# TigreGotico/phoonnx

Measured on AMD Instinct MI355X. Metric: audio samples/sec (22.05 kHz), batch-32 256-phoneme utterances, higher is better.
Workload: dtype f32 (f16x3 split: fp32 operands as two fp16 planes, three MFMA products, fp32 accumulate)

## Files before the change

include/vitsmi.h:

```cpp
#ifndef VITSMI_H
#define VITSMI_H

#include <stddef.h>
#include <stdint.h>

#ifdef __cplusplus
extern "C" {
#endif

typedef struct vits_handle vits_handle;

enum {
    VITS_OK = 0,
    VITS_E_IO = -1,
    VITS_E_FORMAT = -2,
    VITS_E_ARG = -3,
    VITS_E_DEVICE = -4,
    VITS_E_NOMEM = -5,
    VITS_E_RANGE = -6
};

#define VITS_MAX_DIMS 4


// ... 302 lines not shown
int vits_glide_emit_end(const vits_glide_seg *segs, int n_segs, int64_t n_in, int64_t n_out, int64_t X, int64_t *ready);
int64_t vits_warp_stream_cap(int64_t piece_samples, int64_t S_w);
int vits_run_chunked_glided(vits_handle *h, const int64_t *ids, const int64_t *lens, int B, int T, const int64_t *sid,
                            const vits_noise *noise, const vits_controls *ctl, const vits_contour *contour, int chunk_frames,
                            vits_chunk_fn fn, void *user);
int vits_run_chunked_enc_glided(vits_handle *h, const int64_t *ids, const int64_t *lens, int B, int T, const int64_t *sid,
                                const vits_noise *noise, const vits_controls *ctl, const vits_stream_format *fmt,
                                const vits_stream_shaping *shaping, const vits_stream_onset *onsets, const vits_contour *contour,
                                int chunk_frames, vits_enc_chunk_trim_fn fn, void *user);

enum { VITS_FIT_MET = 0, VITS_FIT_FLOOR = 1, VITS_FIT_CEIL = 2, VITS_FIT_KEPT = 3 };
typedef struct {
    const int32_t *group;
    int n_groups;
    const int64_t *target_frames;
    const int32_t *mode;
} vits_fit;
int vits_fit_plan(const float *w, const int64_t *lens, int B, int T, const vits_fit *fit, int64_t *durations, double *scale,
                  int64_t *frames, int32_t *status);
int vits_run_async_fitted(vits_handle *h, const int64_t *ids, const int64_t *lens, int B, int T, const int64_t *sid,
                          const vits_noise *noise, const vits_controls *ctl, const vits_fit *fit);
int vits_run_chunked_fitted(vits_handle *h, const int64_t *ids, const int64_t *lens, int B, int T, const int64_t *sid,
                            const vits_noise *noise, const vits_controls *ctl, const vits_fit *fit, int chunk_frames,
                            vits_chunk_fn fn, void *user);
int vits_run_chunked_enc_fitted(vits_handle *h, const int64_t *ids, const int64_t *lens, int B, int T, const int64_t *sid,
                                const vits_noise *noise, const vits_controls *ctl, const vits_stream_format *fmt,
                                const vits_stream_shaping *shaping, const vits_stream_onset *onsets, const vits_fit *fit,
                                int chunk_frames, vits_enc_chunk_trim_fn fn, void *user);
int vits_last_fit(vits_handle *h, double *scale, int64_t *frames, int32_t *status, int n);

int vits_reserve(vits_handle *h, int B, int T, int F);
int vits_get_stats(vits_handle *h, vits_stats *out);

typedef struct {
    char kernel[128];
    double flops, bytes;
    float ms;
    int stage;
    int cin, cout, k, dil, t;
} vits_launch_record;
int vits_launch_records(vits_handle *h, vits_launch_record *buf, int n);

void *vits_stream(vits_handle *h);


int vits_test_conv1d(int device_id, const float *x, int B, int Cin, int T, const float *w, const float *bias,
                     int Cout, int K, int dil, int pad_l, int flags, float slope, float *out);
int vits_bench_conv1d(int device_id, int B, int Cin, int Cout, int T, int K, int dil, int hint, int iters,
                      int cfg_override, int ck_override, float *ms_out);
int vits_test_conv_transpose1d(int device_id, const float *x, int B, int Cin, int T, const float *w,
                               const float *bias, int Cout, int K, int stride, float *out);
enum {
    VITS_CONV_PRO_LRELU = 1, VITS_CONV_PRO_MASK = 2, VITS_CONV_EPI_RELU = 4, VITS_CONV_EPI_MASK = 8, VITS_CONV_EPI_RES = 16,
    VITS_CONV_EPI_ACC = 32, VITS_CONV_EPI_DIV = 64, VITS_CONV_EPI_COUPLING = 128, VITS_CONV_EPI_WN = 256,
    VITS_CONV_EPI_WN_FIRST = 512
};
typedef struct {
    int B, Cin, T, Cout;
    int K, dil, pad_l;
    int stride;
    int hint, cfg, ck;
    int flags;
    float slope, div, oslope, oslope2;
    int wn_split;
    const float *x;
    const float *w, *bias;
    const int64_t *lens;
    const float *bias_b;
    int bias_b_stride;
    const float *res;
    int x_cstride;
    int out_cstride;
    int out_rows, out_row0;
    const float *old_out, *old_out2;
    float sentinel;
    float *out, *out2;
    int pl_rows;
    float *planes_out;
    char kernel[128];
    int cfg_used, ck_used;
} vits_test_conv_epi_args;
int vits_test_conv1d_epi(int device_id, vits_test_conv_epi_args *a);
int vits_test_wn_gate(int device_id, const float *a, int B, int H, int T, int form, float *acts);
int vits_test_cond_matvec(int device_id, const float *emb_g, int n_speakers, int gin, const int64_t *sid, int B,
                          const float *W, const float *bias, int rows, float *out);
int vits_test_conv1d_sx(int device_id, const float *x, int B, int Cin, int T, const float *w, const float *bias,
                        int Cout, int K, int dil, int pad_l, int flags, float slope, float *out);
enum { VITS_SX_EPI_RES = 1, VITS_SX_EPI_ACC = 2, VITS_SX_EPI_DIV = 4, VITS_SX_EPI_NO_RAW_STORE = 8 };
enum { VITS_SX_BF16X6 = 0, VITS_SX_F16X3 = 1, VITS_SX_F16 = 2 };
typedef struct {
    int B, Cin, T, Cout;
    int K, dil, pad_l;
    int stride;
    int precision;
    int force16, no_s16, min_cfg;
    int run_cfg;
    int flags;
    const float *x;
    const float *w, *bias;
    const float *res;
    int res_is_x;
    int res_planes;
    float res_slope;
    const float *old_out;
    const float *bias_b;
    int bias_b_stride;
    float div, oslope, oslope2, islope;
    const int64_t *lens;
    int rag_add, rag_mul;
    float sentinel;
    float *out;
    float *planes_out;
    float *res_seen;
    char kernel[128];
    int pack_cfg, run_cfg_used, rawin, s16, ck;
    float peak;
} vits_test_conv_sx_epi_args;
int vits_test_conv1d_sx_epi(int device_id, vits_test_conv_sx_epi_args *a);
int vits_test_conv1d_sx_planar(int device_id, const float *x, int B, int Cin, int T, const float *w, const float *bias,
                               int Cout, int K, int dil, int flags, const int64_t *lens, const float *old, int row_split,
                               int pl_rows, float *out, float *planes_out);
long long vits_test_set_sx_small_max(long long wgs);
int vits_test_conv1d_sx_gate(int device_id, const float *x, int B, int Cin, int T, const float *w, const float *bias,
                             const float *bias_b, int Cout, int K, int dil, int flags, float *out);
int vits_test_conv_transpose1d_sx(int device_id, const float *x, int B, int Cin, int T, const float *w,
                                  const float *bias, int Cout, int K, int stride, float *out);
int vits_bench_conv1d_sx(int device_id, int B, int Cin, int Cout, int T, int K, int dil, int dbg, int iters,
                         float *ms_out);
int vits_test_conv_pair_sx(int device_id, const float *x, int B, int C, int T, const float *w1, const float *b1,
                           const float *w2, const float *b2, int K, int dil1, int dil2, int chain, float slope, float *out,
                           float *ms_out);
enum { VITS_P16_EPI_ACC = 1, VITS_P16_EPI_DIV = 2, VITS_P16_EPI_RAW = 4, VITS_P16_EPI_PLANES = 8 };
typedef struct {
    int B, C, T, K, dil1, dil2, chain;
    int precision;
    int flags;
    float slope, div, sentinel;
    const float *x;
    const float *w1, *b1, *w2, *b2;
    const float *old_out;
    const float *x_tail;
    const int64_t *lens;
    int rag_add, rag_mul;
    float *out;
    float *planes_out;
    float *x_seen;
    float *ms_out;
    char kernel[128];
    int BN, BNo, ovl;
    float peak;
    int guard_ok;
} vits_test_conv_pair16_epi_args;
int vits_test_conv_pair16_epi(int device_id, vits_test_conv_pair16_epi_args *a);
int vits_test_attention(int device_id, const float *qkv, int B, int C, int T, int n_heads, const float *rel_k,
                        const float *rel_v, int window, const int64_t *lens, float *out);
int vits_test_attention16(int device_id, const float *qkv, int B, int C, int T, int n_heads, const float *rel_k,
                          const float *rel_v, int window, const int64_t *lens, float *out, uint16_t *out_planes, int kernel,
                          int reps, float *ms_out);
typedef struct {
    int kernel;
    const float *qkv;
    const uint16_t *qkv_planes;
    int B, C, T, n_heads, window;
    const float *rel_k, *rel_v;
    const int64_t *lens;
    int want_out;
    int want_planes;
    int ns, qt;
    int kh;
    float *out;
    uint16_t *out_planes;
    float peak;
    char kernel_name[128];
} vits_test_attention_form_args;
int vits_test_attention_form(int device_id, vits_test_attention_form_args *a);

int vits_test_resample(int device_id, const float *x, const int64_t *lens, int B, int S, int in_rate, int out_rate, float *y,
                       int64_t S_out);
int vits_test_resample_pieces(int device_id, const float *x, const int64_t *lens, int B, int S, int in_rate, int out_rate,
                              int piece_samples, float *y, int64_t S_out, int64_t *ranges, int max_ranges);
int vits_test_resample_rows(int device_id, const float *x, const int64_t *lens, int B, int S, int in_rate,
                            const int32_t *out_rates, float *y, size_t y_elems, int64_t *n_out);
int vits_test_warp(int device_id, const float *x, const int64_t *counts, int B, int S, const vits_warp_seg *segs,
                   const int32_t *seg_first , float *y, int S_w);
int vits_test_glide(int device_id, const float *x, const int64_t *counts, int B, int S, const vits_glide_seg *segs,
                    const int32_t *seg_first , float *y, int S_w);
int vits_test_warp_pieces(int device_id, const float *x, const int64_t *counts, int B, int S, const vits_warp_seg *segs,
                          const int32_t *seg_first , const int64_t *piece_bounds, int n_pieces, float *y, int S_w,
                          int64_t *ranges, int max_ranges);
int vits_test_glide_pieces(int device_id, const float *x, const int64_t *counts, int B, int S, const vits_glide_seg *segs,
                           const int32_t *seg_first , const int64_t *piece_bounds, int n_pieces, float *y, int S_w,
                           int64_t *ranges, int max_ranges);

int vits_test_durations(int device_id, const float *logw, const int64_t *dur, const int64_t *lens, int B, int T, float length_scale,
                        const float *rows, const float *token_rate, float *w_ceil, int32_t *cum, int32_t *y_len);
int vits_test_fit_durations(int device_id, const float *w, const int64_t *lens, int B, int T, const vits_fit *fit, float *w_ceil,
                            int32_t *cum, int32_t *y_len, double *scale, int64_t *frames, int32_t *status);
int vits_test_expand_prior(int device_id, const float *m_logs, int B, int C, int T, const int32_t *cum, const int64_t *lens,
                           const int32_t *y_len, int F, const float *noise, int64_t noise_stride, int noise_frames,
                           float noise_scale, const float *rows, const uint64_t *seeds, float *z_p);
int vits_test_fill_normal(int device_id, int64_t n, uint64_t seed, uint64_t stream_id, float *out);
int vits_test_fill_normal_rows(int device_id, int B, int channels, int T, const uint64_t *seeds, uint32_t stream, const float *rows,
                               int col, float *out);
int vits_test_post_conv(int device_id, const float *x, int B, int C, int T, const float *w, int K, float slope, const int64_t *vlen,
                        int hop, int kernel, float *out);

int vits_test_layernorm(int device_id, const float *x, const float *out_init, int B, int C, int T, const float *gamma,
                        const float *beta, const int64_t *lens, int flags, int form, int in_place, const float *dw_w,
                        const float *dw_b, int K, int dil, float *out, uint16_t *planes);
typedef struct vits_test_dds_layer {
    const float *dw_w, *dw_b;
    const float *ln1_g, *ln1_b;
    const float *pw_w, *pw_b;
    const float *ln2_g, *ln2_b;
    int32_t dil;
} vits_test_dds_layer;
int vits_test_dds(int device_id, int form, const float *x, int B, int C, int T, const int64_t *lens, int n_layers,
                  const vits_test_dds_layer *layers, int mask_out, const float *head_cond, const float *head_z, int head_ch,
                  const float *head_w, const float *head_b, const float *tail_w, const float *tail_b, int tail_rows, float *out);
int vits_test_cf_pre(int device_id, const float *z, int ch, const float *w, const float *bias, const float *cond, int B, int C, int T,
                     float *out);
int vits_test_rqs_inverse(int device_id, const float *pr, const float *z, int B, int T, const int64_t *lens, int ch0, int nb,
                          float sqrt_c, float *out);
int vits_test_ea_logw(int device_id, const float *z, int ch, float m0, float logs0, const int64_t *lens, int B, int T, float *out);

int vits_test_deliver(int device_id, const float *x, const int64_t *counts, int B, int S, const vits_segment *segs, int n_segs,
                      int n_streams, int encoding, void *dst, size_t dst_bytes, int64_t *stream_samples, int64_t *stream_offsets);

int vits_test_deliver_trimmed(int device_id, const float *x, const int64_t *counts, int B, int S, const vits_segment *segs,
                              const vits_trim *trims, int n_segs, int n_streams, int encoding, void *dst, size_t dst_bytes,
                              int64_t *stream_samples, int64_t *stream_offsets, int64_t *kept_first, int64_t *kept_count);

int vits_test_loudness_blocks(int device_id, const float *x, const int64_t *counts, const int64_t *firsts, int B, int S,
                              int sample_rate, float *e, size_t e_cap, int32_t *n_sub, int32_t *chunk);

int vits_test_deliver_leveled(int device_id, const float *x, const int64_t *counts, int B, int S, const vits_segment *segs,
                              const vits_trim *trims, const vits_level *levels, int n_segs, int n_streams, int encoding,
                              int sample_rate, void *dst, size_t dst_bytes, int64_t *stream_samples, int64_t *stream_offsets,
                              int64_t *kept_first, int64_t *kept_count, double *loudness, float *gain);

int vits_test_deliver_shaped(int device_id, const float *x, const int64_t *counts, int B, int S, const vits_segment *segs,
                             const vits_trim *trims, const vits_level *levels, const vits_shape *shapes, const vits_env_point *points,
                             int64_t n_points, int n_segs, int n_streams, int encoding, int sample_rate, void *dst, size_t dst_bytes,
                             int64_t *stream_samples, int64_t *stream_offsets, int64_t *kept_first, int64_t *kept_count,
                             double *loudness, float *gain);

int vits_test_deliver_limited(int device_id, const float *x, const int64_t *counts, int B, int S, const vits_segment *segs,
                              const vits_trim *trims, const vits_level *levels, const vits_shape *shapes, const vits_env_point *points,
                              int64_t n_points, const vits_limit *limits, int n_segs, int n_streams, int encoding, int sample_rate,
                              void *dst, size_t dst_bytes, int64_t *stream_samples, int64_t *stream_offsets, int64_t *kept_first,
                              int64_t *kept_count, double *loudness, float *gain);

int vits_test_stream_pack(int device_id, const float *x, const int64_t *counts, int B, int S, int piece_samples,
                          const vits_stream_format *fmt, void *bytes, size_t bytes_cap, int64_t *pitches, int32_t *valid,
                          float *peaks, int max_pieces);

int vits_test_stream_pack_shaped(int device_id, const float *x, const int64_t *counts, int B, int S, int piece_samples,
                                 const vits_stream_format *fmt, const vits_stream_shaping *shaping, void *bytes, size_t bytes_cap,
                                 int64_t *pitches, int32_t *valid, float *peaks, int64_t *firsts, int64_t *ns, int max_pieces);

int vits_test_stream_pack_trimmed(int device_id, const float *x, const int64_t *counts, int B, int S, int piece_samples,
                                  const vits_stream_format *fmt, const vits_stream_shaping *shaping, const vits_stream_onset *onsets,
                                  void *bytes, size_t bytes_cap, int64_t *pitches, int32_t *valid, int32_t *skip, float *peaks,
                                  int64_t *firsts, int64_t *ns, int32_t *start, int max_pieces);

#ifdef __cplusplus
}
#endif
#endif
```

phoonnx_amd/_ffi.py:

```python
import ctypes as C
import os

import numpy as np

from . import audio_encoding

_HERE = os.path.dirname(os.path.abspath(__file__))
_LIB = None

VITS_MAX_DIMS = 4


class VitsNoise(C.Structure):
    _fields_ = [("noise_dp", C.c_void_p), ("noise_z", C.c_void_p), ("noise_z_stride", C.c_int64),
                ("seed", C.c_uint64)]


class VitsOutput(C.Structure):
    _fields_ = [("data", C.POINTER(C.c_float)), ("dims", C.c_int64 * 4), ("y_lengths", C.POINTER(C.c_int64))]


class VitsStats(C.Structure):
    _fields_ = [("conv_flops", C.c_double), ("conv_bytes", C.c_double), ("dec_flops", C.c_double),
                ("dec_bytes", C.c_double), ("flow_flops", C.c_double), ("enc_flops", C.c_double),
                ("dp_flops", C.c_double), ("conv_ms", C.c_float), ("dec_ms", C.c_float), ("flow_ms", C.c_float),
                ("enc_ms", C.c_float), ("dp_ms", C.c_float), ("total_ms", C.c_float), ("conv_launches", C.c_int),
                ("total_launches", C.c_int), ("sx_flops", C.c_double), ("sx_ms", C.c_float), ("sx_launches", C.c_int),
                ("f16_peak_max", C.c_float), ("f16_peak_min", C.c_float), ("f16_tracked", C.c_int),
                ("f16_saturated", C.c_int), ("sx_bytes", C.c_double)]


class VitsLaunchRecord(C.Structure):
    _fields_ = [("kernel", C.c_char * 128), ("flops", C.c_double), ("bytes", C.c_double), ("ms", C.c_float),
                ("stage", C.c_int), ("cin", C.c_int), ("cout", C.c_int), ("k", C.c_int), ("dil", C.c_int), ("t", C.c_int)]


class VitsTestConvEpiArgs(C.Structure):
    _fields_ = [(n, C.c_int) for n in ("B", "Cin", "T", "Cout", "K", "dil", "pad_l", "stride", "hint", "cfg", "ck", "flags")] + \
               [(n, C.c_float) for n in ("slope", "div", "oslope", "oslope2")] + [("wn_split", C.c_int)] + \
               [(n, C.c_void_p) for n in ("x", "w", "bias", "lens", "bias_b")] + [("bias_b_stride", C.c_int), ("res", C.c_void_p)] + \
               [(n, C.c_int) for n in ("x_cstride", "out_cstride", "out_rows", "out_row0")] + \
               [("old_out", C.c_void_p), ("old_out2", C.c_void_p), ("sentinel", C.c_float), ("out", C.c_void_p), ("out2", C.c_void_p),
                ("pl_rows", C.c_int), ("planes_out", C.c_void_p), ("kernel", C.c_char * 128), ("cfg_used", C.c_int), ("ck_used", C.c_int)]


class VitsTestConvSxEpiArgs(C.Structure):
    _fields_ = [(n, C.c_int) for n in ("B", "Cin", "T", "Cout", "K", "dil", "pad_l", "stride", "precision", "force16", "no_s16",
                                       "min_cfg", "run_cfg", "flags")] + \
               [(n, C.c_void_p) for n in ("x", "w", "bias", "res")] + \
               [("res_is_x", C.c_int), ("res_planes", C.c_int), ("res_slope", C.c_float), ("old_out", C.c_void_p),
                ("bias_b", C.c_void_p), ("bias_b_stride", C.c_int)] + \
               [(n, C.c_float) for n in ("div", "oslope", "oslope2", "islope")] + \
               [("lens", C.c_void_p), ("rag_add", C.c_int), ("rag_mul", C.c_int), ("sentinel", C.c_float), ("out", C.c_void_p),
                ("planes_out", C.c_void_p), ("res_seen", C.c_void_p), ("kernel", C.c_char * 128)] + \
               [(n, C.c_int) for n in ("pack_cfg", "run_cfg_used", "rawin", "s16", "ck")] + [("peak", C.c_float)]


class VitsTestConvPair16EpiArgs(C.Structure):
    _fields_ = [(n, C.c_int) for n in ("B", "C", "T", "K", "dil1", "dil2", "chain", "precision", "flags")] + \
               [(n, C.c_float) for n in ("slope", "div", "sentinel")] + \
               [(n, C.c_void_p) for n in ("x", "w1", "b1", "w2", "b2", "old_out", "x_tail", "lens")] + \
               [("rag_add", C.c_int), ("rag_mul", C.c_int)] + \
               [(n, C.c_void_p) for n in ("out", "planes_out", "x_seen", "ms_out")] + [("kernel", C.c_char * 128)] + \
               [(n, C.c_int) for n in ("BN", "BNo", "ovl")] + [("peak", C.c_float), ("guard_ok", C.c_int)]


class VitsTestAttentionFormArgs(C.Structure):
    _fields_ = [("kernel", C.c_int), ("qkv", C.c_void_p), ("qkv_planes", C.c_void_p)] + \
               [(n, C.c_int) for n in ("B", "C", "T", "n_heads", "window")] + \
               [(n, C.c_void_p) for n in ("rel_k", "rel_v", "lens")] + \
               [(n, C.c_int) for n in ("want_out", "want_planes", "ns", "qt", "kh")] + \
               [("out", C.c_void_p), ("out_planes", C.c_void_p), ("peak", C.c_float), ("kernel_name", C.c_char * 128)]


class VitsOpenOptions(C.Structure):
    _fields_ = [("device_id", C.c_int), ("gen_precision", C.c_char_p), ("arena_dev", C.c_void_p),
                ("arena_bytes", C.c_size_t), ("host_only", C.c_int), ("layout_only", C.c_int)]


class VitsControls(C.Structure):
    _fields_ = [("scales_rows", C.c_void_p), ("seeds", C.c_void_p), ("durations", C.c_void_p), ("token_rate", C.c_void_p)]


class VitsFit(C.Structure):
    _fields_ = [("group", C.c_void_p), ("n_groups", C.c_int), ("target_frames", C.c_void_p), ("mode", C.c_void_p)]


VITS_FIT_MET, VITS_FIT_FLOOR, VITS_FIT_CEIL, VITS_FIT_KEPT = 0, 1, 2, 3


class VitsWarpSeg(C.Structure):
    _fields_ = [("n0", C.c_int64), ("pos0", C.c_int64), ("k", C.c_int64), ("step", C.c_int32), ("c", C.c_int32),
                ("half_taps", C.c_int32), ("pad_", C.c_int32)]


class VitsIntonation(C.Structure):
    _fields_ = [("token_semitones", C.c_void_p), ("compensate", C.c_int)]


class VitsGlideSeg(C.Structure):
    _fields_ = [("n0", C.c_int64), ("pos0", C.c_int64), ("k", C.c_int64), ("step0", C.c_int32), ("step1", C.c_int32),
                ("pad_", C.c_int32 * 2)]


class VitsContour(C.Structure):
    _fields_ = [("token_semitones", C.c_void_p), ("token_semitones_end", C.c_void_p), ("compensate", C.c_int)]


class VitsSegment(C.Structure):
    _fields_ = [("row", C.c_int32), ("stream", C.c_int32), ("lead_samples", C.c_int64), ("normalize", C.c_int32),
                ("volume", C.c_float)]


class VitsTrim(C.Structure):
    _fields_ = [("mode", C.c_int32), ("threshold", C.c_float), ("keep_lead", C.c_int32), ("keep_tail", C.c_int32),
                ("tail_samples", C.c_int64)]


class VitsTestDdsLayer(C.Structure):
    _fields_ = [("dw_w", C.c_void_p), ("dw_b", C.c_void_p), ("ln1_g", C.c_void_p), ("ln1_b", C.c_void_p), ("pw_w", C.c_void_p),
                ("pw_b", C.c_void_p), ("ln2_g", C.c_void_p), ("ln2_b", C.c_void_p), ("dil", C.c_int32)]


class VitsLevel(C.Structure):
    _fields_ = [("mode", C.c_int32), ("target_lufs", C.c_float), ("max_gain_db", C.c_float), ("peak_ceiling", C.c_float)]


class VitsEnvPoint(C.Structure):
    _fields_ = [("pos", C.c_int32), ("gain", C.c_float)]


class VitsShape(C.Structure):
    _fields_ = [("fade_in", C.c_int32), ("fade_out", C.c_int32), ("curve", C.c_int32), ("n_points", C.c_int32),
                ("first_point", C.c_int64)]


class VitsLimit(C.Structure):
    _fields_ = [("mode", C.c_int32), ("ceiling", C.c_float), ("lookahead", C.c_int32), ("reserved", C.c_int32)]


class VitsStreamFormat(C.Structure):
    _fields_ = [("encoding", C.c_int32), ("ref_peak", C.c_void_p), ("volume", C.c_void_p)]


class VitsStreamShaping(C.Structure):
    pass


STREAM_PLAN_FN = C.CFUNCTYPE(C.c_int, C.c_void_p, C.c_int, C.c_int, C.POINTER(C.c_int64), C.POINTER(C.c_int64), C.POINTER(VitsStreamShaping))

VitsStreamShaping._fields_ = [("shapes", C.c_void_p), ("points", C.c_void_p), ("n_points", C.c_int64), ("ceiling", C.c_void_p),
                              ("lookahead", C.c_int32), ("reserved", C.c_int32), ("plan", STREAM_PLAN_FN), ("plan_user", C.c_void_p)]


class VitsStreamOnset(C.Structure):
    _fields_ = [("mode", C.c_int32), ("threshold", C.c_float), ("keep_lead", C.c_int32), ("reserved", C.c_int32)]


ENCODINGS = {name: (code, audio_encoding.DTYPES[name]) for code, name in enumerate(audio_encoding.ENCODINGS)}


CHUNK_FN = C.CFUNCTYPE(C.c_int, C.c_void_p, C.POINTER(C.c_float), C.c_int, C.c_int64, C.c_int64, C.c_int64)

ENC_CHUNK_FN = C.CFUNCTYPE(C.c_int, C.c_void_p, C.c_void_p, C.c_int, C.c_int64, C.c_int64, C.c_int64, C.POINTER(C.c_int32),
                           C.POINTER(C.c_float), C.c_int64)

ENC_CHUNK_TRIM_FN = C.CFUNCTYPE(C.c_int, C.c_void_p, C.c_void_p, C.c_int, C.c_int64, C.c_int64, C.c_int64, C.POINTER(C.c_int32),
                                C.POINTER(C.c_int32), C.POINTER(C.c_float), C.c_int64)

VITS_E_RANGE = -6


EXPORTS = [
    "vits_open", "vits_open_with_arena", "vits_open_host", "vits_open_layout", "vits_open_opts", "vits_close",
    "vits_run_chunked", "vits_run_vocoder_chunked", "vits_last_error", "vits_num_inputs",
    "vits_input_name", "vits_meta", "vits_hparam", "vits_arena_bytes", "vits_arena_host", "vits_arena_device",
    "vits_run", "vits_free_output", "vits_run_device", "vits_sync", "vits_last_y_lengths", "vits_last_pcm16", "vits_run_vocoder",
    "vits_tap",
    "vits_set_timing", "vits_set_tails", "vits_reserve", "vits_get_stats", "vits_stream", "vits_test_conv1d", "vits_test_conv_transpose1d",
    "vits_test_attention", "vits_test_attention16", "vits_bench_conv1d", "vits_test_conv1d_sx", "vits_test_conv1d_sx_planar", "vits_test_conv1d_sx_gate", "vits_test_set_sx_small_max",
    "vits_test_conv_transpose1d_sx",
    "vits_bench_conv1d_sx", "vits_test_conv_pair_sx", "vits_fetch_output", "vits_run_async", "vits_host_alloc", "vits_host_free",
    "vits_launch_records", "vits_run_async_rows", "vits_run_device_rows", "vits_run_chunked_rows",
    "vits_run_async_ctl", "vits_run_chunked_ctl", "vits_last_durations",
    "vits_set_output_rate", "vits_last_sample_counts", "vits_resample_plan", "vits_test_resample", "vits_test_resample_pieces",
    "vits_set_output_rates", "vits_last_sample_rates", "vits_test_resample_rows",
    "vits_run_async_warped", "vits_last_token_spans", "vits_warp_token", "vits_warp_plan", "vits_test_warp",
    "vits_run_async_glided", "vits_glide_token", "vits_glide_cutoff", "vits_glide_plan", "vits_test_glide",
    "vits_warp_emit_end", "vits_glide_emit_end", "vits_warp_stream_cap", "vits_run_chunked_glided", "vits_run_chunked_enc_glided",
    "vits_test_warp_pieces", "vits_test_glide_pieces",
    "vits_fit_plan", "vits_run_async_fitted", "vits_run_chunked_fitted", "vits_run_chunked_enc_fitted", "vits_last_fit",
    "vits_test_fit_durations",
    "vits_test_durations", "vits_test_expand_prior", "vits_test_fill_normal", "vits_test_fill_normal_rows", "vits_test_post_conv",
    "vits_delivery_plan", "vits_deliver", "vits_test_deliver",
    "vits_trim_range", "vits_delivery_plan_trimmed", "vits_deliver_trimmed", "vits_test_deliver_trimmed",
    "vits_loudness_filter", "vits_loudness_gate", "vits_level_gain", "vits_delivery_plan_leveled", "vits_deliver_leveled",
    "vits_test_loudness_blocks", "vits_test_deliver_leveled",
    "vits_shape_check", "vits_shape_gain", "vits_deliver_shaped", "vits_test_deliver_shaped",
    "vits_limit_check", "vits_limit_gains", "vits_deliver_limited", "vits_test_deliver_limited",
    "vits_run_chunked_enc", "vits_run_vocoder_chunked_enc", "vits_test_stream_pack",
    "vits_stream_shaping_check", "vits_stream_emit_range", "vits_run_chunked_enc_shaped", "vits_run_vocoder_chunked_enc_shaped",
    "vits_test_stream_pack_shaped",
    "vits_stream_onset_check", "vits_stream_onset_start", "vits_run_chunked_enc_trimmed", "vits_run_vocoder_chunked_enc_trimmed",
    "vits_test_stream_pack_trimmed",
    "vits_test_layernorm", "vits_test_dds", "vits_test_cf_pre", "vits_test_rqs_inverse", "vits_test_ea_logw",
    "vits_test_conv1d_epi", "vits_test_wn_gate", "vits_test_cond_matvec", "vits_test_conv1d_sx_epi",
    "vits_test_conv_pair16_epi", "vits_test_attention_form",
]


G2P_EXPORTS = ["g2p_open", "g2p_close", "g2p_last_error", "g2p_hparam", "g2p_num_outputs", "g2p_output_name", "g2p_bucket",
               "g2p_run", "g2p_generate", "g2p_generate_batch", "g2p_test_forced_steps", "g2p_test_linear", "g2p_test_step"]


def lib_path():
    return os.environ.get("VITSMI_LIB") or os.path.join(_HERE, "libvitsmi.so")


def load():
    global _LIB
    if _LIB is not None:
        return _LIB
    path = lib_path()
    if not os.environ.get("VITSMI_LIB"):
        from . import build as _build
        if _build.stale():
            try:
                _build.build()
            except Exception as e:
                raise RuntimeError(f"{path} is missing or was not built from the sources in this tree (source_sha "
                                   f"{_build.source_sha()} vs recorded {_build.read_build_info().get('source_sha')}) "
                                   f"and cannot be rebuilt here: {e}") from e
    lib = C.CDLL(path)
    vp, i64p, f32p = C.c_void_p, C.POINTER(C.c_int64), C.POINTER(C.c_float)
    lib.vits_open.argtypes = [C.c_char_p, C.c_int, C.POINTER(vp)]
    lib.vits_open_with_arena.argtypes = [C.c_char_p, C.c_int, vp, C.c_size_t, C.POINTER(vp)]
    lib.vits_open_host.argtypes = [C.c_char_p, C.POINTER(vp)]
    lib.vits_open_layout.argtypes = [C.c_char_p, C.POINTER(vp)]
    lib.vits_open_opts.argtypes = [C.c_char_p, C.POINTER(VitsOpenOptions), C.POINTER(vp)]
    lib.vits_run_chunked.argtypes = [vp, vp, vp, C.c_int, C.c_int, vp, vp, C.POINTER(VitsNoise), C.c_int, CHUNK_FN, vp]
    lib.vits_run_vocoder_chunked.argtypes = [vp, vp, C.c_int, C.c_int, vp, C.c_int, CHUNK_FN, vp]
    lib.vits_close.argtypes = [vp]
    lib.vits_close.restype = None
    lib.vits_last_error.argtypes = [vp]
    lib.vits_last_error.restype = C.c_char_p
    lib.vits_num_inputs.argtypes = [vp]
    lib.vits_input_name.argtypes = [vp, C.c_int]
    lib.vits_input_name.restype = C.c_char_p
    lib.vits_meta.argtypes = [vp, C.c_char_p, C.c_char_p, C.c_size_t]
    lib.vits_hparam.argtypes = [vp, C.c_char_p, i64p]
    lib.vits_arena_bytes.argtypes = [vp]
    lib.vits_arena_bytes.restype = C.c_size_t
    lib.vits_arena_host.argtypes = [vp]
    lib.vits_arena_host.restype = vp
    lib.vits_arena_device.argtypes = [vp]
    lib.vits_arena_device.restype = vp
    run_args = [vp, vp, vp, C.c_int, C.c_int, vp, vp, C.POINTER(VitsNoise), C.POINTER(VitsOutput)]
    lib.vits_run.argtypes = run_args
    lib.vits_run_device.argtypes = run_args
    lib.vits_run_async.argtypes = run_args[:-1]
    lib.vits_run_async_rows.argtypes = run_args[:-1] + [vp]
    lib.vits_run_device_rows.argtypes = run_args[:-1] + [vp, C.POINTER(VitsOutput)]
    lib.vits_run_chunked_rows.argtypes = [vp, vp, vp, C.c_int, C.c_int, vp, vp, C.POINTER(VitsNoise), vp, C.c_int, CHUNK_FN, vp]
    lib.vits_run_async_ctl.argtypes = [vp, vp, vp, C.c_int, C.c_int, vp, C.POINTER(VitsNoise), C.POINTER(VitsControls)]
    lib.vits_run_chunked_ctl.argtypes = [vp, vp, vp, C.c_int, C.c_int, vp, C.POINTER(VitsNoise), C.POINTER(VitsControls),
                                         C.c_int, CHUNK_FN, vp]
    lib.vits_run_chunked_enc.argtypes = [vp, vp, vp, C.c_int, C.c_int, vp, C.POINTER(VitsNoise), C.POINTER(VitsControls),
                                         C.POINTER(VitsStreamFormat), C.c_int, ENC_CHUNK_FN, vp]
    lib.vits_run_vocoder_chunked_enc.argtypes = [vp, vp, C.c_int, C.c_int, vp, C.POINTER(VitsStreamFormat), C.c_int, ENC_CHUNK_FN, vp]
    lib.vits_stream_shaping_check.argtypes = [C.POINTER(VitsStreamShaping), C.POINTER(VitsStreamFormat), C.c_int]
    lib.vits_stream_emit_range.argtypes = [C.c_int64, C.c_int64, C.c_int, C.c_int64, C.c_int, i64p, i64p]
    lib.vits_run_chunked_enc_shaped.argtypes = [vp, vp, vp, C.c_int, C.c_int, vp, C.POINTER(VitsNoise), C.POINTER(VitsControls),
                                                C.POINTER(VitsStreamFormat), C.POINTER(VitsStreamShaping), C.c_int, ENC_CHUNK_FN, vp]
    lib.vits_run_vocoder_chunked_enc_shaped.argtypes = [vp, vp, C.c_int, C.c_int, vp, C.POINTER(VitsStreamFormat),
                                                        C.POINTER(VitsStreamShaping), C.c_int, ENC_CHUNK_FN, vp]
    lib.vits_test_stream_pack_shaped.argtypes = [C.c_int, vp, vp, C.c_int, C.c_int, C.c_int, C.POINTER(VitsStreamFormat),
                                                 C.POINTER(VitsStreamShaping), vp, C.c_size_t, vp, vp, vp, vp, vp, C.c_int]
    lib.vits_stream_onset_check.argtypes = [C.POINTER(VitsStreamOnset), C.POINTER(VitsStreamFormat), C.c_int]
    lib.vits_stream_onset_start.argtypes = [C.c_int64, C.c_int64, C.c_int64, i64p]
    lib.vits_run_chunked_enc_trimmed.argtypes = [vp, vp, vp, C.c_int, C.c_int, vp, C.POINTER(VitsNoise), C.POINTER(VitsControls),
                                                 C.POINTER(VitsStreamFormat), C.POINTER(VitsStreamShaping), C.POINTER(VitsStreamOnset),
                                                 C.c_int, ENC_CHUNK_TRIM_FN, vp]
    lib.vits_run_vocoder_chunked_enc_trimmed.argtypes = [vp, vp, C.c_int, C.c_int, vp, C.POINTER(VitsStreamFormat),
                                                         C.POINTER(VitsStreamShaping), C.POINTER(VitsStreamOnset), C.c_int,
                                                         ENC_CHUNK_TRIM_FN, vp]
    lib.vits_test_stream_pack_trimmed.argtypes = [C.c_int, vp, vp, C.c_int, C.c_int, C.c_int, C.POINTER(VitsStreamFormat),
                                                  C.POINTER(VitsStreamShaping), C.POINTER(VitsStreamOnset), vp, C.c_size_t, vp, vp, vp, vp,
                                                  vp, vp, vp, C.c_int]
    lib.vits_test_stream_pack.argtypes = [C.c_int, vp, vp, C.c_int, C.c_int, C.c_int, C.POINTER(VitsStreamFormat), vp, C.c_size_t,
                                          vp, vp, vp, C.c_int]
    lib.vits_last_durations.argtypes = [vp, i64p, C.c_size_t]
    lib.vits_set_output_rate.argtypes = [vp, C.c_int, C.c_int]
    lib.vits_last_sample_counts.argtypes = [vp, i64p, C.c_int]
    lib.vits_resample_plan.argtypes = [C.c_int, C.c_int, i64p, i64p, i64p, vp, C.c_size_t]
    lib.vits_test_resample.argtypes = [C.c_int, vp, vp, C.c_int, C.c_int, C.c_int, C.c_int, vp, C.c_int64]
    lib.vits_test_resample_pieces.argtypes = [C.c_int, vp, vp, C.c_int, C.c_int, C.c_int, C.c_int, C.c_int, vp, C.c_int64, vp, C.c_int]
    lib.vits_set_output_rates.argtypes = [vp, C.c_int, vp, C.c_int]
    lib.vits_last_sample_rates.argtypes = [vp, vp, C.c_int]
    lib.vits_test_resample_rows.argtypes = [C.c_int, vp, vp, C.c_int, C.c_int, C.c_int, vp, vp, C.c_size_t, vp]
    lib.vits_run_async_warped.argtypes = [vp, vp, vp, C.c_int, C.c_int, vp, C.POINTER(VitsNoise), C.POINTER(VitsControls),
                                          C.POINTER(VitsIntonation)]
    lib.vits_last_token_spans.argtypes = [vp, i64p, C.c_size_t]
    lib.vits_warp_token.argtypes = [C.c_float, i64p, i64p, C.POINTER(C.c_int32)]
    lib.vits_warp_plan.argtypes = [vp, vp, C.c_int, C.c_int, vp, vp, i64p]
    lib.vits_test_warp.argtypes = [C.c_int, vp, vp, C.c_int, C.c_int, vp, vp, vp, C.c_int]
    lib.vits_run_async_glided.argtypes = [vp, vp, vp, C.c_int, C.c_int, vp, C.POINTER(VitsNoise), C.POINTER(VitsControls),
                                          C.POINTER(VitsContour)]
    lib.vits_glide_token.argtypes = [C.c_float, C.c_float, i64p, i64p, C.POINTER(C.c_float)]
    lib.vits_glide_cutoff.argtypes = [C.c_int64, i64p, C.POINTER(C.c_int32)]
    lib.vits_glide_plan.argtypes = [vp, vp, vp, C.c_int, C.c_int, vp, vp, i64p]
    lib.vits_test_glide.argtypes = [C.c_int, vp, vp, C.c_int, C.c_int, vp, vp, vp, C.c_int]
    for name in ("vits_warp_emit_end", "vits_glide_emit_end"):
        getattr(lib, name).argtypes = [vp, C.c_int, C.c_int64, C.c_int64, C.c_int64, i64p]
    lib.vits_warp_stream_cap.argtypes = [C.c_int64, C.c_int64]
    lib.vits_warp_stream_cap.restype = C.c_int64
    lib.vits_run_chunked_glided.argtypes = [vp, vp, vp, C.c_int, C.c_int, vp, C.POINTER(VitsNoise), C.POINTER(VitsControls),
                                            C.POINTER(VitsContour), C.c_int, CHUNK_FN, vp]
    lib.vits_run_chunked_enc_glided.argtypes = [vp, vp, vp, C.c_int, C.c_int, vp, C.POINTER(VitsNoise), C.POINTER(VitsControls),
                                                C.POINTER(VitsStreamFormat), C.POINTER(VitsStreamShaping), C.POINTER(VitsStreamOnset),
                                                C.POINTER(VitsContour), C.c_int, ENC_CHUNK_TRIM_FN, vp]
    for name in ("vits_test_warp_pieces", "vits_test_glide_pieces"):
        getattr(lib, name).argtypes = [C.c_int, vp, vp, C.c_int, C.c_int, vp, vp, vp, C.c_int, vp, C.c_int, vp, C.c_int]
    lib.vits_fit_plan.argtypes = [vp, vp, C.c_int, C.c_int, C.POINTER(VitsFit), vp, vp, vp, vp]
    lib.vits_run_async_fitted.argtypes = [vp, vp, vp, C.c_int, C.c_int, vp, C.POINTER(VitsNoise), C.POINTER(VitsControls),
                                          C.POINTER(VitsFit)]
    lib.vits_run_chunked_fitted.argtypes = [vp, vp, vp, C.c_int, C.c_int, vp, C.POINTER(VitsNoise), C.POINTER(VitsControls),
                                            C.POINTER(VitsFit), C.c_int, CHUNK_FN, vp]
    lib.vits_run_chunked_enc_fitted.argtypes = [vp, vp, vp, C.c_int, C.c_int, vp, C.POINTER(VitsNoise), C.POINTER(VitsControls),
                                                C.POINTER(VitsStreamFormat), C.POINTER(VitsStreamShaping), C.POINTER(VitsStreamOnset),
                                                C.POINTER(VitsFit), C.c_int, ENC_CHUNK_TRIM_FN, vp]
    lib.vits_last_fit.argtypes = [vp, vp, vp, vp, C.c_int]
    lib.vits_test_fit_durations.argtypes = [C.c_int, vp, vp, C.c_int, C.c_int, C.POINTER(VitsFit), vp, vp, vp, vp, vp, vp]
    lib.vits_test_durations.argtypes = [C.c_int, vp, vp, vp, C.c_int, C.c_int, C.c_float, vp, vp, vp, vp, vp]
    lib.vits_test_expand_prior.argtypes = [C.c_int, vp, C.c_int, C.c_int, C.c_int, vp, vp, vp, C.c_int, vp, C.c_int64, C.c_int,
                                           C.c_float, vp, vp, vp]
    lib.vits_test_fill_normal.argtypes = [C.c_int, C.c_int64, C.c_uint64, C.c_uint64, vp]
    lib.vits_test_fill_normal_rows.argtypes = [C.c_int, C.c_int, C.c_int, C.c_int, vp, C.c_uint32, vp, C.c_int, vp]
    lib.vits_test_post_conv.argtypes = [C.c_int, vp, C.c_int, C.c_int, C.c_int, vp, C.c_int, C.c_float, vp, C.c_int, C.c_int, vp]
    lib.vits_test_layernorm.argtypes = [C.c_int, vp, vp, C.c_int, C.c_int, C.c_int, vp, vp, vp, C.c_int, C.c_int, C.c_int, vp, vp,
                                        C.c_int, C.c_int, vp, vp]
    lib.vits_test_dds.argtypes = [C.c_int, C.c_int, vp, C.c_int, C.c_int, C.c_int, vp, C.c_int, C.POINTER(VitsTestDdsLayer), C.c_int,
                                  vp, vp, C.c_int, vp, vp, vp, vp, C.c_int, vp]
    lib.vits_test_cf_pre.argtypes = [C.c_int, vp, C.c_int, vp, vp, vp, C.c_int, C.c_int, C.c_int, vp]
    lib.vits_test_rqs_inverse.argtypes = [C.c_int, vp, vp, C.c_int, C.c_int, vp, C.c_int, C.c_int, C.c_float, vp]
    lib.vits_test_ea_logw.argtypes = [C.c_int, vp, C.c_int, C.c_float, C.c_float, vp, C.c_int, C.c_int, vp]
    lib.vits_delivery_plan.argtypes = [vp, C.c_int, vp, C.c_int, C.c_int, C.c_int, vp, vp, i64p]
    lib.vits_deliver.argtypes = [vp, vp, C.c_int, C.c_int, C.c_int, vp, C.c_size_t, vp, vp]
    lib.vits_test_deliver.argtypes = [C.c_int, vp, vp, C.c_int, C.c_int, vp, C.c_int, C.c_int, C.c_int, vp, C.c_size_t, vp, vp]
    lib.vits_trim_range.argtypes = [C.c_int64, C.c_int64, C.c_int64, C.POINTER(VitsTrim), i64p, i64p]
    lib.vits_delivery_plan_trimmed.argtypes = [vp, C.c_int, vp, vp, C.c_int, C.c_int, C.c_int, vp, vp, i64p]
    lib.vits_deliver_trimmed.argtypes = [vp, vp, vp, C.c_int, C.c_int, C.c_int, vp, C.c_size_t, vp, vp, vp, vp]
    lib.vits_test_deliver_trimmed.argtypes = [C.c_int, vp, vp, C.c_int, C.c_int, vp, vp, C.c_int, C.c_int, C.c_int, vp, C.c_size_t,
                                              vp, vp, vp, vp]
    lib.vits_loudness_filter.argtypes = [C.c_int, vp, vp]
    lib.vits_loudness_gate.argtypes = [vp, vp, C.c_int, C.c_int32, vp, vp, vp, vp]
    lib.vits_level_gain.argtypes = [C.c_double, C.c_float, C.POINTER(VitsLevel), C.POINTER(C.c_float)]
    lib.vits_delivery_plan_leveled.argtypes = [vp, C.c_int, vp, vp, vp, C.c_int, C.c_int, C.c_int, C.c_int, vp, vp, i64p]
    lib.vits_deliver_leveled.argtypes = [vp, vp, vp, vp, C.c_int, C.c_int, C.c_int, C.c_int, vp, C.c_size_t, vp, vp, vp, vp, vp, vp]
    lib.vits_test_loudness_blocks.argtypes = [C.c_int, vp, vp, vp, C.c_int, C.c_int, C.c_int, vp, C.c_size_t, vp, vp]
    lib.vits_test_deliver_leveled.argtypes = [C.c_int, vp, vp, C.c_int, C.c_int, vp, vp, vp, C.c_int, C.c_int, C.c_int, C.c_int, vp,
                                              C.c_size_t, vp, vp, vp, vp, vp, vp]
    lib.vits_shape_check.argtypes = [vp, C.c_int, vp, C.c_int64]
    lib.vits_shape_gain.argtypes = [C.POINTER(VitsShape), vp, C.c_int64, C.c_int64, C.c_int64, C.POINTER(C.c_float)]
    lib.vits_deliver_shaped.argtypes = [vp, vp, vp, vp, vp, vp, C.c_int64, C.c_int, C.c_int, C.c_int, C.c_int, vp, C.c_size_t, vp, vp, vp,
                                        vp, vp, vp]
    lib.vits_test_deliver_shaped.argtypes = [C.c_int, vp, vp, C.c_int, C.c_int, vp, vp, vp, vp, vp, C.c_int64, C.c_int, C.c_int, C.c_int,
                                             C.c_int, vp, C.c_size_t, vp, vp, vp, vp, vp, vp]
    lib.vits_limit_check.argtypes = [vp, vp, C.c_int]
    lib.vits_limit_gains.argtypes = [vp, C.c_int64, C.POINTER(VitsLimit), vp]
    lib.vits_deliver_limited.argtypes = [vp, vp, vp, vp, vp, vp, C.c_int64, vp, C.c_int, C.c_int, C.c_int, C.c_int, vp, C.c_size_t, vp,
                                         vp, vp, vp, vp, vp]
    lib.vits_test_deliver_limited.argtypes = [C.c_int, vp, vp, C.c_int, C.c_int, vp, vp, vp, vp, vp, C.c_int64, vp, C.c_int, C.c_int,
                                              C.c_int, C.c_int, vp, C.c_size_t, vp, vp, vp, vp, vp, vp]
    lib.vits_free_output.argtypes = [vp, C.POINTER(VitsOutput)]
    lib.vits_free_output.restype = None
    lib.vits_sync.argtypes = [vp]
    lib.vits_last_y_lengths.argtypes = [vp, i64p, C.c_int]
    lib.vits_last_pcm16.argtypes = [vp, C.c_int, C.c_float, vp, C.c_size_t]
    lib.vits_run_vocoder.argtypes = [vp, vp, C.c_int, C.c_int, vp, C.POINTER(VitsOutput)]
    lib.vits_tap.argtypes = [vp, C.c_char_p, vp, C.c_size_t, i64p]
    lib.vits_set_timing.argtypes = [vp, C.c_int]
    lib.vits_set_tails.argtypes = [vp, C.c_int]
    lib.vits_reserve.argtypes = [vp, C.c_int, C.c_int, C.c_int]
    lib.vits_get_stats.argtypes = [vp, C.POINTER(VitsStats)]
    lib.vits_stream.argtypes = [vp]
    lib.vits_stream.restype = vp
    lib.vits_fetch_output.argtypes = [vp, vp, C.c_size_t, C.c_size_t]
    lib.vits_host_alloc.argtypes = [C.c_size_t]
    lib.vits_host_alloc.restype = vp
    lib.vits_host_free.argtypes = [vp]
    lib.vits_host_free.restype = None
    lib.vits_launch_records.argtypes = [vp, C.POINTER(VitsLaunchRecord), C.c_int]
    lib.vits_test_conv1d.argtypes = [C.c_int, vp, C.c_int, C.c_int, C.c_int, vp, vp, C.c_int, C.c_int, C.c_int,
                                     C.c_int, C.c_int, C.c_float, vp]
    lib.vits_test_conv_transpose1d.argtypes = [C.c_int, vp, C.c_int, C.c_int, C.c_int, vp, vp, C.c_int, C.c_int,
                                               C.c_int, vp]
    lib.vits_test_attention.argtypes = [C.c_int, vp, C.c_int, C.c_int, C.c_int, C.c_int, vp, vp, C.c_int, vp, vp]
    lib.vits_test_attention16.argtypes = [C.c_int, vp, C.c_int, C.c_int, C.c_int, C.c_int, vp, vp, C.c_int, vp, vp, vp,
                                          C.c_int, C.c_int, f32p]
    lib.vits_bench_conv1d.argtypes = [C.c_int] * 11 + [f32p]
    lib.vits_test_conv1d_sx.argtypes = lib.vits_test_conv1d.argtypes
    lib.vits_test_conv_transpose1d_sx.argtypes = lib.vits_test_conv_transpose1d.argtypes
    lib.vits_test_conv1d_sx_planar.argtypes = [C.c_int, vp, C.c_int, C.c_int, C.c_int, vp, vp, C.c_int, C.c_int, C.c_int, C.c_int,
                                               vp, vp, C.c_int, C.c_int, vp, vp]
    lib.vits_test_set_sx_small_max.argtypes = [C.c_longlong]
    lib.vits_test_set_sx_small_max.restype = C.c_longlong
    lib.vits_test_conv1d_sx_gate.argtypes = [C.c_int, vp, C.c_int, C.c_int, C.c_int, vp, vp, vp, C.c_int, C.c_int, C.c_int, C.c_int, vp]
    lib.vits_bench_conv1d_sx.argtypes = [C.c_int] * 9 + [f32p]
    lib.vits_test_conv1d_epi.argtypes = [C.c_int, C.POINTER(VitsTestConvEpiArgs)]
    lib.vits_test_conv1d_sx_epi.argtypes = [C.c_int, C.POINTER(VitsTestConvSxEpiArgs)]
    lib.vits_test_conv_pair16_epi.argtypes = [C.c_int, C.POINTER(VitsTestConvPair16EpiArgs)]
    lib.vits_test_attention_form.argtypes = [C.c_int, C.POINTER(VitsTestAttentionFormArgs)]
    lib.vits_test_wn_gate.argtypes = [C.c_int, vp, C.c_int, C.c_int, C.c_int, C.c_int, vp]
    lib.vits_test_cond_matvec.argtypes = [C.c_int, vp, C.c_int, C.c_int, vp, C.c_int, vp, vp, C.c_int, vp]
    lib.vits_test_conv_pair_sx.argtypes = [C.c_int, vp, C.c_int, C.c_int, C.c_int, vp, vp, vp, vp, C.c_int, C.c_int,
                                           C.c_int, C.c_int, C.c_float, vp, f32p]
    lib.g2p_open.argtypes = [C.c_char_p, C.c_int, C.POINTER(vp)]
    lib.g2p_close.argtypes = [vp]
    lib.g2p_close.restype = None
    lib.g2p_last_error.argtypes = [vp]
    lib.g2p_last_error.restype = C.c_char_p
    lib.g2p_hparam.argtypes = [vp, C.c_char_p, i64p]
    lib.g2p_num_outputs.argtypes = [vp]
    lib.g2p_output_name.argtypes = [vp, C.c_int]
    lib.g2p_output_name.restype = C.c_char_p
    lib.g2p_bucket.argtypes = [vp, C.c_int, C.c_int]
    lib.g2p_run.argtypes = [vp, vp, C.c_int, vp, vp, C.c_int, vp]
    lib.g2p_generate.argtypes = [vp, vp, C.c_int, C.c_int, C.c_int64, C.c_int64, vp, C.POINTER(C.c_int)]
    lib.g2p_generate_batch.argtypes = [vp, vp, vp, C.c_int, C.c_int, C.c_int64, C.c_int64, vp, vp]
    lib.g2p_test_forced_steps.argtypes = [vp, vp, vp, C.c_int, vp, C.c_int, vp]
    lib.g2p_test_linear.argtypes = [C.c_int, C.c_int, vp, vp, C.c_int, vp, C.c_int, C.c_int, vp, C.c_int64, C.c_int64, C.c_int, vp]
    lib.g2p_test_step.argtypes = [C.c_int, C.c_int, C.c_int, vp, vp, vp, C.c_int, vp, vp, C.c_int, C.c_float, C.c_float, vp, vp]
    _LIB = lib
    return lib


def ptr(a):
    return None if a is None else a.ctypes.data_as(C.c_void_p)


def last_error(h=None):
    return load().vits_last_error(h).decode("utf-8", "replace")
```

phoonnx_amd/csrc/conv_sx_pair.hip.hpp:

```cpp
#pragma once
#include <cstdlib>
#include "conv_geom.hpp"
#include "conv_sx_engine.hip.hpp"

namespace vitsmi {

struct SxPairArgs {
    const float *xr;
    float islope, mslope;
    int T;
    const u32x4 *wp1, *wp2;
    const float *bias1, *bias2;
    float wscale1, wscale2;
    float *out_raw;
    const float *zeros;
    int C, nchunks;
    int K1, dil1, pad1;
    int K2, dil2, pad2;
    int LW1;
    unsigned x_bytes;
    int LW2;
    unsigned y_chunk_bytes;
    int BNo, NT, B;
    int flags;
    float div;
    unsigned *peak;
    struct Chain {
        const u32x4 *wp1, *wp2;
        const float *bias1, *bias2;
        float wscale1, wscale2;
        int K1, dil1, K2, dil2;
        int xoff, yoff;
    } ch[3];
    int nchain;
    unsigned a_ring;
    unsigned bias_off;
    unsigned long long *prof;
    SxRagged rag;
    int xgs = 0;
};

#ifndef SX_PAIR_PROF
#define SX_PAIR_PROF 0
#endif
#ifndef SX_PAIR_SHARED_A
#define SX_PAIR_SHARED_A 0
#endif
#ifndef SX_PAIR_ALIAS
#define SX_PAIR_ALIAS 0
#endif
#ifndef SX_PAIR_DEPTH32
#define SX_PAIR_DEPTH32 2
#endif
#ifndef SX_PAIR_DEPTH64
#define SX_PAIR_DEPTH64 2
#endif
#ifndef SX_PAIR_EARLY_ACC
#define SX_PAIR_EARLY_ACC 0
#endif
#ifndef SX_PAIR_WGS32
#define SX_PAIR_WGS32 3
#endif
#ifndef SX_PAIR_EARLY32
#define SX_PAIR_EARLY32 1
#endif
#ifndef SX_PAIR_ST_SC1
#define SX_PAIR_ST_SC1 0
#endif
#ifndef SX_PAIR_ONE_READ64
#define SX_PAIR_ONE_READ64 1
#endif
#ifndef SX_PAIR_ONE_READ32
#define SX_PAIR_ONE_READ32 1
#endif
template <int MW, int NW, int WM, int WN, int EPI, bool CHAIN, int NCH = 1>
__global__ __launch_bounds__(256, (NW == 2 && !SX_PAIR_EARLY_ACC && NCH == 1) ? SX_PAIR_WGS32 : 2) void conv_sx_pair_kernel(SxPairArgs a) {
    constexpr int BN = NW * WN * 32, NH = NW / 2;
    static_assert(NCH == 1 || (CHAIN && NW == 2 && (EPI & EPI_ACC) == 0), "fused chains: 32 channels, no external running sum");
    constexpr bool ONE_READ = NW == 4 ? SX_PAIR_ONE_READ64 != 0 : SX_PAIR_ONE_READ32 != 0;
    constexpr bool EARLY = ONE_READ || (NW == 2 && SX_PAIR_EARLY32);
    constexpr int DEPTH = NW == 2 ? SX_PAIR_DEPTH32 : SX_PAIR_DEPTH64;
    static_assert(DEPTH >= 2 && DEPTH <= 6, "wait_a covers up to five younger sets");
    constexpr bool ACC = (EPI & EPI_ACC) != 0 && SX_PAIR_EARLY_ACC;
    static_assert(!(ONE_READ && ACC), "the running sum is not pulled into the single-read prologue");
    static_assert(WM * WN == 4 && MW == 1 && BN == 256, "one block row per wave, 256 columns");
    constexpr int NPW = 2, STEPBYTES = WM * MW * NPW * 1024;
    constexpr int MAXCH = WM * 2;
    extern __shared__ __attribute__((aligned(16))) unsigned char lds_sx[];
    const int tid = threadIdx.x, lane = tid & 63;
    const int wave = __builtin_amdgcn_readfirstlane(tid >> 6);
    const int wm = wave / WN, wn = wave % WN;
    const int l31 = lane & 31, hi = lane >> 5;
    const int wg_xcd = blockIdx.x & 7, wg_seq = blockIdx.x >> 3;
    const int tile_nb = __builtin_amdgcn_readfirstlane(sx_xcd_tile(wg_seq, wg_xcd, a.xgs));
    if (tile_nb >= a.NT * a.B) return;
    const int b = tile_nb / a.NT, t0 = (tile_nb - b * a.NT) * a.BNo;
    const int t1 = t0 - a.pad2;
    const int T = a.T, LW = a.LW1;
    const int TV = __builtin_amdgcn_readfirstlane(sx_valid_cols(a.rag, b, T));
    if (t0 >= TV) return;
    const uint32_t lds0 = (uint32_t)(uintptr_t)lds_sx;
    const uint32_t XB = a.x_bytes;
    const char *wbase1 = reinterpret_cast<const char *>(a.wp1) + wm * (MW * NPW * 1024);
    const char *wbase2 = reinterpret_cast<const char *>(a.wp2) + wm * (MW * NPW * 1024);
    const float *xrb = a.xr + (int64_t)b * a.C * T;
    float pk = 0.f;

    struct ASet {
        u32x4 fa[2];
    };
    const uint32_t voff0 = (uint32_t)lane * 16u;
    auto load_a = [&](ASet &f, const char *wb, int step) {
        const char *sb = wb + (int64_t)step * STEPBYTES;
        f.fa[0] = global_read128<0>(voff0, sb);
        f.fa[1] = global_read128<1024>(voff0, sb);
    };

    f32x4 pre[NW / 2][2][4], ad[EARLY && ACC ? NW / 2 : 1][2][4];
    auto load_res = [&](const float *base, f32x4 (*dst)[2][4]) {
        static_for<NW / 2>([&](auto R) {
            constexpr int rr = decltype(R)::value;
#pragma unroll
            for (int j = 0; j < 2; j++) {
                const int row0 = wm * 32;
                const int t = t1 + (wn * NW + rr * 2 + j) * 32 + l31;
                const int tl = t < 0 ? 0 : (t < T ? t : T - 1);
#pragma unroll
                for (int q = 0; q < 4; q++) {
                    const float *p = base + ((int64_t)((row0 >> 3) + q) * T + tl) * 8 + 4 * hi;
                    if constexpr (EARLY) dst[rr][j][q] = __builtin_bit_cast(f32x4, global_read128_v<0>(p));
                    else dst[rr][j][q] = *reinterpret_cast<const f32x4 *>(p);
                }
            }
        });
    };
    auto load_pre = [&]() { load_res(xrb, pre); };

#if SX_PAIR_PROF
    auto stamp = [&]() {
        unsigned long long t;
        __builtin_amdgcn_sched_barrier(0);
        asm volatile("s_memtime %0\n\ts_waitcnt lgkmcnt(0)" : "=s"(t)::"memory");
        __builtin_amdgcn_sched_barrier(0);
        return t;
    };
    unsigned long long tp[8];
    tp[0] = stamp();
#endif
    if constexpr (NW == 2 && WM == 1 && NCH == 1 && SX_PAIR_SHARED_A != 0)
        for (int g = 0; g < 3; g++)
            if (g < ((a.nchunks * a.K1) >> 1)) {
                const int sub = wave >> 1, pl = wave & 1;
                lds_dma<16>(wbase1 + (int64_t)(2 * g + sub) * STEPBYTES + pl * 1024 + lane * 16,
                            reinterpret_cast<float *>(lds_sx + a.a_ring + (unsigned)((g * 2 + sub) * 2048 + pl * 1024)));
            }
    constexpr bool BIAS_LDS = NCH == 1;
    if constexpr (BIAS_LDS) {
        if (wave == 0) {
            constexpr int CC = WM * 32;
            const int k = lane - (lane >= CC / 4 ? CC / 4 : 0);
            const float *bp = lane < CC / 4 ? a.bias1 : a.bias2;
            const void *src = (bp && lane < CC / 2) ? static_cast<const void *>(bp + 4 * k) : static_cast<const void *>(a.zeros + 4 * (lane & 31));
            lds_dma<16>(src, reinterpret_cast<float *>(lds_sx + a.bias_off));
        }
    }
    auto bias_from_lds = [&](int conv, f32x4 (&bq)[4]) __attribute__((always_inline)) {
        u32x4 t4[4];
#pragma unroll
        for (int q = 0; q < 4; q++)
            asm volatile("ds_read_b128 %0, %1" : "=v"(t4[q]) : "v"(lds0 + a.bias_off + (uint32_t)(conv * (WM * 32) + wm * 32 + 8 * q + 4 * hi) * 4u) : "memory");
        asm volatile("s_waitcnt lgkmcnt(0)" ::: "memory");
        __builtin_amdgcn_sched_barrier(0);
#pragma unroll
        for (int q = 0; q < 4; q++) bq[q] = __builtin_bit_cast(f32x4, t4[q]);
    };
    constexpr int NXC = 3;
    if constexpr (ONE_READ) {
        constexpr int NXH = MAXCH, NG = 2 * MAXCH;
        const int HW = LW - 256, pad1 = a.pad1;
        const int nhc = HW * NG, nxh = (nhc + 255) >> 8;
        u32x4 hst[NXH][2];
        bool hin[NXH], hok[NXH];
        uint32_t hlds[NXH];
        const float *hp[NXH];
#pragma unroll
        for (int it = 0; it < NXH; it++) {
            const int h = it * 256 + tid;
            hin[it] = h < nhc;
            const int g = hin[it] ? h / HW : 0;
            const int c = hin[it] ? h - g * HW : 0;
            const int col = c < pad1 ? c : c + 256;
            const int t = t1 - pad1 + col;
            hok[it] = hin[it] && t >= 0 && t < TV;
            hp[it] = xrb + (hok[it] ? ((int64_t)g * T + t) * 8 : (int64_t)0);
            hlds[it] = lds0 + (uint32_t)(g >> 1) * XB + (uint32_t)((g & 1) * LW + col) * 16u;
        }
        static_for<NXH>([&](auto I) {
            constexpr int it = decltype(I)::value;
            if (it < nxh) {
                hst[it][0] = global_read128_v<0>(hp[it]);
                hst[it][1] = global_read128_v<16>(hp[it]);
            }
        });
        load_pre();
        const float isl = a.islope;
        static_for<NW>([&](auto N) {
            constexpr int n = decltype(N)::value;
            asm volatile("s_waitcnt vmcnt(%0)" ::"n"(4 * (NW - 1 - n)) : "memory");
            __builtin_amdgcn_sched_barrier(0);
#if SX_PAIR_PROF
            if constexpr (n == 0) tp[1] = stamp();
#endif
            if constexpr (n == 0) {
                static_for<NXH>([&](auto I) {
                    constexpr int it = decltype(I)::value;
                    if (it < nxh && hin[it]) {
                        float v[8];
#pragma unroll
                        for (int e = 0; e < 8; e++) {
                            const float x = hok[it] ? __uint_as_float(hst[it][e >> 2][e & 3]) : 0.f;
                            v[e] = fmaxf(x, x * isl);
                        }
                        unsigned p0[4], p1[4];
#pragma unroll
                        for (int e = 0; e < 4; e++) split2h_pair_pk(v[2 * e], v[2 * e + 1], p0[e], p1[e], pk);
                        ds_write128(hlds[it], u32x4{p0[0], p0[1], p0[2], p0[3]});
                        ds_write128(hlds[it] + (uint32_t)(2 * LW) * 16u, u32x4{p1[0], p1[1], p1[2], p1[3]});
                    }
                });
            }
            const int col = (wn * NW + n) * 32 + l31;
            const int t = t1 + col;
            const bool ok = t >= 0 && t < TV;
#pragma unroll
            for (int q = 0; q < 4; q++) {
                float v[4];
#pragma unroll
                for (int e = 0; e < 4; e++) {
                    const float x = ok ? pre[n / 2][n % 2][q][e] : 0.f;
                    v[e] = fmaxf(x, x * isl);
                }
                unsigned wa[2], wb[2];
                split2h_pair_pk(v[0], v[1], wa[0], wa[1], pk);
                split2h_pair_pk(v[2], v[3], wb[0], wb[1], pk);
                const int g = 4 * wm + q;
                const uint32_t cell = lds0 + (uint32_t)(g >> 1) * XB + (uint32_t)((g & 1) * LW + pad1 + col) * 16u + 8u * hi;
                asm volatile("ds_write_b64 %0, %1" ::"v"(cell), "v"(u32x2{wa[0], wb[0]}) : "memory");
                asm volatile("ds_write_b64 %0, %1" ::"v"(cell + (uint32_t)(2 * LW) * 16u), "v"(u32x2{wa[1], wb[1]}) : "memory");
            }
            asm volatile("" : "+v"(pk));
        });
    } else {
        u32x4 xst[MAXCH][NXC][2];
        const int nxc = (2 * LW + 255) >> 8;
        uint32_t xroff[NXC];
        bool xrok[NXC];
        int xkh[NXC], xcol[NXC];
#pragma unroll
        for (int it = 0; it < NXC; it++) {
            const int i = it * 256 + tid;
            const int kh = (i >= LW ? 1 : 0) + (i >= 2 * LW ? 1 : 0);
            const int col = i - kh * LW;
            const int t = t1 - a.pad1 + col;
            xkh[it] = kh;
            xcol[it] = col;
            xrok[it] = it < nxc && kh < 2 && t >= 0 && t < TV;
            xroff[it] = xrok[it] ? (uint32_t)(((int64_t)kh * T + t) * 32) : 0u;
        }
        static_for<MAXCH>([&](auto CH) {
            constexpr int ch = decltype(CH)::value;
            const float *cbase = xrb + (int64_t)(2 * ch) * T * 8;
            static_for<NXC>([&](auto I) {
                constexpr int it = decltype(I)::value;
                if (it < nxc) {
                    xst[ch][it][0] = global_read128_x<0>(xroff[it], cbase);
                    xst[ch][it][1] = global_read128_x<16>(xroff[it], cbase);
                }
            });
        });
        if constexpr (EARLY) {
            load_pre();
            if constexpr (ACC) {
                load_res(a.out_raw + (int64_t)b * a.C * T, ad);
                asm volatile("s_waitcnt vmcnt(16)" ::: "memory");
            } else
                asm volatile("s_waitcnt vmcnt(8)" ::: "memory");
        } else
            asm volatile("s_waitcnt vmcnt(0)" ::: "memory");
#if SX_PAIR_PROF
        tp[1] = stamp();
#endif
        const float isl = a.islope;
        static_for<MAXCH>([&](auto CH) {
            constexpr int ch = decltype(CH)::value;
            static_for<NXC>([&](auto I) {
                constexpr int it = decltype(I)::value;
                if (it < nxc && xkh[it] < 2) {
                    float v[8];
#pragma unroll
                    for (int e = 0; e < 8; e++) {
                        const float x = xrok[it] ? __uint_as_float(xst[ch][it][e >> 2][e & 3]) : 0.f;
                        v[e] = fmaxf(x, x * isl);
                    }
                    unsigned p0[4], p1[4];
#pragma unroll
                    for (int e = 0; e < 4; e++) split2h_pair_pk(v[2 * e], v[2 * e + 1], p0[e], p1[e], pk);
                    const uint32_t ad = lds0 + (uint32_t)ch * XB + (uint32_t)(xkh[it] * LW + xcol[it]) * 16u;
                    ds_write128(ad, u32x4{p0[0], p0[1], p0[2], p0[3]});
                    ds_write128(ad + (uint32_t)(2 * LW) * 16u, u32x4{p1[0], p1[1], p1[2], p1[3]});
                }
            });
        });
    }

    f32x16 acc[NW];
    auto zero_acc = [&]() {
#pragma unroll
        for (int n = 0; n < NW; n++)
#pragma unroll
            for (int r = 0; r < 16; r++) acc[n][r] = 0.f;
    };
    zero_acc();
    u32x4 fb[NW][2];
// ... 24 lines not shown
    };
    const std::integral_constant<int, 0> H0{};
    const std::integral_constant<int, 1> H1{};

    auto wait_a = [&](int younger) {
        switch (younger) {
            case 0: asm volatile("s_waitcnt vmcnt(0)" ::: "memory"); break;
            case 1: asm volatile("s_waitcnt vmcnt(2)" ::: "memory"); break;
            case 2: asm volatile("s_waitcnt vmcnt(4)" ::: "memory"); break;
            case 3: asm volatile("s_waitcnt vmcnt(6)" ::: "memory"); break;
            case 4: asm volatile("s_waitcnt vmcnt(8)" ::: "memory"); break;
            default: asm volatile("s_waitcnt vmcnt(10)" ::: "memory"); break;
        }
    };
    auto run_conv = [&](ASet(&fs)[DEPTH + 1], const char *wb, int K, int dil, uint32_t rows0, uint32_t chunk_bytes,
                        uint32_t pstride) {
        constexpr int NS = DEPTH + 1;
        const int S = a.nchunks * K;
        int chunk = 0, tap = 0;
        static_for<DEPTH - 1>([&](auto I) {
            constexpr int i = decltype(I)::value + 1;
            if (i < S) load_a(fs[i], wb, i);
        });
        load_b_half(H0, rows0, pstride);
        load_b_half(H1, rows0, pstride);
        auto step = [&](ASet &fc, ASet &fload, int s) {
            const int left = S - 1 - s;
            wait_a(left < DEPTH - 1 ? left : DEPTH - 1);
            __builtin_amdgcn_sched_barrier(0);
            if (s + DEPTH < S && !SX_NOA) load_a(fload, wb, s + DEPTH);
            int ntap = tap + 1, nchunk = chunk;
            if (ntap == K) {
                ntap = 0;
                nchunk++;
            }
            const bool more = s + 1 < S;
            const uint32_t next = rows0 + (uint32_t)nchunk * chunk_bytes + (uint32_t)(ntap * dil) * 16u;
            __builtin_amdgcn_sched_barrier(0);
            wait_lds_older_half();
            __builtin_amdgcn_sched_barrier(0);
            mma_half(fc, H0);
            __builtin_amdgcn_sched_barrier(0);
            if (more) {
                load_b_half(H0, next, pstride);
                wait_lds_older_half();
            } else
                asm volatile("s_waitcnt lgkmcnt(0)" ::: "memory");
            __builtin_amdgcn_sched_barrier(0);
            mma_half(fc, H1);
            __builtin_amdgcn_sched_barrier(0);
            if (more) load_b_half(H1, next, pstride);
            __builtin_amdgcn_sched_barrier(0);
            tap = ntap;
            chunk = nchunk;
        };
        int s = 0;
        for (; s + NS <= S; s += NS)
            static_for<NS>([&](auto I) {
                constexpr int i = decltype(I)::value;
                step(fs[i], fs[(i + DEPTH) % NS], s + i);
            });
        __builtin_amdgcn_sched_barrier(0);
        asm volatile("s_waitcnt lgkmcnt(0)" ::: "memory");
        __builtin_amdgcn_sched_barrier(0);
        static_for<NS - 1>([&](auto I) {
            constexpr int i = decltype(I)::value;
            if (s + i < S) step(fs[i], fs[(i + DEPTH) % NS], s + i);
        });
    };

    constexpr bool SHA = NW == 2 && WM == 1 && NCH == 1 && SX_PAIR_SHARED_A != 0;
    constexpr int RG = 3;
    auto sha_dma = [&](const char *wb, int g) {
        const int sub = wave >> 1, pl = wave & 1;
        const char *src = wb + (int64_t)(2 * g + sub) * STEPBYTES + pl * 1024 + lane * 16;
        lds_dma<16>(src, reinterpret_cast<float *>(lds_sx + a.a_ring + (unsigned)(((g % RG) * 2 + sub) * 2048 + pl * 1024)));
    };
    auto sha_prefetch = [&](const char *wb, int K) {
        const int NG = (a.nchunks * K) >> 1;
#pragma unroll
        for (int g = 0; g < RG; g++)
            if (g < NG) sha_dma(wb, g);
    };
    auto wait_vm_le = [&](int n) {
        switch (n) {
            case 0: asm volatile("s_waitcnt vmcnt(0)" ::: "memory"); break;
            case 1: asm volatile("s_waitcnt vmcnt(1)" ::: "memory"); break;
            default: asm volatile("s_waitcnt vmcnt(2)" ::: "memory"); break;
        }
    };
    auto run_conv_sha = [&](ASet &fa0, ASet &fa1, const char *wb, int K, int dil, uint32_t rows0, uint32_t chunk_bytes,
                            uint32_t pstride) {
        const int S = a.nchunks * K, NG = S >> 1;
        const uint32_t alds = lds0 + a.a_ring + (uint32_t)lane * 16u;
        auto read_a = [&](ASet &f, int st) {
            const uint32_t ad = alds + (uint32_t)((((st >> 1) % RG) * 2 + (st & 1)) * 2048);
            f.fa[0] = ds_read128<0>(ad);
            f.fa[1] = ds_read128<1024>(ad);
        };
        int chunk = 0, tap = 0;
        wait_vm_le((NG < RG ? NG : RG) - 1);
        __builtin_amdgcn_s_barrier();
        __builtin_amdgcn_sched_barrier(0);
        read_a(fa0, 0);
        load_b_half(H0, rows0, pstride);
        load_b_half(H1, rows0, pstride);
        auto step = [&](ASet &fc, ASet &fload, int st, bool boundary) {
            int ntap = tap + 1, nchunk = chunk;
            if (ntap == K) {
                ntap = 0;
                nchunk++;
            }
            const bool more = st + 1 < S;
            const uint32_t next = rows0 + (uint32_t)nchunk * chunk_bytes + (uint32_t)(ntap * dil) * 16u;
            __builtin_amdgcn_sched_barrier(0);
            wait_lds_older_half();
            __builtin_amdgcn_sched_barrier(0);
            mma_half(fc, H0);
            __builtin_amdgcn_sched_barrier(0);
            if (more) {
                if (boundary && NG > RG) {
                    const int g = st >> 1;
                    const int last = g + RG - 1 < NG - 1 ? g + RG - 1 : NG - 1;
                    wait_vm_le(last - (g + 1));
                    __builtin_amdgcn_s_barrier();
                    __builtin_amdgcn_sched_barrier(0);
                    if (g + RG < NG) sha_dma(wb, g + RG);
                }
                read_a(fload, st + 1);
                load_b_half(H0, next, pstride);
                asm volatile("s_waitcnt lgkmcnt(4)" ::: "memory");
            } else
                asm volatile("s_waitcnt lgkmcnt(0)" ::: "memory");
            __builtin_amdgcn_sched_barrier(0);
            mma_half(fc, H1);
            __builtin_amdgcn_sched_barrier(0);
            if (more) load_b_half(H1, next, pstride);
            __builtin_amdgcn_sched_barrier(0);
            tap = ntap;
            chunk = nchunk;
        };
        for (int g = 0; g < NG; g++) {
            step(fa0, fa1, 2 * g, false);
            step(fa1, fa0, 2 * g + 1, true);
        }
    };

    struct ChainPar {
        const char *wb1, *wb2;
        const float *bias1, *bias2;
        float ws1, ws2;
        int K1, dil1, K2, dil2;
        uint32_t xoff, yoff;
    };
    auto chain_par = [&](int ci) {
        ChainPar c;
        if constexpr (NCH == 1) {
            c = ChainPar{wbase1, wbase2, a.bias1, a.bias2, a.wscale1, a.wscale2, a.K1, a.dil1, a.K2, a.dil2, 0u, 0u};
        } else {
            const auto &h = a.ch[ci];
            c = ChainPar{reinterpret_cast<const char *>(h.wp1) + wm * (MW * NPW * 1024),
                         reinterpret_cast<const char *>(h.wp2) + wm * (MW * NPW * 1024),
                         h.bias1, h.bias2, h.wscale1, h.wscale2, h.K1, h.dil1, h.K2, h.dil2, (uint32_t)h.xoff, (uint32_t)h.yoff};
        }
        return c;
    };
    static_assert(NCH == 1 || EARLY, "fused chains keep x in registers from the prologue on");
    const uint32_t ylds = NCH > 1 ? lds0 + (uint32_t)a.nchunks * XB : lds0;
    f32x4 xkeep[NCH > 1 ? NW / 2 : 1][2][4], tot[NCH > 1 ? NW / 2 : 1][2][4];
#if SX_PAIR_ALIAS
    ASet f1s[DEPTH + 1];
    ASet(&f2s)[DEPTH + 1] = f1s;
#else
    ASet f1s[DEPTH + 1], f2s[DEPTH + 1];
#endif
#pragma unroll 1
    for (int ci = 0; ci < NCH; ci++) {
    const ChainPar cp = chain_par(ci);
    if constexpr (NCH > 1) {
        if (ci > 0) {
#pragma unroll
            for (int rr = 0; rr < NW / 2; rr++)
#pragma unroll
                for (int j = 0; j < 2; j++)
#pragma unroll
                    for (int q = 0; q < 4; q++) pre[rr][j][q] = xkeep[rr][j][q];
            zero_acc();
        }
    }
    if constexpr (!SHA) load_a(f1s[0], cp.wb1, 0);
    if (ci == 0) {
        asm volatile("s_waitcnt lgkmcnt(0)" ::: "memory");
#if SX_PAIR_PROF
        tp[2] = stamp();
#endif
        __builtin_amdgcn_s_barrier();
#if SX_PAIR_PROF
        tp[3] = stamp();
#endif
    }
    __builtin_amdgcn_sched_barrier(0);
    if constexpr (SHA)
        run_conv_sha(f1s[0], f1s[1], cp.wb1, cp.K1, cp.dil1, lds0 + (uint32_t)(hi * LW + wn * (NW * 32) + l31 + (int)cp.xoff) * 16u,
                     XB, (uint32_t)(2 * LW) * 16u);
    else
        run_conv(f1s, cp.wb1, cp.K1, cp.dil1, lds0 + (uint32_t)(hi * LW + wn * (NW * 32) + l31 + (int)cp.xoff) * 16u, XB,
                 (uint32_t)(2 * LW) * 16u);

#if SX_PAIR_PROF
    tp[4] = stamp();
#endif
    if constexpr (CHAIN && !EARLY) load_pre();

    if constexpr (!SHA) load_a(f2s[0], cp.wb2, 0);
    asm volatile("s_waitcnt lgkmcnt(0)" ::: "memory");
    __builtin_amdgcn_s_barrier();
    __builtin_amdgcn_sched_barrier(0);
    if constexpr (SHA) sha_prefetch(cp.wb2, cp.K2);
    {
        const float wsc = cp.ws1, msl = a.mslope;
        const float *biasp = cp.bias1 ? cp.bias1 : a.zeros;
        const int b_on = cp.bias1 ? 1 : 0;
        const uint32_t YC = a.y_chunk_bytes, LW2 = (uint32_t)a.LW2;
        const int row0 = wm * 32;
        f32x4 bq[4];
        if constexpr (BIAS_LDS) bias_from_lds(0, bq);
        else {
#pragma unroll
            for (int q = 0; q < 4; q++) bq[q] = *reinterpret_cast<const f32x4 *>(biasp + (row0 + 8 * q + 4 * hi) * b_on);
        }
#pragma unroll
        for (int n = 0; n < NW; n++) {
            const int col = (wn * NW + n) * 32 + l31;
            const int t = t1 + col;
            const bool live = t >= 0 && t < TV;
#pragma unroll
            for (int q = 0; q < 4; q++) {
                float o[4];
#pragma unroll
                for (int e = 0; e < 4; e++) {
                    float v = __builtin_fmaf(acc[n][4 * q + e], wsc, bq[q][e]);
                    if constexpr (CHAIN) {
                        if constexpr (NCH > 1) {
                            if (ci == 0) xkeep[n / 2][n % 2][q][e] = pre[n / 2][n % 2][q][e];
                        }
                        v += pre[n / 2][n % 2][q][e];
                        pre[n / 2][n % 2][q][e] = v;
                    }
                    o[e] = live ? fmaxf(v, v * msl) : 0.f;
                }
                unsigned wa[2], wb[2];
                split2h_pair_pk(o[0], o[1], wa[0], wa[1], pk);
                split2h_pair_pk(o[2], o[3], wb[0], wb[1], pk);
                const int g = 4 * wm + q;
                const uint32_t cell = ylds + (uint32_t)(g >> 1) * YC + ((uint32_t)(g & 1) * LW2 + (uint32_t)(col + a.pad2)) * 16u + 8u * hi;
                asm volatile("ds_write_b64 %0, %1" ::"v"(cell), "v"(u32x2{wa[0], wb[0]}) : "memory");
                asm volatile("ds_write_b64 %0, %1" ::"v"(cell + 2u * LW2 * 16u), "v"(u32x2{wa[1], wb[1]}) : "memory");
            }
            asm volatile("" : "+v"(pk));
        }
    }
    zero_acc();
    asm volatile("s_waitcnt lgkmcnt(0)" ::: "memory");
    __builtin_amdgcn_s_barrier();
    __builtin_amdgcn_sched_barrier(0);
#if SX_PAIR_PROF
    tp[5] = stamp();
#endif

    if constexpr (SHA)
        run_conv_sha(f2s[0], f2s[1], cp.wb2, cp.K2, cp.dil2, ylds + (uint32_t)(hi * a.LW2 + wn * (NW * 32) + l31 + (int)cp.yoff) * 16u,
                     a.y_chunk_bytes, (uint32_t)(2 * a.LW2) * 16u);
    else
        run_conv(f2s, cp.wb2, cp.K2, cp.dil2, ylds + (uint32_t)(hi * a.LW2 + wn * (NW * 32) + l31 + (int)cp.yoff) * 16u,
                 a.y_chunk_bytes, (uint32_t)(2 * a.LW2) * 16u);
#if SX_PAIR_PROF
    tp[6] = stamp();
#endif
    if constexpr (!CHAIN && !EARLY) load_pre();

    {
        constexpr int flags = EPI;
        float *rawb = a.out_raw + (int64_t)b * a.C * T;
        const float wsc = cp.ws2, rdiv = a.div;
        const float *biasp = cp.bias2 ? cp.bias2 : a.zeros;
        const int b_on = cp.bias2 ? 1 : 0;
        const int row0 = wm * 32;
        f32x4 bq[4];
        if constexpr (BIAS_LDS) bias_from_lds(1, bq);
        else {
#pragma unroll
            for (int q = 0; q < 4; q++) bq[q] = *reinterpret_cast<const f32x4 *>(biasp + (row0 + 8 * q + 4 * hi) * b_on);
        }
        static_for<NW / 2>([&](auto R) {
            constexpr int rr = decltype(R)::value;
            f32x4 adl[2][4];
            if constexpr ((flags & EPI_ACC) != 0 && !(EARLY && ACC)) {
#pragma unroll
                for (int j = 0; j < 2; j++) {
                    const int t = t1 + (wn * NW + rr * 2 + j) * 32 + l31;
                    const int tl = t < 0 ? 0 : (t < T ? t : T - 1);
#pragma unroll
                    for (int q = 0; q < 4; q++)
                        adl[j][q] = *reinterpret_cast<const f32x4 *>(rawb + ((int64_t)((row0 >> 3) + q) * T + tl) * 8 + 4 * hi);
                }
            }
#pragma unroll
            for (int j = 0; j < 2; j++) {
                const int n = rr * 2 + j;
                const int col = (wn * NW + n) * 32 + l31;
                const int t = t1 + col;
                const bool kept = !(col < a.pad2 || col >= a.pad2 + a.BNo || t >= TV);
                if constexpr (NCH == 1) {
                    if (!kept) continue;
                }
#pragma unroll
                for (int q = 0; q < 4; q++) {
                    f32x4 v;
#pragma unroll
                    for (int e = 0; e < 4; e++) v[e] = __builtin_fmaf(acc[n][4 * q + e], wsc, bq[q][e]);
                    v += pre[rr][j][q];
                    if constexpr (NCH > 1) {
                        if (ci > 0) v += tot[rr][j][q];
                        tot[rr][j][q] = v;
                        if (ci < NCH - 1 || !kept) continue;
                    }
                    if constexpr ((flags & EPI_ACC) != 0) {
                        if constexpr (EARLY && ACC) v += ad[rr][j][q];
                        else v += adl[j][q];
                    }
                    if constexpr ((flags & EPI_DIV) != 0) {
#pragma unroll
                        for (int e = 0; e < 4; e++) v[e] = v[e] / rdiv;
                    }
#if SX_PAIR_ST_SC1
                    {
                        float *sp = rawb + ((int64_t)((row0 >> 3) + q) * T + t) * 8 + 4 * hi;
                        const f32x4 sv = v;
                        asm volatile("global_store_dwordx4 %0, %1, off sc1" ::"v"(sp), "v"(sv) : "memory");
                    }
#else
                    *reinterpret_cast<f32x4 *>(rawb + ((int64_t)((row0 >> 3) + q) * T + t) * 8 + 4 * hi) = v;
#endif
                }
            }
        });
    }
    }
#if SX_PAIR_PROF
    asm volatile("s_waitcnt vmcnt(0)" ::: "memory");
    tp[7] = stamp();
    if (a.prof && tid == 0) {
        for (int i = 0; i < 7; i++) atomicAdd(a.prof + i, tp[i + 1] - tp[i]);
        atomicAdd(a.prof + 7, 1ull);
    }
#endif
    if (a.peak) sx_publish_peak(a.peak, (int)blockIdx.x, pk);
}

template <int MW, int NW, int WM, int WN, int EPI, bool CHAIN, int NCH = 1>
inline hipError_t launch_conv_sx_pair_k(const SxPairArgs &a, dim3 grid, size_t lds, hipStream_t stream) {
    static std::atomic<uint64_t> attr_done{0};
    auto kern = conv_sx_pair_kernel<MW, NW, WM, WN, EPI, CHAIN, NCH>;
    if (hipError_t e = sx_allow_big_lds(reinterpret_cast<const void *>(kern), attr_done); e != hipSuccess) return e;
    if (g_launch_name_on)
        snprintf(g_launch_name, sizeof g_launch_name, "conv_sx_pair_kernel<%d, %d, %d, %d, %d, %s, %d>", MW, NW, WM, WN, EPI,
                 CHAIN ? "true" : "false", NCH);
    kern<<<grid, 256, lds, stream>>>(a);
    return hipGetLastError();
}

inline bool sx_pair_supported(int C, int cfg, int K1, int dil1, int K2, int dil2) {
    if (K1 < 3 || K2 < 3 || dil1 < 1 || dil2 < 1) return false;
    if (!((C == 64 && cfg == 1) || (C == 32 && cfg == 2))) return false;
    const int LW1 = 256 + (K1 - 1) * dil1;
    if (2 * LW1 > kSxRawStageCells) return false;
    const int halo2 = (K2 - 1) * dil2;
    static const int keep_min = [] {
        const char *e = std::getenv("VITSMI_PAIR_MIN_KEEP");
        return e ? std::atoi(e) : 160;
    }();
    if (halo2 % 2 || 256 - halo2 < keep_min) return false;
    static const int keep64 = [] {
        const char *e = std::getenv("VITSMI_PAIR_MIN_KEEP64");
        return e ? std::atoi(e) : 200;
    }();
    if (C == 64 && 256 - halo2 < keep64) return false;
    const size_t lds_y = (size_t)(C / 16) * 4 * (size_t)((256 + halo2 / 2 + 7) / 8 * 8) * 16 + (size_t)(halo2 / 2) * 16;
    const size_t lds_x = (size_t)(C / 16) * 4 * LW1 * 16;
    return (lds_y > lds_x ? lds_y : lds_x) <= kLdsTwoPerCu;
}

hipError_t launch_conv_sx_pair(SxPairArgs a, int cfg, int B, hipStream_t stream, bool chain = false);
hipError_t launch_conv_sx_mrf(SxPairArgs a, int B, hipStream_t stream);
#ifdef VITSMI_IMPL_PAIR
hipError_t launch_conv_sx_pair(SxPairArgs a, int cfg, int B, hipStream_t stream, bool chain) {
    a.LW1 = 256 + (a.K1 - 1) * a.dil1;
    a.x_bytes = (unsigned)((size_t)4 * a.LW1 * 16);
    if (a.dil2 < 1) a.dil2 = 1;
    const int halo2 = (a.K2 - 1) * a.dil2;
    if (a.pad2 * 2 != halo2) return hipErrorInvalidValue;
    a.LW2 = (256 + a.pad2 + 7) / 8 * 8;
    a.y_chunk_bytes = (unsigned)(4 * a.LW2 * 16);
    a.BNo = 256 - halo2;
    a.NT = (a.T + a.BNo - 1) / a.BNo;
    a.B = B;
    a.nchunks = a.C / 16;
    if (a.islope == 0.f) a.islope = 1.f;
    if (a.mslope == 0.f) a.mslope = 1.f;
    if (a.wscale1 == 0.f) a.wscale1 = 1.f;
    if (a.wscale2 == 0.f) a.wscale2 = 1.f;
    if ((long long)a.T * 64 + 64 >= (1ll << 32)) return hipErrorInvalidValue;
    const size_t lds_x = (size_t)a.nchunks * a.x_bytes, lds_y = (size_t)a.nchunks * a.y_chunk_bytes + (size_t)a.pad2 * 16;
    size_t lds = lds_x > lds_y ? lds_x : lds_y;
    if (lds > kLdsTwoPerCu || !sx_pair_supported(a.C, cfg, a.K1, a.dil1, a.K2, a.dil2)) return hipErrorInvalidValue;
    if (cfg != 1 && SX_PAIR_SHARED_A) {
        a.a_ring = (unsigned)((lds + 1023) / 1024 * 1024);
        lds = a.a_ring + 3 * 4096;
    }
    a.bias_off = (unsigned)((lds + 15) / 16 * 16);
    lds = a.bias_off + 1024;
    const long long nb = (long long)a.NT * B;
    if (nb == 0) return hipSuccess;
    a.xgs = a.NT >= (2 << sx_xcd_group_shift()) ? sx_xcd_group_shift() : 0;
    const long long per_round = 8ll << a.xgs;
    const long long wgs = (nb + per_round - 1) / per_round * per_round;
    if (wgs >= (1ll << 31)) return hipErrorInvalidValue;
    dim3 grid((unsigned)wgs, 1, 1);
    const int epi = a.flags & (EPI_ACC | EPI_DIV);
    if ((epi & EPI_DIV) && !(epi & EPI_ACC)) return hipErrorInvalidValue;
#define SX_PAIR_CASES(MW, NW, WM, WN, CH)                                                                        \
    switch (epi) {                                                                                               \
        case 0: return launch_conv_sx_pair_k<MW, NW, WM, WN, 0, CH>(a, grid, lds, stream);                       \
        case EPI_ACC: return launch_conv_sx_pair_k<MW, NW, WM, WN, EPI_ACC, CH>(a, grid, lds, stream);           \
        default: return launch_conv_sx_pair_k<MW, NW, WM, WN, EPI_ACC | EPI_DIV, CH>(a, grid, lds, stream);      \
    }
    if (cfg == 1) {
        if (chain) {
            SX_PAIR_CASES(1, 4, 2, 2, true)
        }
        SX_PAIR_CASES(1, 4, 2, 2, false)
    }
    if (chain) {
        SX_PAIR_CASES(1, 2, 1, 4, true)
    }
    SX_PAIR_CASES(1, 2, 1, 4, false)
#undef SX_PAIR_CASES
}
#endif

struct SxMrfGeom {
    int pad1, pad2, LW1, LW2;
    size_t lds;
};
inline bool sx_mrf_geom(int C, int n, const int *K1, const int *dil1, const int *K2, const int *dil2, SxMrfGeom *g) {
    if (C != 32 || n < 2 || n > 3) return false;
    int p1 = 0, p2 = 0;
    for (int i = 0; i < n; i++) {
        if (K1[i] < 3 || K2[i] < 3 || !(K1[i] & 1) || !(K2[i] & 1) || dil1[i] < 1 || dil2[i] < 1) return false;
        const int a1 = (K1[i] - 1) / 2 * dil1[i], a2 = (K2[i] - 1) / 2 * dil2[i];
        p1 = a1 > p1 ? a1 : p1;
        p2 = a2 > p2 ? a2 : p2;
    }
    const int LW1 = 256 + 2 * p1;
    if (2 * LW1 > kSxRawStageCells) return false;
    if (256 - 2 * p2 < 160) return false;
    const int LW2 = (256 + p2 + 7) / 8 * 8;
    const size_t lds = (size_t)(C / 16) * 4 * LW1 * 16 + (size_t)(C / 16) * 4 * LW2 * 16 + (size_t)p2 * 16;
    if (lds > kLdsTwoPerCu) return false;
    if (g) *g = SxMrfGeom{p1, p2, LW1, LW2, lds};
    return true;
}

#ifdef VITSMI_IMPL_PAIR
hipError_t launch_conv_sx_mrf(SxPairArgs a, int B, hipStream_t stream) {
    int K1[3], d1[3], K2[3], d2[3];
    if (a.nchain < 2 || a.nchain > 3) return hipErrorInvalidValue;
    for (int i = 0; i < a.nchain; i++) {
        K1[i] = a.ch[i].K1;
        d1[i] = a.ch[i].dil1;
        K2[i] = a.ch[i].K2;
        d2[i] = a.ch[i].dil2;
    }
    SxMrfGeom g;
    if (!sx_mrf_geom(a.C, a.nchain, K1, d1, K2, d2, &g)) return hipErrorInvalidValue;
    for (int i = 0; i < a.nchain; i++) {
        a.ch[i].xoff = g.pad1 - (K1[i] - 1) / 2 * d1[i];
        a.ch[i].yoff = g.pad2 - (K2[i] - 1) / 2 * d2[i];
        if (a.ch[i].wscale1 == 0.f) a.ch[i].wscale1 = 1.f;
        if (a.ch[i].wscale2 == 0.f) a.ch[i].wscale2 = 1.f;
    }
    a.pad1 = g.pad1;
    a.pad2 = g.pad2;
    a.LW1 = g.LW1;
    a.x_bytes = (unsigned)((size_t)4 * a.LW1 * 16);
    a.LW2 = g.LW2;
    a.y_chunk_bytes = (unsigned)(4 * a.LW2 * 16);
    a.BNo = 256 - 2 * g.pad2;
    a.NT = (a.T + a.BNo - 1) / a.BNo;
    a.B = B;
    a.nchunks = a.C / 16;
    if (a.islope == 0.f) a.islope = 1.f;
    if (a.mslope == 0.f) a.mslope = 1.f;
    if ((long long)a.T * 64 + 64 >= (1ll << 32)) return hipErrorInvalidValue;
    const long long nb = (long long)a.NT * B;
    if (nb == 0) return hipSuccess;
    a.xgs = a.NT >= (2 << sx_xcd_group_shift()) ? sx_xcd_group_shift() : 0;
    const long long per_round = 8ll << a.xgs;
    const long long wgs = (nb + per_round - 1) / per_round * per_round;
    if (wgs >= (1ll << 31)) return hipErrorInvalidValue;
    dim3 grid((unsigned)wgs, 1, 1);
    a.flags = EPI_DIV;
    if (a.nchain == 2) return launch_conv_sx_pair_k<1, 2, 1, 4, EPI_DIV, true, 2>(a, grid, g.lds, stream);
    return launch_conv_sx_pair_k<1, 2, 1, 4, EPI_DIV, true, 3>(a, grid, g.lds, stream);
}
#endif

}
```

phoonnx_amd/csrc/vitsmi.hip:

```cpp
#include <climits>
#include <hip/hip_runtime.h>

#include <cmath>
#include <cstdarg>
#include <chrono>
#include <cstdio>
#include <cstring>
#include <mutex>
#include <string>
#include <vector>

#include "../../include/vitsmi.h"
#include "conv_geom.hpp"
#include "conv_sx_engine.hip.hpp"
#include "conv_sx_pair.hip.hpp"
#include "conv_sx_pair16.hip.hpp"
#include "attention16.hip.hpp"
#include "conv_sx_small.hip.hpp"
#include "delivery.hip.hpp"
#include "delivery_run.hip.hpp"
#include "fit.hip.hpp"
#include "shape.hip.hpp"
#include "kernels.hip.hpp"
#include "loudness.hip.hpp"
// ... 585 lines not shown
    const int ns = ns_arg ? ns_arg : (env_ns ? env_ns : 2), qt = qt_arg ? qt_arg : (env_qt ? env_qt : 1);
    if (dk == 32) return launch_attention16_t<1, 3, 1>(st, a);
    if (dk == 64) return launch_attention16_t<2, 3, 1>(st, a);
    if (qt == 2) return ns >= 3 ? launch_attention16_t<3, 3, 2>(st, a) : launch_attention16_t<3, 2, 2>(st, a);
    if (ns >= 4) return launch_attention16_t<3, 4, 1>(st, a);
    return ns == 3 ? launch_attention16_t<3, 3, 1>(st, a) : launch_attention16_t<3, 2, 1>(st, a);
}

void launch_durations(hipStream_t st, int B, int T, const float *logw, const int *len, float length_scale, const float *rows,
                      const float *token_rate, float *w_ceil, int *cum, int *y_len) {
    duration_kernel<<<B, 256, 0, st>>>(logw, len, length_scale, rows, token_rate, w_ceil, cum, y_len, T);
}

void launch_fit_weights(hipStream_t st, int B, int T, const float *logw, const int *len, float length_scale, const float *rows,
                        const float *token_rate, float *w) {
    fit_weight_kernel<<<dim3((T + 255) / 256, B), 256, 0, st>>>(logw, len, length_scale, rows, token_rate, w, T);
}

void launch_fit_durations(hipStream_t st, int B, int T, int G, const float *w, const int *len, const int *group, const int64_t *target,
                          const int *mode, float *w_ceil, int *cum, int *y_len, FitResult *res) {
    fit_duration_kernel<<<G, 256, 0, st>>>(w, len, group, target, mode, B, T, w_ceil, cum, y_len, res);
}

void launch_forced_durations(hipStream_t st, int B, int T, const int64_t *dur, const int *len, float *w_ceil, int *cum, int *y_len) {
    forced_duration_kernel<<<B, 256, 0, st>>>(dur, len, w_ceil, cum, y_len, T);
}

void launch_fill_normal_rows(hipStream_t st, int B, int channels, int T, float *out, const uint64_t *seeds, uint32_t stream,
                             const float *rows, int col) {
    fill_normal_rows_kernel<<<dim3((unsigned)(((T + 3) / 4 + 63) / 64), channels, B), 64, 0, st>>>(out, T, seeds, stream, rows, col);
}

void launch_fill_normal(hipStream_t st, float *out, int64_t n, uint64_t seed, uint64_t stream_id) {
    fill_normal_kernel<<<(unsigned)((n / 4 + 256) / 256), 256, 0, st>>>(out, n, seed, stream_id);
}

void launch_expand_prior(hipStream_t st, int B, int C, int T, int F, const float *m_p, const float *logs_p, int64_t bstride,
                         const int *cum, const int *len, const int *y_len, const float *noise, int64_t noise_stride,
                         float noise_scale, const float *rows, const uint64_t *seeds, float *z_p, int Fnoise) {
    expand_prior_strided_kernel<<<dim3((F + 255) / 256, (C + 3) / 4, B), 64, 0, st>>>(m_p, logs_p, bstride, cum, len, y_len, noise,
                                                                                     noise_stride, noise_scale, rows, seeds, z_p, C,
                                                                                     T, F, Fnoise);
}

size_t post_conv_lds(int C, int K) { return ((size_t)C * (256 + K - 1) + (size_t)C * K) * sizeof(float); }
void launch_post_conv(hipStream_t st, int B, int C, int K, int T, const float *x, const float *w, float *out, float slope,
                      const int *vlen, int hop) {
    const size_t lds = post_conv_lds(C, K);
    post_conv_tanh_kernel<<<dim3((T + 255) / 256, B), 256, lds, st>>>(x, w, out, C, K, T, slope, vlen, hop);
}

size_t post_conv_blocked_lds(int C, int K) { return (size_t)C * (256 + K - 1) * sizeof(float); }
void launch_post_conv_blocked(hipStream_t st, int B, int C, int K, int T, const float *x, const float *w, float *out, float slope,
                              const int *vlen, int hop, bool generic = false) {
    const size_t lds = post_conv_blocked_lds(C, K);
    if (K == 7 && !generic)
        post_conv_tanh_blocked_kernel<7><<<dim3((T + 255) / 256, B), 256, lds, st>>>(x, w, out, C, K, T, slope, vlen, hop);
    else
        post_conv_tanh_blocked_kernel<0><<<dim3((T + 255) / 256, B), 256, lds, st>>>(x, w, out, C, K, T, slope, vlen, hop);
}

void conv_sx_planar(Ctx &c, const ConvDesc &d, const uint16_t *x_pl, int T, float *out, uint16_t *out_pl, int flags,
                    SxOpt o = {}) {
    o.row_split = d.Cout;
    o.pl_rows = out_pl ? d.Cout : 0;
    conv_sx(c, d, x_pl, T, out, out_pl, SX_WN_RMW | flags, o);
}

void split_planes(Ctx &c, const float *x, uint16_t *pl, int C, int T, const int *len) {
    sx_split_planes_kernel<<<dim3((T + 255) / 256, C / 8, c.B), 256, 0, c.st>>>(x, (int64_t)C * T, T, len, pl, C, T, 1,
                                                                                range_slots(c.h, true));
    c.note(hipGetLastError());
    c.h->stats.total_launches++;
}

void fused_launch_end(Ctx &c, bool ev, const ConvDesc *const *members, int n, const ConvDesc &rec, int T, double fl, double by) {
    vits_stats &st = c.h->stats;
    if (ev) conv_event_end(c, true, fl, by, rec, T);
    for (int i = 0; i < n; i++) conv_account(c, *members[i], T);
    st.conv_launches -= n - 1;
    st.total_launches -= n - 1;
    st.sx_flops += fl;
    st.sx_bytes += by;
    st.sx_launches++;
}

bool sx_pair_ok(const vits_handle *h, const ConvDesc &c1, const ConvDesc &c2) {
    static const bool off = std::getenv("VITSMI_SX_NO_PAIR") != nullptr;
    return !off && h->gen_nprod == 2 && c1.f16 && c2.f16 && c1.rawin && c2.rawin && c1.cfg == c2.cfg && c1.ups == 1 &&
           c2.ups == 1 && c1.Cin == c1.Cout && c2.Cin == c2.Cout && c1.Cin == c2.Cin && c2.padL * 2 == (c2.K - 1) * c2.dil &&
           sx_pair_supported(c1.Cin, c1.cfg, c1.K, c1.dil, c2.K, c2.dil);
}

void conv_sx_pair(Ctx &c, const ConvDesc &c1, const ConvDesc &c2, const float *x, int T, float *out, int flags, float div,
                  float slope, bool chain = false) {
    SxPairArgs a{};
    a.xr = x;
    a.islope = slope;
    a.mslope = slope;
    a.T = T;
    a.wp1 = reinterpret_cast<const u32x4 *>(c.P(c1.w_off));
    a.wp2 = reinterpret_cast<const u32x4 *>(c.P(c2.w_off));
    a.bias1 = c.P(c1.b_off);
    a.bias2 = c.P(c2.b_off);
    a.wscale1 = c1.wscale;
    a.wscale2 = c2.wscale;
    a.out_raw = out;
    a.zeros = c.P(c.m.zeros_off);
    a.C = c1.Cin;
    a.K1 = c1.K;
    a.dil1 = c1.dil;
    a.pad1 = c1.padL;
    a.K2 = c2.K;
    a.dil2 = c2.dil;
    a.pad2 = c2.padL;
    a.flags = flags & (EPI_ACC | EPI_DIV);
    a.div = div;
    vits_handle *h = c.h;
    a.rag = c.rag_at(T);
    a.peak = range_slots(h, true);
#if SX_PAIR_PROF
    {
        static unsigned long long *rows = nullptr;
        static int idx = 0;
        if (!rows) {
            hipMalloc((void **)&rows, 64 * 8 * sizeof(unsigned long long));
            hipMemset(rows, 0, 64 * 8 * sizeof(unsigned long long));
        }
        if (h->stats.sx_launches == 0 || idx >= 64) idx = 0;
        a.prof = rows + (idx++ % 64) * 8;
        if (std::getenv("VITSMI_PAIR_PROF_DUMP") && idx == 1) {
            unsigned long long hrows[64 * 8];
            hipDeviceSynchronize();
            hipMemcpy(hrows, rows, sizeof hrows, hipMemcpyDeviceToHost);
            for (int r = 0; r < 64; r++)
                if (hrows[r * 8 + 7]) {
                    fprintf(stderr, "pairprof row %d wgs %llu:", r, hrows[r * 8 + 7]);
                    for (int i = 0; i < 7; i++) fprintf(stderr, " %.0f", (double)hrows[r * 8 + i] / (double)hrows[r * 8 + 7]);
                    fprintf(stderr, "\n");
                }
            hipMemset(rows, 0, sizeof hrows);
        }
    }
#endif
    const bool ev = conv_event_begin(c);
    c.note(launch_conv_sx_pair(a, c1.cfg, c.B, c.st, chain));
    const double wf = c.work_frac();
    const double fl = 2.0 * (c1.macs_per_t + c2.macs_per_t) * (double)T * c.B * wf;
    const double by = 4.0 * c.B * ((double)(c1.Cin + c1.Cout) * T + (double)(c2.Cin + c2.Cout) * T) * wf;
    const ConvDesc *const members[] = {&c1, &c2};
    fused_launch_end(c, ev, members, 2, c1, T, fl, by);
}

bool sx_pair16_ok(const vits_handle *h, const ConvDesc &c1, const ConvDesc &c2) {
    static const bool off = [] {
        const char *e = std::getenv("VITSMI_PAIR16");
        return (e && e[0] == '0') || std::getenv("VITSMI_SX_NO_PAIR") != nullptr;
    }();
    if (off || c1.Cin != c1.Cout || c2.Cin != c2.Cout || c1.Cin != c2.Cin || c1.ups != 1 || c2.ups != 1) return false;
    if (c1.padL * 2 != (c1.K - 1) * c1.dil || c2.padL * 2 != (c2.K - 1) * c2.dil) return false;
    const bool h1 = c1.h1 && c2.h1, f3 = c1.f16 && c2.f16 && c1.s16 && c2.s16 && !c1.rawin && !c2.rawin;
    if (!h1 && !f3) return false;
    if (c1.cfg != c2.cfg || c1.cfg != (c1.Cin == 64 ? 1 : 2)) return false;
    (void)h;
    return sx_pair16_plan(c1.Cin, h1 ? 1 : 2, c1.K, c1.dil, c2.K, c2.dil, nullptr) != 0;
}

static SxPair16Args sx_pair16_args(const ConvDesc &c1, const ConvDesc &c2, const float *A, const float *zeros, const uint16_t *x, int T,
                                   float *out_raw, uint16_t *out_pl, int flags, float div, float slope, SxRagged rag, unsigned *peak) {
    SxPair16Args a{};
    const int C = c1.Cin;
    const auto P = [A](int64_t off) { return off >= 0 ? A + off : nullptr; };
    a.xpl = x;
    a.x_bstride = (int64_t)3 * C * T;
    a.islope = a.mslope = a.oslope = slope;
    a.T = T;
    a.wp1 = reinterpret_cast<const u32x4 *>(P(c1.w_off));
    a.wp2 = reinterpret_cast<const u32x4 *>(P(c2.w_off));
    a.bias1 = P(c1.b_off);
    a.bias2 = P(c2.b_off);
    a.wscale1 = c1.wscale;
    a.wscale2 = c2.wscale;
    a.out_raw = out_raw;
    a.raw_bstride = (int64_t)C * T;
    a.out_pl = out_pl;
    a.pl_bstride = (int64_t)3 * C * T;
    a.zeros = zeros;
    a.K1 = c1.K; a.dil1 = c1.dil; a.pad1 = c1.padL;
    a.K2 = c2.K; a.dil2 = c2.dil; a.pad2 = c2.padL;
    a.flags = flags;
    a.div = div;
    a.rag = rag;
    a.peak = peak;
    return a;
}

void conv_sx_pair16(Ctx &c, const ConvDesc &c1, const ConvDesc &c2, const uint16_t *x, int T, float *out_raw, uint16_t *out_pl, int flags,
                    float div, float slope, bool chain) {
    const bool h1 = c1.h1;
    const int C = c1.Cin;
    vits_handle *h = c.h;
    const SxPair16Args a = sx_pair16_args(c1, c2, c.A, c.P(c.m.zeros_off), x, T, out_raw, out_pl, flags, div, slope, c.rag_at(T),
                                          range_slots(h, true));
    const double ebytes = h1 ? 2.0 : 4.0;
    const bool ev = conv_event_begin(c);
    c.note(launch_conv_sx_pair16(a, C, h1 ? 1 : 2, c.B, c.st, chain));
    const double fl = 2.0 * (c1.macs_per_t + c2.macs_per_t) * (double)T * c.B * c.work_frac();
    const double by = ebytes * c.B * ((double)(c1.Cin + c1.Cout) * T + (double)(c2.Cin + c2.Cout) * T) * c.work_frac();
    const ConvDesc *const members[] = {&c1, &c2};
    fused_launch_end(c, ev, members, 2, c1, T, fl, by);
}

bool sx_mrf_ok(const vits_handle *h, const UpStageDesc &stg) {
    const bool off = std::getenv("VITSMI_SX_MRF") == nullptr;
    const int n = (int)stg.rbs.size();
    if (off || n < 2 || n > 3) return false;
    int K1[3], d1[3], K2[3], d2[3];
    for (int j = 0; j < n; j++) {
        const auto &rb = stg.rbs[j];
        if (rb.type1 || rb.n != 2 || !sx_pair_ok(h, rb.c1[0], rb.c1[1]) || rb.c1[0].padL * 2 != (rb.c1[0].K - 1) * rb.c1[0].dil)
            return false;
        K1[j] = rb.c1[0].K;
        d1[j] = rb.c1[0].dil;
        K2[j] = rb.c1[1].K;
        d2[j] = rb.c1[1].dil;
    }
    return sx_mrf_geom(stg.rbs[0].c1[0].Cin, n, K1, d1, K2, d2, nullptr);
}

void conv_sx_mrf(Ctx &c, const UpStageDesc &stg, const float *x, int T, float *out, float slope) {
    const int n = (int)stg.rbs.size();
    SxPairArgs a{};
    a.xr = x;
    a.islope = slope;
    a.mslope = slope;
    a.T = T;
    a.out_raw = out;
    a.zeros = c.P(c.m.zeros_off);
    a.C = stg.rbs[0].c1[0].Cin;
    a.div = (float)n;
    a.nchain = n;
    double macs = 0, bytes = 0;
    const ConvDesc *members[6];
    for (int j = 0; j < n; j++) {
        const ConvDesc &c1 = stg.rbs[j].c1[0], &c2 = stg.rbs[j].c1[1];
        members[2 * j] = &c1;
        members[2 * j + 1] = &c2;
        auto &ch = a.ch[j];
        ch.wp1 = reinterpret_cast<const u32x4 *>(c.P(c1.w_off));
        ch.wp2 = reinterpret_cast<const u32x4 *>(c.P(c2.w_off));
        ch.bias1 = c.P(c1.b_off);
        ch.bias2 = c.P(c2.b_off);
        ch.wscale1 = c1.wscale;
        ch.wscale2 = c2.wscale;
        ch.K1 = c1.K;
        ch.dil1 = c1.dil;
        ch.K2 = c2.K;
        ch.dil2 = c2.dil;
        macs += c1.macs_per_t + c2.macs_per_t;
        bytes += 4.0 * ((double)(c1.Cin + c1.Cout) + (double)(c2.Cin + c2.Cout));
    }
    vits_handle *h = c.h;
    a.rag = c.rag_at(T);
    a.peak = range_slots(h, true);
    macs *= c.work_frac();
    bytes *= c.work_frac();
    const bool ev = conv_event_begin(c);
    c.note(launch_conv_sx_mrf(a, c.B, c.st));
    fused_launch_end(c, ev, members, 2 * n, stg.rbs[n - 1].c1[0], T, 2.0 * macs * (double)T * c.B, bytes * T * c.B);
}

void *pinned_get(vits_handle *h, size_t bytes) {
    PinnedPool &p = h->pin;
    if (!p.busy) {
        if (bytes > p.cap) {
            if (p.base) hipHostFree(p.base);
            p.base = nullptr;
            p.cap = 0;
            size_t want = bytes + bytes / 4 + 4096;
            if (hipHostMalloc((void **)&p.base, want) != hipSuccess) return nullptr;
            p.cap = want;
        }
        p.busy = true;
        return p.base;
    }
    void *q = nullptr;
    return hipHostMalloc(&q, bytes) == hipSuccess ? q : nullptr;
}

void pinned_put(vits_handle *h, void *q) {
    if (!q) return;
    if (h && q == h->pin.base) h->pin.busy = false;
    else hipHostFree(q);
}

enum LnForm : int { LN_FORM_TILE16 = 0, LN_FORM_TILE32 = 1, LN_FORM_COLUMN = 2 };
void launch_layernorm(hipStream_t st, int form, int B, int C, int T, const float *in, float *out, const float *gamma,
                      const float *beta, const int *len, int flags, uint16_t *planes, unsigned *peak) {
    if (form == LN_FORM_TILE16 && planes)
        ln_tile_kernel<0, true, 16><<<dim3((T + 15) / 16, B), 256, 0, st>>>(in, out, gamma, beta, len, C, T, flags, nullptr, nullptr, 1, 1,
                                                                              planes, peak);
    else if (form == LN_FORM_TILE32 && planes)
        ln_tile_kernel<0, true><<<dim3((T + 31) / 32, B), 256, 0, st>>>(in, out, gamma, beta, len, C, T, flags, nullptr, nullptr, 1, 1,
                                                                          planes, peak);
    else if (form == LN_FORM_TILE16)
        ln_tile_kernel<0, false, 16><<<dim3((T + 15) / 16, B), 256, 0, st>>>(in, out, gamma, beta, len, C, T, flags, nullptr, nullptr, 1, 1);
// ... 530 lines not shown
void run_generator_planes(vits_handle *h, Ctx &c, const float *z, int64_t z_bstride, int z_cstride, const int *ylen, int B,
                          int F, const float *dec_cond, const GenBufs &gb) {
    const Model &m = h->model;
    hipStream_t st = h->stream;
    uint16_t *const *stage_in = gb.stage_in, *y_pl = gb.y_pl, *const *raa = gb.raa, *tmp_pl = gb.tmp_pl;
    float *xs_raw = gb.xs_raw;
    rag_begin(h, c, ylen, B, F);
    const float S = 0.1f;
    const int nst = (int)m.ups.size();
    SxOpt act;
    act.oslope2 = S;
    sx_split_planes_kernel<<<dim3((F + 255) / 256, m.C / 8, B), 256, 0, st>>>(z, z_bstride, z_cstride, ylen, tmp_pl, m.C, F,
                                                                              m.gen_h1 ? 2 : 1, range_slots(h, true));
    c.note(hipGetLastError());
    h->stats.total_launches++;
    SxOpt pre = act;
    pre.bias_b = dec_cond;
    pre.bias_b_stride = m.C0;
    conv_sx(c, m.conv_pre, tmp_pl, F, nullptr, stage_in[0], 0, pre);
    const uint16_t *xa = stage_in[0];
    int T = F;
    for (int si = 0; si < nst; si++) {
        const auto &stg = m.ups[si];
        rag_margin(c, m.gen_rf_stage[si]);
        conv_sx(c, stg.up, xa, T, nullptr, y_pl, 0, act);
        T *= stg.u;
        uint16_t *xs_pl = stage_in[(si + 1) & 1];
        const int nk = (int)stg.rbs.size();
        const bool last_stage = si == nst - 1;
        for (int j = 0; j < nk; j++) {
            const auto &rbk = stg.rbs[j];
            auto step_out = [&](int q) {
                StepOut w{EPI_RES, nullptr, raa[q & 1]};
                if (q == rbk.n - 1) {
                    w.flags |= mrf_flags(j, nk);
                    w.raw = xs_raw;
                    w.pl = nullptr;
                    if (j == nk - 1 && !last_stage) {
                        w.pl = xs_pl;
                        if (nk > 1) w.flags |= SX_NO_RAW_STORE;
                        else w.raw = nullptr;
                    }
                }
                return w;
            };
            auto p16_flags = [](const StepOut &w) {
                return (w.flags & (EPI_ACC | EPI_DIV)) | (w.raw && !(w.flags & SX_NO_RAW_STORE) ? P16_HAS_RAW : 0) | (w.pl ? P16_HAS_PL : 0);
            };
            const uint16_t *cur = y_pl;
            for (int q = 0; q < rbk.n; q++) {
                StepOut w = step_out(q);
                SxOpt res = act;
                res.div = (float)nk;
                res.res_pl = cur;
                res.res_slope = S;
                if (rbk.type1) {
                    if (sx_pair16_ok(h, rbk.c1[q], rbk.c2[q]))
                        conv_sx_pair16(c, rbk.c1[q], rbk.c2[q], cur, T, w.raw, w.pl, p16_flags(w), (float)nk, S, false);
                    else {
                        conv_sx(c, rbk.c1[q], cur, T, nullptr, tmp_pl, 0, act);
                        conv_sx(c, rbk.c2[q], tmp_pl, T, w.raw, w.pl, w.flags, res);
                    }
                } else if (q + 1 < rbk.n && sx_pair16_ok(h, rbk.c1[q], rbk.c1[q + 1])) {
                    w = step_out(++q);
                    conv_sx_pair16(c, rbk.c1[q - 1], rbk.c1[q], cur, T, w.raw, w.pl, p16_flags(w), (float)nk, S, true);
                } else
                    conv_sx(c, rbk.c1[q], cur, T, w.raw, w.pl, w.flags, res);
                cur = w.pl;
            }
        }
        xa = xs_pl;
    }
    conv_post_sx(h, c, xs_raw, ylen, B, T, F, gb.out);
}

bool res_planes_on() {
    const char *e = std::getenv("VITSMI_F16X3_RES");
    return e ? std::string(e) != "raw" : true;
}

void run_generator_sx(vits_handle *h, Ctx &c, const float *z, int64_t z_bstride, int z_cstride, const int *ylen, int B,
                      int F, const float *dec_cond, const GenBufs &gb) {
    const Model &m = h->model;
    hipStream_t st = h->stream;
    uint16_t *const *stage_in = gb.stage_in, *y_pl = gb.y_pl, *const *raa = gb.raa, *tmp_pl = gb.tmp_pl;
    float *y_raw = gb.y_raw, *const *ra = gb.ra, *xs_raw = gb.xs_raw;
    float *tmp_raw = reinterpret_cast<float *>(tmp_pl), *xin_raw = reinterpret_cast<float *>(stage_in[0]);
    rag_begin(h, c, ylen, B, F);
    const float S = 0.1f;
    const int nst = (int)m.ups.size();
    SxOpt lrelu;
    lrelu.oslope2 = S;
    lrelu.islope = S;
    const void *zin;
    if (sx_raw_format(m.C)) {
        sx_block_kernel<<<dim3((F + 255) / 256, m.C / 8, B), 256, 0, st>>>(z, z_bstride, z_cstride, ylen, tmp_raw, m.C, F,
                                                                           range_slots(h, m.gen_f16));
        zin = tmp_raw;
    } else {
        sx_split_planes_kernel<<<dim3((F + 255) / 256, m.C / 8, B), 256, 0, st>>>(z, z_bstride, z_cstride, ylen, tmp_pl, m.C, F,
                                                                                  m.gen_f16 ? 1 : 0, range_slots(h, m.gen_f16));
        zin = tmp_pl;
    }
    c.note(hipGetLastError());
    h->stats.total_launches++;
    SxOpt pre;
    pre.bias_b = dec_cond;
    pre.bias_b_stride = m.C0;
    const void *xa;
    if (sx_raw_format(m.C0)) {
        conv_sx(c, m.conv_pre, zin, F, xin_raw, nullptr, 0, pre);
        xa = xin_raw;
    } else {
        pre.oslope2 = S;
        conv_sx(c, m.conv_pre, zin, F, nullptr, stage_in[0], 0, pre);
        xa = stage_in[0];
    }
    int T = F;
    for (int si = 0; si < nst; si++) {
        const auto &stg = m.ups[si];
        rag_margin(c, m.gen_rf_stage[si]);
        const bool fr = sx_raw_format(stg.C);
        SxOpt act;
        if (fr) act.islope = S;
        else act.oslope2 = S;
        bool rpl = !fr && h->gen_nprod == 2 && res_planes_on() && stg.up.s16;
        for (const auto &rbk : stg.rbs)
            for (int q = 0; q < rbk.n && rpl; q++) rpl = rbk.c1[q].s16 && rbk.c1[q].f16 && (!rbk.type1 || (rbk.c2[q].s16 && rbk.c2[q].f16));
        conv_sx(c, stg.up, xa, T, rpl ? nullptr : y_raw, fr ? nullptr : y_pl, 0, lrelu);
        T *= stg.u;
        uint16_t *xs_pl = stage_in[(si + 1) & 1];
        const int nk = (int)stg.rbs.size();
        const bool last_stage = si == nst - 1;
        if (fr && sx_mrf_ok(h, stg)) {
            conv_sx_mrf(c, stg, y_raw, T, xs_raw, S);
            xa = xs_raw;
            continue;
        }
        for (int j = 0; j < nk; j++) {
            const auto &rbk = stg.rbs[j];
            auto step_out = [&](int q) {
                StepOut w{EPI_RES, rpl ? nullptr : ra[q & 1], fr ? nullptr : raa[q & 1]};
                if (q == rbk.n - 1) {
                    w.flags |= mrf_flags(j, nk);
                    w.raw = xs_raw;
                    w.pl = nullptr;
                    if (j == nk - 1 && !last_stage && !fr) {
                        w.pl = xs_pl;
                        w.flags |= SX_NO_RAW_STORE;
                    }
                }
                return w;
            };
            const float *cur = y_raw;
            const uint16_t *cura = y_pl;
            for (int q = 0; q < rbk.n; q++) {
                StepOut w = step_out(q);
                if (rbk.type1 && fr && sx_pair_ok(h, rbk.c1[q], rbk.c2[q])) {
                    conv_sx_pair(c, rbk.c1[q], rbk.c2[q], cur, T, w.raw, w.flags, (float)nk, S);
                } else if (!rbk.type1 && fr && q + 1 < rbk.n && sx_pair_ok(h, rbk.c1[q], rbk.c1[q + 1])) {
                    w = step_out(++q);
                    conv_sx_pair(c, rbk.c1[q - 1], rbk.c1[q], cur, T, w.raw, w.flags, (float)nk, S, true);
                } else {
                    const void *in = fr ? static_cast<const void *>(cur) : static_cast<const void *>(cura);
                    SxOpt res = rbk.type1 || rpl ? act : lrelu;
                    res.div = (float)nk;
                    if (rpl) {
                        res.res_pl = cura;
                        res.res_slope = S;
                    } else
                        res.res = cur;
                    if (rbk.type1) {
                        conv_sx(c, rbk.c1[q], in, T, fr ? tmp_raw : nullptr, fr ? nullptr : tmp_pl, 0, act);
                        conv_sx(c, rbk.c2[q], tmp_pl, T, w.raw, w.pl, w.flags, res);
                    } else
                        conv_sx(c, rbk.c1[q], in, T, w.raw, w.pl, w.flags, res);
                }
                cur = w.raw;
                cura = w.pl;
            }
        }
        xa = (fr || last_stage) ? static_cast<const void *>(xs_raw) : static_cast<const void *>(xs_pl);
    }
    conv_post_sx(h, c, xs_raw, ylen, B, T, F, gb.out);
}

void run_generator_f32(vits_handle *h, Ctx &c, const float *z, int64_t z_bstride, int z_cstride, const int *ylen, int B,
                       int F, const float *dec_cond, const GenBufs &gb) {
    const Model &m = h->model;
    hipStream_t st = h->stream;
    float *const *reg = gb.reg;
    const float S = 0.1f;
    const int nst = (int)m.ups.size();
    ConvOpt gen;
    gen.slope = 1.f;
    ConvOpt mid = gen;
    mid.oslope = S;
    float *xa = reg[0];
    const int Fp = (F + 3) & ~3;
    ConvOpt pre = gen;
    pre.len = ylen;
    pre.bias_b = dec_cond;
    pre.bias_b_stride = m.C0;
    pre.oslope = S;
    pre.x_cstride = z_cstride;
    pre.out_cstride = Fp;
    conv(c, m.conv_pre, z, z_bstride, F, xa, (int64_t)m.C0 * Fp, ylen ? PRO_MASK : 0, pre);
    int T = F, Cc = m.C0, xs_idx = 0;
    int in_pitch = Fp;
    for (int si = 0; si < nst; si++) {
        const auto &stg = m.ups[si];
        float *y = reg[2], *ya = reg[3];
        const int To = T * stg.u;
        ConvOpt up = gen;
        up.out2 = ya;
        up.oslope2 = S;
        up.x_cstride = in_pitch;
        conv(c, stg.up, xa, (int64_t)Cc * in_pitch, T, y, (int64_t)stg.C * To, 0, up);
        in_pitch = To;
        T = To;
        Cc = stg.C;
        const int64_t sCT = (int64_t)Cc * T;
        xs_idx ^= 1;
        float *xs = reg[xs_idx];
        float *ra[2] = {reg[4], reg[6]}, *raa[2] = {reg[5], reg[7]}, *tmp = reg[8];
        const int nk = (int)stg.rbs.size();
        const float out_slope = si == nst - 1 ? 0.01f : S;
        for (int j = 0; j < nk; j++) {
            const auto &rbk = stg.rbs[j];
            const float *cur = y, *cura = ya;
            for (int q = 0; q < rbk.n; q++) {
                const bool last = q == rbk.n - 1;
                float *dst = last ? xs : ra[q & 1];
                const int fl = EPI_RES | (last ? mrf_flags(j, nk) : 0);
                ConvOpt res = gen;
                res.res = cur;
                res.res_bstride = sCT;
                res.div = (float)nk;
                res.oslope = last && j == nk - 1 ? out_slope : 1.f;
                res.out2 = last ? nullptr : raa[q & 1];
                res.oslope2 = S;
                if (rbk.type1) {
                    conv(c, rbk.c1[q], cura, sCT, T, tmp, sCT, 0, mid);
                    conv(c, rbk.c2[q], tmp, sCT, T, dst, sCT, fl, res);
                } else
                    conv(c, rbk.c1[q], cura, sCT, T, dst, sCT, fl, res);
                cur = dst;
                cura = res.out2;
            }
        }
        xa = xs;
    }
    h->S = T;
    h->d_out = gb.out;
    launch_post_conv(st, B, m.post_cin, m.post_k, T, xa, c.P(m.post_w), h->d_out, 1.0f, tail_len(h, ylen), T / F);
    conv_post_account(h, c, B, T);
}

int run_generator(vits_handle *h, Ctx &c, const float *z, int64_t z_bstride, int z_cstride, const int *ylen, int B,
                  int F, const float *dec_cond, const GenBufs &gb) {
    const Model &m = h->model;
    h->cur_stage = 3;
    stage_mark(h, 3);
    if (!m.gen_sx) run_generator_f32(h, c, z, z_bstride, z_cstride, ylen, B, F, dec_cond, gb);
    else if (m.gen_planes) run_generator_planes(h, c, z, z_bstride, z_cstride, ylen, B, F, dec_cond, gb);
    else run_generator_sx(h, c, z, z_bstride, z_cstride, ylen, B, F, dec_cond, gb);
    c.rag = SxRagged{nullptr, 0, 0};
    stage_mark(h, 4);
    return 0;
}

__global__ void chunk_len_kernel(const int *ylen, int *out, int B, int lo, int n) {
    const int b = blockIdx.x * blockDim.x + threadIdx.x;
    if (b < B) {
        const int v = ylen ? ylen[b] - lo : n;
        out[b] = v < 0 ? 0 : (v > n ? n : v);
    }
}


int resample_count(vits_handle *h, int64_t S_in, int &S_out) {
    const ResamplePlan &p = h->rs.plan;
    const int64_t so = p.count(S_in);
    S_out = (int)so;
    if (so <= INT_MAX) return 0;
    return fail(h, VITS_E_ARG, "%lld samples at %d Hz are %lld samples at %d Hz: more than a row admits (%d)", (long long)S_in, p.fi,
                (long long)so, p.fo, INT_MAX);
}

int resample_carve(vits_handle *h, int B, int64_t S_in, ResampleBufs &rb, int &S_out) {
    if (int rc = resample_count(h, S_in, S_out)) return rc;
    return slab_carve(h, h->io, "staging", [&](Carver &cv) { rb = carve_resample(cv, B, S_out, (int)h->rs.plan.K); });
}

int resample_run(vits_handle *h, const int *ylen, int B) {
    const ResamplePlan &p = h->rs.plan;
    const int S = h->S;
    ResampleBufs rb;
    int S_out = 0;
    if (int rc = resample_carve(h, B, S, rb, S_out)) return rc;
    hipStream_t st = h->stream;
    resample_counts_kernel<<<(B + 63) / 64, 64, 0, st>>>(ylen, h->model.hop, S, p.L, p.M, rb.n_in, rb.n_out, B);
    ResampleArgs a = resample_args(h->rs);
    a.x = h->d_out;
    a.x_pitch = S;
    a.x_n = S;
// ... 2873 lines not shown
    unsigned *dpk = D.fill<unsigned>((size_t)kSxPeakSlots * kSxPeakStride);
    TCHECK(D.err);
    const dim3 grid((T + 255) / 256, C / 8, B);
    sx_split_planes_kernel<<<grid, 256>>>(dx, (int64_t)CT, T, nullptr, dxp, C, T, mode);
    sx_block_kernel<<<grid, 256>>>(dimg, (int64_t)CT, T, nullptr, draw, C, T);
    sx_split_planes_kernel<<<grid, 256>>>(dsen, (int64_t)CT, T, nullptr, dop, C, T, mode);
    TCHECK(hipGetLastError());
    TCHECK(hipMemcpy(draw + n, graw.data(), G * 4, hipMemcpyHostToDevice));
    TCHECK(hipMemcpy(dop + n * 3, gpl.data(), G * 2, hipMemcpyHostToDevice));
    const int kflags = ((flags & VITS_P16_EPI_ACC) ? EPI_ACC : 0) | ((flags & VITS_P16_EPI_DIV) ? EPI_DIV : 0) |
                       ((flags & VITS_P16_EPI_RAW) ? P16_HAS_RAW : 0) | ((flags & VITS_P16_EPI_PLANES) ? P16_HAS_PL : 0);
    const SxRagged rag = dlen ? SxRagged{dlen, p->rag_add, p->rag_mul} : SxRagged{nullptr, 0, 0};
    SxPair16Args a = sx_pair16_args(d1, d2, dA, dA, dxp, T, draw, dop, kflags, p->div == 0.f ? 1.f : p->div, slope, rag, dpk);
    SxPair16Tile tile{};
    auto go = [&] { return launch_conv_sx_pair16(a, C, npl, B, nullptr, chain, &tile); };
    const bool name_was_on = g_launch_name_on;
    g_launch_name_on = true;
    g_launch_name[0] = 0;
    const hipError_t le = go();
    g_launch_name_on = name_was_on;
    if (le != hipSuccess) return fail(nullptr, VITS_E_DEVICE, "pair16 epilogue hook: launch_conv_sx_pair16: %s", hipGetErrorString(le));
    TCHECK(hipDeviceSynchronize());
    std::snprintf(p->kernel, sizeof p->kernel, "%s", g_launch_name);
    p->BN = tile.BN;
    p->BNo = tile.BNo;
    p->ovl = tile.ovl ? 1 : 0;
    if (p->out) {
        sx_unblock_kernel<<<grid, 256>>>(draw, nullptr, dout, C, T, mode);
        TCHECK(hipGetLastError());
        TCHECK(hipDeviceSynchronize());
        TCHECK(download(p->out, dout, n));
    }
    if (p->planes_out) {
        sx_unblock_kernel<<<grid, 256>>>(nullptr, dop, dout, C, T, mode);
        TCHECK(hipGetLastError());
        TCHECK(hipDeviceSynchronize());
        TCHECK(download(p->planes_out, dout, n));
    }
    if (p->x_seen) {
        sx_unblock_kernel<<<grid, 256>>>(nullptr, dxp, dout, C, T, mode);
        TCHECK(hipGetLastError());
        TCHECK(hipDeviceSynchronize());
        TCHECK(download(p->x_seen, dout, n));
        const float un = 1.f / slope;
        for (size_t i = 0; i < n; i++)
            if (p->x_seen[i] < 0.f) p->x_seen[i] *= un;
    }
    {
        std::vector<float> gr(G);
        std::vector<uint16_t> hp(n * 3 + G);
        TCHECK(download(gr.data(), draw + n, G));
        TCHECK(download(hp.data(), dop, hp.size()));
        bool ok = std::memcmp(gr.data(), graw.data(), G * 4) == 0 && std::memcmp(hp.data() + n * 3, gpl.data(), G * 2) == 0;
        for (int b = 0; b < B && ok; b++)
            for (size_t i = (size_t)npl * CT; i < 3 * CT && ok; i++) ok = hp[(size_t)b * 3 * CT + i] == 0;
        p->guard_ok = ok ? 1 : 0;
    }
    {
        std::vector<unsigned> slots((size_t)kSxPeakSlots * kSxPeakStride);
        TCHECK(download(slots.data(), dpk, slots.size()));
        unsigned top = 0;
        for (int s = 0; s < kSxPeakSlots; s++) top = std::max(top, slots[(size_t)s * kSxPeakStride]);
        std::memcpy(&p->peak, &top, 4);
    }
#if P16_PROF
    {
        const size_t nwg = 1 << 17;
        unsigned long long *dprof = D.fill<unsigned long long>(nwg * 8);
        TCHECK(D.err);
        a.prof = dprof;
        TCHECK(go());
        TCHECK(hipDeviceSynchronize());
        std::vector<unsigned long long> hp(nwg * 8);
        TCHECK(download(hp.data(), dprof, nwg * 8));
        double sum[7] = {0, 0, 0, 0, 0, 0, 0};
        unsigned long long nt = 0, wgs = 0;
        for (size_t w = 0; w < nwg; w++)
            if (hp[w * 8 + 7]) {
                wgs++;
                nt += hp[w * 8 + 7];
                for (int i = 0; i < 7; i++) sum[i] += (double)hp[w * 8 + i];
            }
        fprintf(stderr, "p16prof C %d npl %d K %d wgs %llu tiles %llu | x wait %.0f  barrier %.0f  phase1 %.0f  hand-over %.0f  phase2 %.0f  epilogue %.0f  drain %.0f (cycles per TILE)\n",
                C, npl, K, wgs, nt, sum[0] / nt, sum[1] / nt, sum[2] / nt, sum[3] / nt, sum[4] / nt, sum[5] / nt, sum[6] / nt);
        a.prof = nullptr;
    }
#endif
    if (p->ms_out) TCHECK(time_launches(10, go, p->ms_out));
    return VITS_OK;
}

int vits_test_conv_pair_sx(int device_id, const float *x, int B, int C, int T, const float *w1, const float *b1,
                           const float *w2, const float *b2, int K, int dil1, int dil2, int chain, float slope, float *out,
                           float *ms_out) {
    if (int rc = test_dev(device_id)) return rc;
    const int kern = (chain >> 1) & 3;
    const bool from_plane = (chain & 8) != 0;
    chain &= 1;
    if (kern) {
        vits_test_conv_pair16_epi_args e{};
        e.B = B, e.C = C, e.T = T, e.K = K, e.dil1 = dil1, e.dil2 = dil2, e.chain = chain;
        e.precision = kern == 2 ? VITS_SX_F16 : VITS_SX_F16X3;
        e.flags = from_plane ? VITS_P16_EPI_PLANES : VITS_P16_EPI_RAW;
        e.slope = slope, e.div = 1.f, e.sentinel = 0.f;
        e.x = x, e.w1 = w1, e.b1 = b1, e.w2 = w2, e.b2 = b2;
        (from_plane ? e.planes_out : e.out) = out;
        e.ms_out = ms_out;
        return vits_test_conv_pair16_epi(device_id, &e);
    }
    ConvDesc d1, d2;
    std::vector<float> arena;
    const TestPack o = sx_test_pack(SxPack::F16X2);
    std::string e = pack_test_conv(w1, b1, C, C, K, dil1, dil1 * (K - 1) / 2, 3, &d1, &arena, o);
    if (e.empty()) e = pack_test_conv(w2, b2, C, C, K, dil2, dil2 * (K - 1) / 2, 3, &d2, &arena, o);
    if (!e.empty()) return fail(nullptr, VITS_E_ARG, "%s", e.c_str());
    const size_t n = (size_t)B * C * T;
    DevBufs D;
    if (!d1.rawin || !d2.rawin || d1.cfg != d2.cfg || !sx_pair_supported(C, d1.cfg, d1.K, d1.dil, d2.K, d2.dil))
        return fail(nullptr, VITS_E_ARG, "this conv pair cannot run fused (C %d, kernel %d, dilation %d)", C, K, dil1);
    float *dA = D.up(arena.data(), arena.size());
    float *dx = D.up(x, n, 16);
    float *dxr = D.alloc<float>(n, 16);
    float *draw = D.fill<float>(n, 0, 16);
    float *dout = D.alloc<float>(n, 16);
    TCHECK(D.err);
    sx_block_kernel<<<dim3((T + 255) / 256, C / 8, B), 256>>>(dx, (int64_t)C * T, T, nullptr, dxr, C, T);
    SxPairArgs a{};
    a.xr = dxr;
    a.islope = a.mslope = slope;
    a.T = T;
    a.wp1 = reinterpret_cast<const u32x4 *>(dA + d1.w_off);
    a.wp2 = reinterpret_cast<const u32x4 *>(dA + d2.w_off);
    a.bias1 = d1.b_off >= 0 ? dA + d1.b_off : nullptr;
    a.bias2 = d2.b_off >= 0 ? dA + d2.b_off : nullptr;
    a.wscale1 = d1.wscale;
    a.wscale2 = d2.wscale;
    a.out_raw = draw;
    a.zeros = dA;
    a.C = C;
    a.K1 = d1.K; a.dil1 = d1.dil; a.pad1 = d1.padL;
    a.K2 = d2.K; a.dil2 = d2.dil; a.pad2 = d2.padL;
    a.div = 1.f;
    auto go = [&] { return launch_conv_sx_pair(a, d1.cfg, B, nullptr, chain != 0); };
    TCHECK(go());
    TCHECK(hipDeviceSynchronize());
    if (ms_out) TCHECK(time_launches(10, go, ms_out));
    sx_unblock_kernel<<<dim3((T + 255) / 256, C / 8, B), 256>>>(draw, nullptr, dout, C, T, 1);
    TCHECK(hipGetLastError());
    TCHECK(hipDeviceSynchronize());
    TCHECK(download(out, dout, n));
    return VITS_OK;
}

int vits_bench_conv1d_sx(int device_id, int B, int Cin, int Cout, int T, int K, int dil, int dbg, int iters,
                         float *ms_out) {
    if (int rc = test_dev(device_id)) return rc;
    std::vector<float> w((size_t)Cout * Cin * K), x((size_t)B * Cin * T);
    bench_fill(w, x);
    ConvDesc d;
    std::vector<float> arena;
    TestPack o = sx_test_pack((dbg & 64) ? SxPack::F16X1 : ((dbg & 128) ? SxPack::F16X2 : SxPack::BF16X3));
    o.sx.no_s16 = (dbg & (1 | 2 | 16 | 256)) != 0;
    std::string e = pack_test_conv(w.data(), nullptr, Cin, Cout, K, dil, dil * (K - 1) / 2, 3, &d, &arena, o);
    if (!e.empty()) return fail(nullptr, VITS_E_ARG, "%s", e.c_str());
    const size_t nx = x.size(), no = (size_t)B * Cout * T;
    DevBufs D;
    float *dA = D.up(arena.data(), arena.size());
    float *dx = D.up(x.data(), nx);
    uint16_t *dxp = D.alloc<uint16_t>(nx * 3);
    float *draw = D.alloc<float>(no);
    float *dres = D.fill<float>(no);
    uint16_t *dop = D.alloc<uint16_t>(no * 3);
    unsigned long long *dprof = (dbg & 16) ? D.fill<unsigned long long>(8) : nullptr;
    TCHECK(D.err);
    sx_split_planes_kernel<<<dim3((T + 255) / 256, Cin / 8, B), 256>>>(dx, (int64_t)Cin * T, T, nullptr, dxp, Cin, T,
                                                                       d.h1 ? 2 : (d.f16 ? 1 : 0));
    SxArgs a = sx_args(d, dA, dA, T);
    a.xp = reinterpret_cast<const u32x4 *>(dxp);
    a.out_pl = dop;
    a.oslope2 = 0.1f;
    a.flags = ((dbg & 1) ? DBG_NO_DMA : 0) | ((dbg & 2) ? DBG_NO_EPI : 0);
    if (dbg & 8) {
        a.flags |= EPI_RES;
        if (d.h1) {
            a.res_pl = reinterpret_cast<const uint16_t *>(dres);
            a.res_unslope = 10.f;
        } else {
            a.res = dres;
            a.out_raw = draw;
        }
    }
    if (d.rawin) {
        a.xr = dx;
        a.islope = 0.1f;
        a.out_pl = nullptr;
        a.out_raw = draw;
    }
    a.prof = dprof;
    auto go = [&] { return launch_conv_sx(a, d.cfg, B, nullptr, d.rawin, d.h1 ? 1 : (d.f16 ? 2 : 6)); };
    for (int i = 0; i < 2; i++) TCHECK(go());
    TCHECK(hipDeviceSynchronize());
    if (dprof) TCHECK(hipMemset(dprof, 0, 64));
    float ms = 0.f;
    TCHECK(time_launches(iters, go, &ms));
    if (ms_out) {
        ms_out[0] = ms;
        ms_out[1] = (float)d.cfg;
        ms_out[2] = 0.f;
        if (dprof) {
            unsigned long long hp[8];
            TCHECK(download(hp, dprof, 8));
            for (int i = 0; i < 5; i++) ms_out[3 + i] = hp[5] ? (float)((double)hp[i] / (double)hp[5]) : 0.f;
            ms_out[2] = hp[7] ? (float)((double)hp[6] / (double)hp[7] * 0.1) : 0.f;
        }
    }
    return VITS_OK;
}

int vits_test_attention(int device_id, const float *qkv, int B, int C, int T, int n_heads, const float *rel_k,
                        const float *rel_v, int window, const int64_t *lens, float *out) {
    if (int rc = test_dev(device_id)) return rc;
    if (window > 4 || C % n_heads) return fail(nullptr, VITS_E_ARG, "bad attention test arguments");
    int dk = C / n_heads;
    if (dk > kAttMaxHeadWidth) return fail(nullptr, VITS_E_ARG, "attention head width %d > %d is unsupported", dk, kAttMaxHeadWidth);
    size_t nq = (size_t)B * 3 * C * T, no = (size_t)B * C * T, nr = (size_t)(2 * window + 1) * dk;
    std::vector<int> l32(B);
    for (int b = 0; b < B; b++) l32[b] = (int)lens[b];
    DevBufs D;
    float *dq = D.up(qkv, nq);
    float *dout = D.alloc<float>(no);
    float *drk = D.up(rel_k, nr);
    float *drv = D.up(rel_v, nr);
    int *dlen = D.up(l32.data(), (size_t)B);
    TCHECK(D.err);
    launch_attention(nullptr, B, T, n_heads, dk, window, dq, dout, drk, drv, dlen, C);
    TCHECK(hipGetLastError());
    TCHECK(hipDeviceSynchronize());
    TCHECK(download(out, dout, no));
    return VITS_OK;
}

int vits_test_attention16(int device_id, const float *qkv, int B, int C, int T, int n_heads, const float *rel_k,
                          const float *rel_v, int window, const int64_t *lens, float *out, uint16_t *out_planes, int kernel,
                          int reps, float *ms_out) {
    if (int rc = test_dev(device_id)) return rc;
    if (window > 4 || C % n_heads || C % 8) return fail(nullptr, VITS_E_ARG, "bad attention test arguments");
    int dk = C / n_heads;
    if (kernel == 1 && !(dk % 32 == 0 && dk <= 96)) return fail(nullptr, VITS_E_ARG, "attention16 needs a head width of 32, 64 or 96");
    if (dk > kAttMaxHeadWidth) return fail(nullptr, VITS_E_ARG, "attention head width %d > %d is unsupported", dk, kAttMaxHeadWidth);
    size_t nq = (size_t)B * 3 * C * T, no = (size_t)B * C * T, nr = (size_t)(2 * window + 1) * dk;
    std::vector<int> l32(B);
    for (int b = 0; b < B; b++) l32[b] = (int)lens[b];
    DevBufs D;
    float *dq = D.up(qkv, nq);
    uint16_t *dqp = D.alloc<uint16_t>(nq * 3);
    uint16_t *dop = D.fill<uint16_t>(no * 3, 0xff);
    unsigned *dpk = D.fill<unsigned>((size_t)kSxPeakSlots * kSxPeakStride);
    float *dout = D.fill<float>(no, 0xff);
    float *drk = D.up(rel_k, nr);
    float *drv = D.up(rel_v, nr);
    int *dlen = D.up(l32.data(), (size_t)B);
    unsigned long long *dprof = nullptr;
    const int prof_wgs = ((n_heads * B + 7) / 8) * 8 * ((T + 63) / 64);
#if ATT16_PROF
    dprof = D.fill<unsigned long long>((size_t)prof_wgs * 4);
#endif
    TCHECK(D.err);
    sx_split_planes_kernel<<<dim3((T + 255) / 256, 3 * C / 8, B), 256>>>(dq, (int64_t)3 * C * T, T, nullptr, dqp, 3 * C, T, 1, dpk);
    auto go = [&] {
        if (kernel == 1) (void)launch_attention16(nullptr, B, T, n_heads, dk, window, dqp, dout, dop, drk, drv, dlen, C, dpk, dprof);
        else launch_attention(nullptr, B, T, n_heads, dk, window, dq, dout, drk, drv, dlen, C, dk % 8 == 0 ? dop : nullptr, dpk);
        return hipSuccess;
    };
    go();
    TCHECK(hipGetLastError());
    TCHECK(hipDeviceSynchronize());
    if (reps > 0 && ms_out) TCHECK(time_launches(reps, go, ms_out));
    if (dprof && kernel == 1) {
        std::vector<unsigned long long> hp((size_t)prof_wgs * 4);
        TCHECK(download(hp.data(), dprof, hp.size()));
        double d[3] = {0, 0, 0};
        unsigned long long t0 = ~0ull, t1 = 0;
        int n = 0;
        for (int w = 0; w < prof_wgs; w++) {
            if (!hp[w * 4 + 3]) continue;
            for (int k = 0; k < 3; k++) d[k] += (double)(hp[w * 4 + k + 1] - hp[w * 4 + k]);
            t0 = hp[w * 4] < t0 ? hp[w * 4] : t0;
            t1 = hp[w * 4 + 3] > t1 ? hp[w * 4 + 3] : t1;
            n++;
        }
        if (n) std::fprintf(stderr, "att16 stamps B=%d T=%d: %d workgroups; cycles prologue %.0f loop %.0f epilogue %.0f; first start -> last end %llu\n",
                            B, T, n, d[0] / n, d[1] / n, d[2] / n, t1 - t0);
    }
    TCHECK(download(out, dout, no));
    if (out_planes) TCHECK(download(out_planes, dop, no * 3));
    return VITS_OK;
}

int vits_test_attention_form(int device_id, vits_test_attention_form_args *p) {
    if (int rc = test_dev(device_id)) return rc;
    if (!p) return fail(nullptr, VITS_E_ARG, "no attention test arguments");
    const int B = p->B, C = p->C, T = p->T, n_heads = p->n_heads, window = p->window;
    if (B <= 0 || C <= 0 || T <= 0 || n_heads <= 0 || window < 0 || !p->rel_k || !p->rel_v || !p->lens)
        return fail(nullptr, VITS_E_ARG, "bad attention test arguments");
    if (window > 4) return fail(nullptr, VITS_E_ARG, "attention window %d > 4 is unsupported", window);
    if (C % n_heads) return fail(nullptr, VITS_E_ARG, "%d channels do not divide into %d heads", C, n_heads);
// ... 953 lines not shown
```

phoonnx_amd/session.py:

```python
import contextlib
import ctypes as C
import dataclasses
import time
from collections import namedtuple
from dataclasses import dataclass
from typing import Dict, List, Optional, Sequence

import numpy as np

from . import _ffi


class SessionError(RuntimeError):
    """Raised for every failure of the engine (onnxruntime raises its own
    InvalidArgument/RuntimeException at voice.py:374; callers there do not catch either)."""


class RangeError(SessionError):
    """VITS_E_RANGE: the f16x3 generator arithmetic met an activation beyond the range of its fp16 operand planes
    (|x| > 65504) or a non-finite value.  The engine reports this instead of returning clamped audio; `MiSession`
    (range_fallback=True, the default) then reopens the voice with the bf16x6 arithmetic (fp32 range) and repeats the
    call, so user code only sees this when the fallback is switched off or impossible (borrowed weight arena)."""


# ... 2232 lines not shown
    a.old_out, a.old_out2, a.sentinel = _ffi.ptr(old_out), _ffi.ptr(old_out2), CONV_EPI_SENTINEL
    a.out, a.out2, a.pl_rows, a.planes_out = _ffi.ptr(out), _ffi.ptr(o2), pl_rows, _ffi.ptr(pl)
    rc = lib.vits_test_conv1d_epi(device_id, C.byref(a))
    if rc != 0:
        raise SessionError(_ffi.last_error(None))
    return {"out": out, "out2": o2, "planes": pl, "kernel": a.kernel.decode(), "cfg": a.cfg_used, "ck": a.ck_used}


SX_EPI_FLAGS = {"res": 1, "acc": 2, "div": 4, "no_raw_store": 8}
SX_PRECISIONS = {"bf16x6": 0, "f16x3": 1, "f16": 2}


def test_conv1d_sx_epi(x, w, bias=None, flags=(), precision="f16x3", dil=1, pad_l=None, stride=1, force16=False, no_s16=False,
                       min_cfg=0, run_cfg=-1, res=None, res_is_x=False, res_planes=False, res_slope=1.0, old_out=None,
                       bias_b=None, div=1.0, oslope=1.0, oslope2=1.0, islope=1.0, raw=True, planes=False, lens=None,
                       rag_add=0, rag_mul=1, sentinel=CONV_EPI_SENTINEL, device_id=0):
    lib = _ffi.load()
    f32 = lambda a: None if a is None else np.ascontiguousarray(a, np.float32)
    x, w, bias, bias_b, res, old_out = (f32(a) for a in (x, w, bias, bias_b, res, old_out))
    B, Cin, T = x.shape
    Cout, K = (w.shape[1] if stride > 1 else w.shape[0]), w.shape[2]
    To = T * stride
    ln = None if lens is None else np.ascontiguousarray(lens, np.int64)
    for name, arr, shape in (("w", w, (Cin, Cout, K) if stride > 1 else (Cout, Cin, K)), ("bias", bias, (Cout,)),
                             ("res", res, (B, Cout, To)), ("old_out", old_out, (B, Cout, To)), ("lens", ln, (B,))):
        if arr is not None and arr.shape != shape:
            raise ValueError(f"{name} has shape {arr.shape}, the launch needs {shape}")
    if bias_b is not None and (bias_b.ndim != 2 or bias_b.shape[0] != B):
        raise ValueError(f"bias_b has shape {bias_b.shape}, the launch needs ({B}, stride)")
    out = np.empty((B, Cout, To), np.float32) if raw else None
    pl = np.empty((B, Cout, To), np.float32) if planes else None
    seen = np.empty((B, Cout, To), np.float32) if (res_planes and res is not None) else None
    a = _ffi.VitsTestConvSxEpiArgs()
    a.B, a.Cin, a.T, a.Cout, a.K, a.dil, a.stride = B, Cin, T, Cout, K, dil, stride
    a.pad_l = dil * (K - 1) // 2 if pad_l is None else pad_l
    a.precision, a.force16, a.no_s16, a.min_cfg, a.run_cfg = SX_PRECISIONS[precision], int(force16), int(no_s16), min_cfg, run_cfg
    a.flags = sum(SX_EPI_FLAGS[f] for f in flags)
    a.x, a.w, a.bias, a.res, a.old_out, a.bias_b, a.lens = (_ffi.ptr(v) for v in (x, w, bias, res, old_out, bias_b, ln))
    a.res_is_x, a.res_planes, a.res_slope = int(res_is_x), int(res_planes), res_slope
    a.bias_b_stride = 0 if bias_b is None else bias_b.shape[1]
    a.div, a.oslope, a.oslope2, a.islope = div, oslope, oslope2, islope
    a.rag_add, a.rag_mul, a.sentinel = rag_add, rag_mul, sentinel
    a.out, a.planes_out, a.res_seen = _ffi.ptr(out), _ffi.ptr(pl), _ffi.ptr(seen)
    rc = lib.vits_test_conv1d_sx_epi(device_id, C.byref(a))
    if rc != 0:
        raise SessionError(_ffi.last_error(None))
    return {"out": out, "planes": pl, "res_seen": seen, "kernel": a.kernel.decode(), "pack_cfg": a.pack_cfg, "run_cfg": a.run_cfg_used,
            "rawin": bool(a.rawin), "s16": bool(a.s16), "ck": a.ck, "peak": float(a.peak)}


def test_wn_gate(a, blocked=False, device_id=0):
    lib = _ffi.load()
    a = np.ascontiguousarray(a, np.float32)
    B, C2, T = a.shape
    if C2 % 2:
        raise ValueError("a holds the tanh rows and as many sigmoid rows")
    out = np.empty((B, C2 // 2, T), np.float32)
    rc = lib.vits_test_wn_gate(device_id, _ffi.ptr(a), B, C2 // 2, T, 1 if blocked else 0, _ffi.ptr(out))
    if rc != 0:
        raise SessionError(_ffi.last_error(None))
    return out


def test_cond_matvec(emb_g, sid, W, bias=None, device_id=0):
    lib = _ffi.load()
    emb_g = np.ascontiguousarray(emb_g, np.float32)
    W = np.ascontiguousarray(W, np.float32)
    b = None if bias is None else np.ascontiguousarray(bias, np.float32)
    sid = np.ascontiguousarray(sid, np.int64)
    if emb_g.ndim != 2 or W.ndim != 2 or W.shape[1] != emb_g.shape[1] or sid.ndim != 1 or (b is not None and b.shape != W.shape[:1]):
        raise ValueError("emb_g [n_speakers, gin], W [rows, gin], bias [rows], sid [B]")
    out = np.empty((len(sid), W.shape[0]), np.float32)
    rc = lib.vits_test_cond_matvec(device_id, _ffi.ptr(emb_g), emb_g.shape[0], emb_g.shape[1], _ffi.ptr(sid), len(sid),
                                   _ffi.ptr(W), _ffi.ptr(b), W.shape[0], _ffi.ptr(out))
    if rc != 0:
        raise SessionError(_ffi.last_error(None))
    return out


def test_conv1d_sx_gate(x, w, bias, g, dil=1, small=False, planes=False, device_id=0):
    lib = _ffi.load()
    x = np.ascontiguousarray(x, np.float32)
    B, Cin, T = x.shape
    C2, _, K = w.shape
    H = C2 // 2
    perm = np.concatenate([np.concatenate([np.arange(p, p + 32), H + np.arange(p, p + 32)]) for p in range(0, H, 32)])
    wp = np.ascontiguousarray(np.asarray(w, np.float32)[perm])
    bp = np.ascontiguousarray(np.asarray(bias, np.float32)[perm])
    gg = np.ascontiguousarray(g, np.float32)
    out = np.empty((B, H, T), np.float32)
    rc = lib.vits_test_conv1d_sx_gate(device_id, _ffi.ptr(x), B, Cin, T, _ffi.ptr(wp), _ffi.ptr(bp), _ffi.ptr(gg), C2, K, dil,
                                      (1 if small else 0) | (2 if planes else 0), _ffi.ptr(out))
    if rc != 0:
        raise SessionError(_ffi.last_error(None))
    return out


def test_conv_pair_sx(x, w1, b1, w2, b2, dil1=1, dil2=1, chain=False, slope=0.1, device_id=0, timed=False, kernel="pair",
                      from_plane=False):
    lib = _ffi.load()
    x = np.ascontiguousarray(x, np.float32)
    w1 = np.ascontiguousarray(w1, np.float32)
    w2 = np.ascontiguousarray(w2, np.float32)
    B, Cc, T = x.shape
    K = w1.shape[2]
    if w1.shape != (Cc, Cc, K) or w2.shape != (Cc, Cc, K):
        raise ValueError("both convs are C -> C with the same kernel size")
    b1 = None if b1 is None else np.ascontiguousarray(b1, np.float32)
    b2 = None if b2 is None else np.ascontiguousarray(b2, np.float32)
    out = np.empty_like(x)
    ms = C.c_float(0.0)
    rc = lib.vits_test_conv_pair_sx(device_id, _ffi.ptr(x), B, Cc, T, _ffi.ptr(w1), _ffi.ptr(b1), _ffi.ptr(w2),
                                    _ffi.ptr(b2), K, dil1, dil2,
                                    (1 if chain else 0) | ({"pair": 0, "pair16": 1, "pair16_f16": 2}[kernel] << 1) | (8 if from_plane else 0),
                                    float(slope), _ffi.ptr(out),
                                    C.byref(ms) if timed else None)
    if rc != 0:
        raise SessionError(_ffi.last_error(None))
    return (out, float(ms.value)) if timed else out


P16_EPI_FLAGS = {"acc": 1, "div": 2, "raw": 4, "planes": 8}


def test_conv_pair16_epi(x, w1, b1, w2, b2, flags=("raw",), dil1=1, dil2=1, chain=False, slope=0.1, precision="f16x3", div=1.0,
                         old_out=None, lens=None, rag_add=0, rag_mul=1, x_tail=None, sentinel=CONV_EPI_SENTINEL, device_id=0):
    lib = _ffi.load()
    f32 = lambda a: None if a is None else np.ascontiguousarray(a, np.float32)
    x, w1, b1, w2, b2, old_out, x_tail = (f32(a) for a in (x, w1, b1, w2, b2, old_out, x_tail))
    B, Cc, T = x.shape
    K = w1.shape[2]
    ln = None if lens is None else np.ascontiguousarray(lens, np.int64)
    for name, arr, shape in (("w1", w1, (Cc, Cc, K)), ("w2", w2, (Cc, Cc, K)), ("b1", b1, (Cc,)), ("b2", b2, (Cc,)),
                             ("old_out", old_out, (B, Cc, T)), ("x_tail", x_tail, (B, Cc, T)), ("lens", ln, (B,))):
        if arr is not None and arr.shape != shape:
            raise ValueError(f"{name} has shape {arr.shape}, the launch needs {shape}")
    out = np.empty((B, Cc, T), np.float32)
    pl = np.empty((B, Cc, T), np.float32) if "planes" in flags else None
    seen = np.empty((B, Cc, T), np.float32)
    a = _ffi.VitsTestConvPair16EpiArgs()
    a.B, a.C, a.T, a.K, a.dil1, a.dil2, a.chain = B, Cc, T, K, dil1, dil2, int(bool(chain))
    a.precision, a.flags = SX_PRECISIONS[precision], sum(P16_EPI_FLAGS[f] for f in flags)
    a.slope, a.div, a.sentinel = slope, div, sentinel
    a.x, a.w1, a.b1, a.w2, a.b2, a.old_out, a.x_tail, a.lens = (_ffi.ptr(v) for v in (x, w1, b1, w2, b2, old_out, x_tail, ln))
    a.rag_add, a.rag_mul = rag_add, rag_mul
    a.out, a.planes_out, a.x_seen = _ffi.ptr(out), _ffi.ptr(pl), _ffi.ptr(seen)
    rc = lib.vits_test_conv_pair16_epi(device_id, C.byref(a))
    if rc != 0:
        raise SessionError(_ffi.last_error(None))
    return {"out": out, "planes": pl, "x_seen": seen, "kernel": a.kernel.decode(), "BN": a.BN, "BNo": a.BNo, "ovl": bool(a.ovl),
            "peak": float(a.peak), "guard_ok": bool(a.guard_ok)}


def bench_conv1d_sx(B, Cin, Cout, T, K, dil=1, dbg=0, iters=20, device_id=0):
    lib = _ffi.load()
    res = np.zeros(8, np.float32)
    rc = lib.vits_bench_conv1d_sx(device_id, B, Cin, Cout, T, K, dil, dbg, iters,
                                  res.ctypes.data_as(_ffi.C.POINTER(_ffi.C.c_float)))
    if rc != 0:
        raise SessionError(_ffi.last_error(None))
    if dbg & 16:
        return float(res[0]), int(res[1]), [float(v) for v in res[3:8]] + [float(res[2])]
    return float(res[0]), int(res[1])


def test_conv_transpose1d(x, w, bias, stride, device_id=0, sx=False):
    lib = _ffi.load()
    x = np.ascontiguousarray(x, np.float32)
    w = np.ascontiguousarray(w, np.float32)
    B, Cin, T = x.shape
    _, Cout, K = w.shape
    b = None if bias is None else np.ascontiguousarray(bias, np.float32)
    out = np.empty((B, Cout, T * stride), np.float32)
    fn = lib.vits_test_conv_transpose1d_sx if sx else lib.vits_test_conv_transpose1d
    rc = fn(device_id, _ffi.ptr(x), B, Cin, T, _ffi.ptr(w), _ffi.ptr(b), Cout, K, -stride if sx == "f16" else stride,
            _ffi.ptr(out))
    if rc != 0:
        raise SessionError(_ffi.last_error(None))
    return out


def test_attention16(qkv, n_heads, rel_k, rel_v, lens, device_id=0, kernel=1, planes=False, reps=0):
    lib = _ffi.load()
    qkv = np.ascontiguousarray(qkv, np.float32)
    B, C3, T = qkv.shape
    Cc = C3 // 3
    rel_k = np.ascontiguousarray(rel_k, np.float32)
    rel_v = np.ascontiguousarray(rel_v, np.float32)
    window = (rel_k.shape[0] - 1) // 2
    lens = np.ascontiguousarray(lens, np.int64)
    out = np.empty((B, Cc, T), np.float32)
    opl = np.empty((B, 3, Cc // 8, T, 8), np.uint16) if planes else None
    ms = (C.c_float * 1)()
    rc = lib.vits_test_attention16(device_id, _ffi.ptr(qkv), B, Cc, T, n_heads, _ffi.ptr(rel_k), _ffi.ptr(rel_v), window,
                                   _ffi.ptr(lens), _ffi.ptr(out), _ffi.ptr(opl) if planes else None, int(kernel), int(reps), ms)
    if rc != 0:
        raise SessionError(_ffi.last_error(None))
    res = (out,)
    if planes:
        res += (opl,)
    if reps > 0:
        res += (float(ms[0]),)
    return res[0] if len(res) == 1 else res


def test_attention_form(qkv, n_heads, rel_k, rel_v, lens, kernel=16, want_out=True, want_planes=True, ns=0, qt=0, kh=0,
                        qkv_planes=None, device_id=0):
    lib = _ffi.load()
    qkv = np.ascontiguousarray(qkv, np.float32)
    B, C3, T = qkv.shape
    Cc = C3 // 3
    rel_k = np.ascontiguousarray(rel_k, np.float32)
    rel_v = np.ascontiguousarray(rel_v, np.float32)
    window = (rel_k.shape[0] - 1) // 2
    lens = np.ascontiguousarray(lens, np.int64)
    if C3 != 3 * Cc or n_heads <= 0 or Cc % n_heads or lens.shape != (B,):
        raise ValueError(f"q|k|v {qkv.shape} with {n_heads} heads and lens {lens.shape}")
    dk = Cc // n_heads
    if rel_k.shape != (2 * window + 1, dk) or rel_v.shape != rel_k.shape:
        raise ValueError(f"relative embeddings {rel_k.shape} / {rel_v.shape}, head width {dk}")
    qp = None
    if qkv_planes is not None:
        qp = np.ascontiguousarray(qkv_planes, np.uint16)
        if C3 % 8 or qp.shape != (B, 3, C3 // 8, T, 8):
            raise ValueError(f"q|k|v planes {qp.shape}, the launch needs {(B, 3, C3 // 8, T, 8)}")
    out = np.empty((B, Cc, T), np.float32)
    opl = np.empty((B, 3, Cc // 8, T, 8), np.uint16) if Cc % 8 == 0 else None
    a = _ffi.VitsTestAttentionFormArgs()
    a.kernel, a.qkv, a.qkv_planes = int(kernel), _ffi.ptr(qkv), _ffi.ptr(qp)
    a.B, a.C, a.T, a.n_heads, a.window = B, Cc, T, n_heads, window
    a.rel_k, a.rel_v, a.lens = _ffi.ptr(rel_k), _ffi.ptr(rel_v), _ffi.ptr(lens)
    a.want_out, a.want_planes, a.ns, a.qt, a.kh = int(bool(want_out)), int(bool(want_planes)), int(ns), int(qt), int(kh)
    a.out, a.out_planes = _ffi.ptr(out), _ffi.ptr(opl)
    rc = lib.vits_test_attention_form(device_id, C.byref(a))
    if rc != 0:
        raise SessionError(_ffi.last_error(None))
    return {"out": out, "planes": opl, "peak": float(a.peak), "kernel": a.kernel_name.decode()}


def test_attention(qkv, n_heads, rel_k, rel_v, lens, device_id=0):
    lib = _ffi.load()
    qkv = np.ascontiguousarray(qkv, np.float32)
    B, C3, T = qkv.shape
    Cc = C3 // 3
    rel_k = np.ascontiguousarray(rel_k, np.float32)
    rel_v = np.ascontiguousarray(rel_v, np.float32)
    window = (rel_k.shape[0] - 1) // 2
    lens = np.ascontiguousarray(lens, np.int64)
    out = np.empty((B, Cc, T), np.float32)
    rc = lib.vits_test_attention(device_id, _ffi.ptr(qkv), B, Cc, T, n_heads, _ffi.ptr(rel_k), _ffi.ptr(rel_v), window,
                                 _ffi.ptr(lens), _ffi.ptr(out))
    if rc != 0:
        raise SessionError(_ffi.last_error(None))
    return out


def _resample_test_args(x, lens, in_rate, out_rate):
    x = np.ascontiguousarray(x, np.float32)
    lens = np.ascontiguousarray(lens, np.int64)
    if x.ndim != 2 or lens.shape != (x.shape[0],):
        raise SessionError(f"x must be [B, S] and lens [B], got {x.shape} / {lens.shape}")
    L, M, _ = resample_plan(in_rate, out_rate)
    return x, lens, L, M


def test_resample(x, lens, in_rate, out_rate, device_id=0):
    x, lens, L, M = _resample_test_args(x, lens, in_rate, out_rate)
    B, S = x.shape
    counts = -(-np.clip(lens, 0, S) * L // M)
    y = np.full((B, max(1, int(counts.max()))), np.nan, np.float32)
    rc = _ffi.load().vits_test_resample(device_id, _ffi.ptr(x), _ffi.ptr(lens), B, S, int(in_rate), int(out_rate), _ffi.ptr(y),
                                        y.shape[1])
    if rc != 0:
        raise SessionError(f"vits_test_resample failed [{rc}]: {_ffi.last_error(None)}")
    return y, counts


def test_resample_rows(x, lens, in_rate, out_rates, device_id=0):
    x = np.ascontiguousarray(x, np.float32)
    lens = np.ascontiguousarray(lens, np.int64)
    rates = np.asarray([int(r or 0) for r in out_rates], np.int32)
    if x.ndim != 2 or lens.shape != (x.shape[0],) or rates.shape != lens.shape:
        raise SessionError(f"x must be [B, S], lens and out_rates [B], got {x.shape} / {lens.shape} / {rates.shape}")
    B, S = x.shape
    cap = -(-S * max(int(rates.max()), int(in_rate)) // max(int(in_rate), 1)) + 1
    buf = np.full(B * cap, np.nan, np.float32)
    counts = np.zeros(B, np.int64)
    rc = _ffi.load().vits_test_resample_rows(device_id, _ffi.ptr(x), _ffi.ptr(lens), B, S, int(in_rate), _ffi.ptr(rates), _ffi.ptr(buf),
                                             buf.size, _ffi.ptr(counts))
    if rc != 0:
        raise SessionError(f"vits_test_resample_rows failed [{rc}]: {_ffi.last_error(None)}")
    S_out = int(counts.max())
    if S_out == 0:
        return np.zeros((B, 1), np.float32), counts
    return buf[:B * S_out].reshape(B, S_out).copy(), counts


def warp_token(semitones):
    step, c, Kh = C.c_int64(), C.c_int64(), C.c_int32()
    rc = _ffi.load().vits_warp_token(float(semitones), C.byref(step), C.byref(c), C.byref(Kh))
    if rc != 0:
        raise SessionError(f"vits_warp_token failed [{rc}]: {_ffi.last_error(None)}")
    return step.value, c.value, Kh.value


def warp_plan(durations, semitones, hop):
# ... 585 lines not shown
```

Measured before the change: 142.1 million.

## Fuse all ResBlock1 conv-pair steps into one launch with overlapping halos

Adds a STEPS variant of the split-precision conv-pair kernel that runs two or three ResBlock1 steps back to back inside one workgroup. The residual stays in registers and each step's leaky-ReLU output is written back into the LDS input tile, so the intermediate tensors never go to global memory. The output tile shrinks by the summed receptive-field halo, which means more tiles and redundant halo compute in exchange for fewer launches and less global traffic. The generator path uses the fused launch whenever sx_steps_ok allows it, and a test hook is added.

```diff
diff --git a/include/vitsmi.h b/include/vitsmi.h
--- a/include/vitsmi.h
+++ b/include/vitsmi.h
@@ -478,6 +478,23 @@
     int guard_ok;
 } vits_test_conv_pair16_epi_args;
 int vits_test_conv_pair16_epi(int device_id, vits_test_conv_pair16_epi_args *a);
+typedef struct {
+    int B, C, T, K, n;
+    int dil1[3], dil2[3];
+    int flags;
+    float slope, div, sentinel;
+    const float *x;
+    const float *w1[3], *b1[3], *w2[3], *b2[3];
+    const float *old_out;
+    const int64_t *lens;
+    int rag_add, rag_mul;
+    float *out;
+    float *ms_out;
+    char kernel[128];
+    int BNo;
+    float peak;
+} vits_test_conv_pair_steps_args;
+int vits_test_conv_pair_steps(int device_id, vits_test_conv_pair_steps_args *a);
 int vits_test_attention(int device_id, const float *qkv, int B, int C, int T, int n_heads, const float *rel_k,
                         const float *rel_v, int window, const int64_t *lens, float *out);
 int vits_test_attention16(int device_id, const float *qkv, int B, int C, int T, int n_heads, const float *rel_k,
diff --git a/phoonnx_amd/_ffi.py b/phoonnx_amd/_ffi.py
--- a/phoonnx_amd/_ffi.py
+++ b/phoonnx_amd/_ffi.py
@@ -63,6 +63,14 @@
                [("rag_add", C.c_int), ("rag_mul", C.c_int)] + \
                [(n, C.c_void_p) for n in ("out", "planes_out", "x_seen", "ms_out")] + [("kernel", C.c_char * 128)] + \
                [(n, C.c_int) for n in ("BN", "BNo", "ovl")] + [("peak", C.c_float), ("guard_ok", C.c_int)]
+
+
+class VitsTestConvPairStepsArgs(C.Structure):
+    _fields_ = [(n, C.c_int) for n in ("B", "C", "T", "K", "n")] + [("dil1", C.c_int * 3), ("dil2", C.c_int * 3), ("flags", C.c_int)] + \
+               [(n, C.c_float) for n in ("slope", "div", "sentinel")] + [("x", C.c_void_p)] + \
+               [(n, C.c_void_p * 3) for n in ("w1", "b1", "w2", "b2")] + [("old_out", C.c_void_p), ("lens", C.c_void_p)] + \
+               [("rag_add", C.c_int), ("rag_mul", C.c_int), ("out", C.c_void_p), ("ms_out", C.c_void_p), ("kernel", C.c_char * 128),
+                ("BNo", C.c_int), ("peak", C.c_float)]
 
 
 class VitsTestAttentionFormArgs(C.Structure):
@@ -205,7 +213,7 @@
     "vits_test_stream_pack_trimmed",
     "vits_test_layernorm", "vits_test_dds", "vits_test_cf_pre", "vits_test_rqs_inverse", "vits_test_ea_logw",
     "vits_test_conv1d_epi", "vits_test_wn_gate", "vits_test_cond_matvec", "vits_test_conv1d_sx_epi",
-    "vits_test_conv_pair16_epi", "vits_test_attention_form",
+    "vits_test_conv_pair16_epi", "vits_test_attention_form", "vits_test_conv_pair_steps",
 ]
 
 
@@ -411,6 +419,7 @@
     lib.vits_test_conv1d_sx_epi.argtypes = [C.c_int, C.POINTER(VitsTestConvSxEpiArgs)]
     lib.vits_test_conv_pair16_epi.argtypes = [C.c_int, C.POINTER(VitsTestConvPair16EpiArgs)]
     lib.vits_test_attention_form.argtypes = [C.c_int, C.POINTER(VitsTestAttentionFormArgs)]
+    lib.vits_test_conv_pair_steps.argtypes = [C.c_int, C.POINTER(VitsTestConvPairStepsArgs)]
     lib.vits_test_wn_gate.argtypes = [C.c_int, vp, C.c_int, C.c_int, C.c_int, C.c_int, vp]
     lib.vits_test_cond_matvec.argtypes = [C.c_int, vp, C.c_int, C.c_int, vp, C.c_int, vp, vp, C.c_int, vp]
     lib.vits_test_conv_pair_sx.argtypes = [C.c_int, vp, C.c_int, C.c_int, C.c_int, vp, vp, vp, vp, C.c_int, C.c_int,
diff --git a/phoonnx_amd/csrc/conv_sx_pair.hip.hpp b/phoonnx_amd/csrc/conv_sx_pair.hip.hpp
--- a/phoonnx_amd/csrc/conv_sx_pair.hip.hpp
+++ b/phoonnx_amd/csrc/conv_sx_pair.hip.hpp
@@ -31,8 +31,10 @@
         float wscale1, wscale2;
         int K1, dil1, K2, dil2;
         int xoff, yoff;
+        int ylo, xlo;
     } ch[3];
     int nchain;
+    int koff;
     unsigned a_ring;
     unsigned bias_off;
     unsigned long long *prof;
@@ -73,9 +75,10 @@
 #ifndef SX_PAIR_ONE_READ32
 #define SX_PAIR_ONE_READ32 1
 #endif
-template <int MW, int NW, int WM, int WN, int EPI, bool CHAIN, int NCH = 1>
+template <int MW, int NW, int WM, int WN, int EPI, bool CHAIN, int NCH = 1, bool STEPS = false>
 __global__ __launch_bounds__(256, (NW == 2 && !SX_PAIR_EARLY_ACC && NCH == 1) ? SX_PAIR_WGS32 : 2) void conv_sx_pair_kernel(SxPairArgs a) {
     constexpr int BN = NW * WN * 32, NH = NW / 2;
+    static_assert(!STEPS || (!CHAIN && NCH == 1), "fused steps: ResBlock1 steps, one receptive field");
     static_assert(NCH == 1 || (CHAIN && NW == 2 && (EPI & EPI_ACC) == 0), "fused chains: 32 channels, no external running sum");
     constexpr bool ONE_READ = NW == 4 ? SX_PAIR_ONE_READ64 != 0 : SX_PAIR_ONE_READ32 != 0;
     constexpr bool EARLY = ONE_READ || (NW == 2 && SX_PAIR_EARLY32);
@@ -83,6 +86,7 @@
     static_assert(DEPTH >= 2 && DEPTH <= 6, "wait_a covers up to five younger sets");
     constexpr bool ACC = (EPI & EPI_ACC) != 0 && SX_PAIR_EARLY_ACC;
     static_assert(!(ONE_READ && ACC), "the running sum is not pulled into the single-read prologue");
+    static_assert(!STEPS || ONE_READ, "fused steps: the residual lives in `pre` from the prologue on");
     static_assert(WM * WN == 4 && MW == 1 && BN == 256, "one block row per wave, 256 columns");
     constexpr int NPW = 2, STEPBYTES = WM * MW * NPW * 1024;
     constexpr int MAXCH = WM * 2;
@@ -95,7 +99,9 @@
     const int tile_nb = __builtin_amdgcn_readfirstlane(sx_xcd_tile(wg_seq, wg_xcd, a.xgs));
     if (tile_nb >= a.NT * a.B) return;
     const int b = tile_nb / a.NT, t0 = (tile_nb - b * a.NT) * a.BNo;
-    const int t1 = t0 - a.pad2;
+    const int koff = STEPS ? a.koff : a.pad2;
+    const int nst = STEPS ? __builtin_amdgcn_readfirstlane(a.nchain) : NCH;
+    const int t1 = t0 - koff;
     const int T = a.T, LW = a.LW1;
     const int TV = __builtin_amdgcn_readfirstlane(sx_valid_cols(a.rag, b, T));
     if (t0 >= TV) return;
@@ -155,20 +161,26 @@
                             reinterpret_cast<float *>(lds_sx + a.a_ring + (unsigned)((g * 2 + sub) * 2048 + pl * 1024)));
             }
     constexpr bool BIAS_LDS = NCH == 1;
+    uint32_t bias_slot = 0;
     if constexpr (BIAS_LDS) {
-        if (wave == 0) {
+        if (STEPS ? wave < nst : wave == 0) {
             constexpr int CC = WM * 32;
             const int k = lane - (lane >= CC / 4 ? CC / 4 : 0);
-            const float *bp = lane < CC / 4 ? a.bias1 : a.bias2;
+            const float *b1 = a.bias1, *b2 = a.bias2;
+            if constexpr (STEPS) {
+                b1 = a.ch[wave].bias1;
+                b2 = a.ch[wave].bias2;
+            }
+            const float *bp = lane < CC / 4 ? b1 : b2;
             const void *src = (bp && lane < CC / 2) ? static_cast<const void *>(bp + 4 * k) : static_cast<const void *>(a.zeros + 4 * (lane & 31));
-            lds_dma<16>(src, reinterpret_cast<float *>(lds_sx + a.bias_off));
+            lds_dma<16>(src, reinterpret_cast<float *>(lds_sx + a.bias_off + (STEPS ? wave * 1024 : 0)));
         }
     }
     auto bias_from_lds = [&](int conv, f32x4 (&bq)[4]) __attribute__((always_inline)) {
         u32x4 t4[4];
 #pragma unroll
         for (int q = 0; q < 4; q++)
-            asm volatile("ds_read_b128 %0, %1" : "=v"(t4[q]) : "v"(lds0 + a.bias_off + (uint32_t)(conv * (WM * 32) + wm * 32 + 8 * q + 4 * hi) * 4u) : "memory");
+            asm volatile("ds_read_b128 %0, %1" : "=v"(t4[q]) : "v"(lds0 + a.bias_off + bias_slot + (uint32_t)(conv * (WM * 32) + wm * 32 + 8 * q + 4 * hi) * 4u) : "memory");
         asm volatile("s_waitcnt lgkmcnt(0)" ::: "memory");
         __builtin_amdgcn_sched_barrier(0);
 #pragma unroll
@@ -499,16 +511,18 @@
         float ws1, ws2;
         int K1, dil1, K2, dil2;
         uint32_t xoff, yoff;
+        int ylo, xlo;
     };
     auto chain_par = [&](int ci) {
         ChainPar c;
-        if constexpr (NCH == 1) {
-            c = ChainPar{wbase1, wbase2, a.bias1, a.bias2, a.wscale1, a.wscale2, a.K1, a.dil1, a.K2, a.dil2, 0u, 0u};
+        if constexpr (NCH == 1 && !STEPS) {
+            c = ChainPar{wbase1, wbase2, a.bias1, a.bias2, a.wscale1, a.wscale2, a.K1, a.dil1, a.K2, a.dil2, 0u, 0u, 0, 0};
         } else {
             const auto &h = a.ch[ci];
             c = ChainPar{reinterpret_cast<const char *>(h.wp1) + wm * (MW * NPW * 1024),
                          reinterpret_cast<const char *>(h.wp2) + wm * (MW * NPW * 1024),
-                         h.bias1, h.bias2, h.wscale1, h.wscale2, h.K1, h.dil1, h.K2, h.dil2, (uint32_t)h.xoff, (uint32_t)h.yoff};
+                         h.bias1, h.bias2, h.wscale1, h.wscale2, h.K1, h.dil1, h.K2, h.dil2, (uint32_t)h.xoff, (uint32_t)h.yoff,
+                         h.ylo, h.xlo};
         }
         return c;
     };
@@ -521,8 +535,16 @@
 #else
     ASet f1s[DEPTH + 1], f2s[DEPTH + 1];
 #endif
+    auto fresh = [&](int v) __attribute__((always_inline)) {
+        if constexpr (STEPS) asm volatile("" : "+v"(v));
+        return v;
+    };
+    auto next_ci = [&](int ci) __attribute__((always_inline)) {
+        if constexpr (STEPS) return __builtin_amdgcn_readfirstlane(ci + 1);
+        else return ci + 1;
+    };
 #pragma unroll 1
-    for (int ci = 0; ci < NCH; ci++) {
+    for (int ci = 0; ci < nst; ci = next_ci(ci)) {
     const ChainPar cp = chain_par(ci);
     if constexpr (NCH > 1) {
         if (ci > 0) {
@@ -536,14 +558,14 @@
         }
     }
     if constexpr (!SHA) load_a(f1s[0], cp.wb1, 0);
-    if (ci == 0) {
+    if (ci == 0 || STEPS) {
         asm volatile("s_waitcnt lgkmcnt(0)" ::: "memory");
 #if SX_PAIR_PROF
-        tp[2] = stamp();
+        if (ci == 0) tp[2] = stamp();
 #endif
         __builtin_amdgcn_s_barrier();
 #if SX_PAIR_PROF
-        tp[3] = stamp();
+        if (ci == 0) tp[3] = stamp();
 #endif
     }
     __builtin_amdgcn_sched_barrier(0);
@@ -576,11 +598,13 @@
 #pragma unroll
             for (int q = 0; q < 4; q++) bq[q] = *reinterpret_cast<const f32x4 *>(biasp + (row0 + 8 * q + 4 * hi) * b_on);
         }
+        const int l31 = fresh(lane & 31), hi = fresh(lane >> 5);
 #pragma unroll
         for (int n = 0; n < NW; n++) {
             const int col = (wn * NW + n) * 32 + l31;
             const int t = t1 + col;
-            const bool live = t >= 0 && t < TV;
+            bool live = t >= 0 && t < TV;
+            if constexpr (STEPS) live = live && col >= cp.ylo && col < 256 - cp.ylo;
 #pragma unroll
             for (int q = 0; q < 4; q++) {
                 float o[4];
@@ -639,12 +663,14 @@
 #pragma unroll
             for (int q = 0; q < 4; q++) bq[q] = *reinterpret_cast<const f32x4 *>(biasp + (row0 + 8 * q + 4 * hi) * b_on);
         }
+        const int l31 = fresh(lane & 31), hi = fresh(lane >> 5);
         static_for<NW / 2>([&](auto R) {
             constexpr int rr = decltype(R)::value;
             f32x4 adl[2][4];
             if constexpr ((flags & EPI_ACC) != 0 && !(EARLY && ACC)) {
 #pragma unroll
                 for (int j = 0; j < 2; j++) {
+                    if (STEPS && ci + 1 < nst) continue;
                     const int t = t1 + (wn * NW + rr * 2 + j) * 32 + l31;
                     const int tl = t < 0 ? 0 : (t < T ? t : T - 1);
 #pragma unroll
@@ -657,9 +683,9 @@
                 const int n = rr * 2 + j;
                 const int col = (wn * NW + n) * 32 + l31;
                 const int t = t1 + col;
-                const bool kept = !(col < a.pad2 || col >= a.pad2 + a.BNo || t >= TV);
+                const bool kept = !(col < koff || col >= koff + a.BNo || t >= TV);
                 if constexpr (NCH == 1) {
-                    if (!kept) continue;
+                    if (!kept && !(STEPS && ci + 1 < nst)) continue;
                 }
 #pragma unroll
                 for (int q = 0; q < 4; q++) {
@@ -667,6 +693,12 @@
 #pragma unroll
                     for (int e = 0; e < 4; e++) v[e] = __builtin_fmaf(acc[n][4 * q + e], wsc, bq[q][e]);
                     v += pre[rr][j][q];
+                    if constexpr (STEPS) {
+                        if (ci + 1 < nst) {
+                            pre[rr][j][q] = v;
+                            continue;
+                        }
+                    }
                     if constexpr (NCH > 1) {
                         if (ci > 0) v += tot[rr][j][q];
                         tot[rr][j][q] = v;
@@ -693,6 +725,41 @@
             }
         });
     }
+    if constexpr (STEPS) {
+        if (ci + 1 < nst) {
+            asm volatile("s_waitcnt lgkmcnt(0)" ::: "memory");
+            __builtin_amdgcn_s_barrier();
+            __builtin_amdgcn_sched_barrier(0);
+            const float isl = a.islope;
+            const int pad1 = a.pad1;
+            const int l31 = fresh(lane & 31), hi = fresh(lane >> 5);
+#pragma unroll
+            for (int n = 0; n < NW; n++) {
+                const int col = (wn * NW + n) * 32 + l31;
+                const int t = t1 + col;
+                const bool ok = t >= 0 && t < TV && col >= cp.xlo && col < 256 - cp.xlo;
+#pragma unroll
+                for (int q = 0; q < 4; q++) {
+                    float v[4];
+#pragma unroll
+                    for (int e = 0; e < 4; e++) {
+                        const float x = ok ? pre[n / 2][n % 2][q][e] : 0.f;
+                        v[e] = fmaxf(x, x * isl);
+                    }
+                    unsigned wa[2], wb[2];
+                    split2h_pair_pk(v[0], v[1], wa[0], wa[1], pk);
+                    split2h_pair_pk(v[2], v[3], wb[0], wb[1], pk);
+                    const int g = 4 * wm + q;
+                    const uint32_t cell = lds0 + (uint32_t)(g >> 1) * XB + (uint32_t)((g & 1) * LW + pad1 + col) * 16u + 8u * hi;
+                    asm volatile("ds_write_b64 %0, %1" ::"v"(cell), "v"(u32x2{wa[0], wb[0]}) : "memory");
+                    asm volatile("ds_write_b64 %0, %1" ::"v"(cell + (uint32_t)(2 * LW) * 16u), "v"(u32x2{wa[1], wb[1]}) : "memory");
+                }
+                asm volatile("" : "+v"(pk));
+            }
+            zero_acc();
+            bias_slot += 1024u;
+        }
+    }
     }
 #if SX_PAIR_PROF
     asm volatile("s_waitcnt vmcnt(0)" ::: "memory");
@@ -705,16 +772,28 @@
     if (a.peak) sx_publish_peak(a.peak, (int)blockIdx.x, pk);
 }
 
-template <int MW, int NW, int WM, int WN, int EPI, bool CHAIN, int NCH = 1>
+template <int MW, int NW, int WM, int WN, int EPI, bool CHAIN, int NCH = 1, bool STEPS = false>
 inline hipError_t launch_conv_sx_pair_k(const SxPairArgs &a, dim3 grid, size_t lds, hipStream_t stream) {
     static std::atomic<uint64_t> attr_done{0};
-    auto kern = conv_sx_pair_kernel<MW, NW, WM, WN, EPI, CHAIN, NCH>;
+    auto kern = conv_sx_pair_kernel<MW, NW, WM, WN, EPI, CHAIN, NCH, STEPS>;
     if (hipError_t e = sx_allow_big_lds(reinterpret_cast<const void *>(kern), attr_done); e != hipSuccess) return e;
     if (g_launch_name_on)
-        snprintf(g_launch_name, sizeof g_launch_name, "conv_sx_pair_kernel<%d, %d, %d, %d, %d, %s, %d>", MW, NW, WM, WN, EPI,
-                 CHAIN ? "true" : "false", NCH);
+        snprintf(g_launch_name, sizeof g_launch_name, "conv_sx_pair_kernel<%d, %d, %d, %d, %d, %s, %d, %s>", MW, NW, WM, WN, EPI,
+                 CHAIN ? "true" : "false", NCH, STEPS ? "true" : "false");
     kern<<<grid, 256, lds, stream>>>(a);
     return hipGetLastError();
+}
+
+inline int sx_pair_min_keep(int C) {
+    static const int keep_min = [] {
+        const char *e = std::getenv("VITSMI_PAIR_MIN_KEEP");
+        return e ? std::atoi(e) : 160;
+    }();
+    static const int keep64 = [] {
+        const char *e = std::getenv("VITSMI_PAIR_MIN_KEEP64");
+        return e ? std::atoi(e) : 200;
+    }();
+    return C == 64 && keep64 > keep_min ? keep64 : keep_min;
 }
 
 inline bool sx_pair_supported(int C, int cfg, int K1, int dil1, int K2, int dil2) {
@@ -723,16 +802,7 @@
     const int LW1 = 256 + (K1 - 1) * dil1;
     if (2 * LW1 > kSxRawStageCells) return false;
     const int halo2 = (K2 - 1) * dil2;
-    static const int keep_min = [] {
-        const char *e = std::getenv("VITSMI_PAIR_MIN_KEEP");
-        return e ? std::atoi(e) : 160;
-    }();
-    if (halo2 % 2 || 256 - halo2 < keep_min) return false;
-    static const int keep64 = [] {
-        const char *e = std::getenv("VITSMI_PAIR_MIN_KEEP64");
-        return e ? std::atoi(e) : 200;
-    }();
-    if (C == 64 && 256 - halo2 < keep64) return false;
+    if (halo2 % 2 || 256 - halo2 < sx_pair_min_keep(C)) return false;
     const size_t lds_y = (size_t)(C / 16) * 4 * (size_t)((256 + halo2 / 2 + 7) / 8 * 8) * 16 + (size_t)(halo2 / 2) * 16;
     const size_t lds_x = (size_t)(C / 16) * 4 * LW1 * 16;
     return (lds_y > lds_x ? lds_y : lds_x) <= kLdsTwoPerCu;
@@ -796,6 +866,102 @@
 }
 #endif
 
+struct SxStepsGeom {
+    int pad1, pad2, LW1, LW2, koff, BNo;
+    int xoff[3], yoff[3], ylo[3], xlo[3];
+    size_t lds;
+};
+inline bool sx_steps_geom(int C, int cfg, int n, const int *K1, const int *dil1, const int *K2, const int *dil2, SxStepsGeom *g) {
+    if (n < 2 || n > 3) return false;
+    SxStepsGeom s{};
+    int r1[3], r2[3];
+    for (int i = 0; i < n; i++) {
+        if (!(K1[i] & 1) || !(K2[i] & 1) || !sx_pair_supported(C, cfg, K1[i], dil1[i], K2[i], dil2[i])) return false;
+        r1[i] = (K1[i] - 1) / 2 * dil1[i];
+        r2[i] = (K2[i] - 1) / 2 * dil2[i];
+        s.pad1 = r1[i] > s.pad1 ? r1[i] : s.pad1;
+        s.pad2 = r2[i] > s.pad2 ? r2[i] : s.pad2;
+    }
+    int lo = 0;
+    for (int i = 0; i < n; i++) {
+        s.xoff[i] = s.pad1 - r1[i];
+        s.yoff[i] = s.pad2 - r2[i];
+        s.ylo[i] = i ? lo + r1[i] : 0;
+        s.xlo[i] = lo = s.ylo[i] + r2[i];
+    }
+    s.koff = lo;
+    s.BNo = 256 - 2 * lo;
+    if (s.BNo < sx_pair_min_keep(C)) return false;
+    s.LW1 = 256 + 2 * s.pad1;
+    if (2 * s.LW1 > kSxRawStageCells) return false;
+    s.LW2 = (256 + s.pad2 + 7) / 8 * 8;
+    const size_t lds_x = (size_t)(C / 16) * 4 * s.LW1 * 16, lds_y = (size_t)(C / 16) * 4 * s.LW2 * 16 + (size_t)s.pad2 * 16;
+    s.lds = lds_x > lds_y ? lds_x : lds_y;
+    if (s.lds + 3 * 1024 > kLdsTwoPerCu) return false;
+    if (g) *g = s;
+    return true;
+}
+
+hipError_t launch_conv_sx_steps(SxPairArgs a, int cfg, int B, hipStream_t stream);
+#ifdef VITSMI_IMPL_PAIR
+hipError_t launch_conv_sx_steps(SxPairArgs a, int cfg, int B, hipStream_t stream) {
+    int K1[3], d1[3], K2[3], d2[3];
+    if (a.nchain < 2 || a.nchain > 3) return hipErrorInvalidValue;
+    for (int i = 0; i < a.nchain; i++) {
+        K1[i] = a.ch[i].K1;
+        d1[i] = a.ch[i].dil1;
+        K2[i] = a.ch[i].K2;
+        d2[i] = a.ch[i].dil2;
+    }
+    SxStepsGeom g;
+    if (!sx_steps_geom(a.C, cfg, a.nchain, K1, d1, K2, d2, &g)) return hipErrorInvalidValue;
+    for (int i = 0; i < a.nchain; i++) {
+        a.ch[i].xoff = g.xoff[i];
+        a.ch[i].yoff = g.yoff[i];
+        a.ch[i].ylo = g.ylo[i];
+        a.ch[i].xlo = g.xlo[i];
+        if (a.ch[i].wscale1 == 0.f) a.ch[i].wscale1 = 1.f;
+        if (a.ch[i].wscale2 == 0.f) a.ch[i].wscale2 = 1.f;
+    }
+    a.pad1 = g.pad1;
+    a.pad2 = g.pad2;
+    a.LW1 = g.LW1;
+    a.x_bytes = (unsigned)((size_t)4 * a.LW1 * 16);
+    a.LW2 = g.LW2;
+    a.y_chunk_bytes = (unsigned)(4 * a.LW2 * 16);
+    a.koff = g.koff;
+    a.BNo = g.BNo;
+    a.NT = (a.T + a.BNo - 1) / a.BNo;
+    a.B = B;
+    a.nchunks = a.C / 16;
+    if (a.islope == 0.f) a.islope = 1.f;
+    if (a.mslope == 0.f) a.mslope = 1.f;
+    if ((long long)a.T * 64 + 64 >= (1ll << 32)) return hipErrorInvalidValue;
+    a.bias_off = (unsigned)((g.lds + 15) / 16 * 16);
+    const size_t lds = a.bias_off + 3 * 1024;
+    const long long nb = (long long)a.NT * B;
+    if (nb == 0) return hipSuccess;
+    a.xgs = a.NT >= (2 << sx_xcd_group_shift()) ? sx_xcd_group_shift() : 0;
+    const long long per_round = 8ll << a.xgs;
+    const long long wgs = (nb + per_round - 1) / per_round * per_round;
+    if (wgs >= (1ll << 31)) return hipErrorInvalidValue;
+    dim3 grid((unsigned)wgs, 1, 1);
+    const int epi = a.flags & (EPI_ACC | EPI_DIV);
+    if ((epi & EPI_DIV) && !(epi & EPI_ACC)) return hipErrorInvalidValue;
+#define SX_STEPS_CASES(MW, NW, WM, WN)                                                                                    \
+    switch (epi) {                                                                                                        \
+        case 0: return launch_conv_sx_pair_k<MW, NW, WM, WN, 0, false, 1, true>(a, grid, lds, stream);                    \
+        case EPI_ACC: return launch_conv_sx_pair_k<MW, NW, WM, WN, EPI_ACC, false, 1, true>(a, grid, lds, stream);        \
+        default: return launch_conv_sx_pair_k<MW, NW, WM, WN, EPI_ACC | EPI_DIV, false, 1, true>(a, grid, lds, stream);   \
+    }
+    if (cfg == 1) {
+        SX_STEPS_CASES(1, 4, 2, 2)
+    }
+    SX_STEPS_CASES(1, 2, 1, 4)
+#undef SX_STEPS_CASES
+}
+#endif
+
 struct SxMrfGeom {
     int pad1, pad2, LW1, LW2;
     size_t lds;
diff --git a/phoonnx_amd/csrc/vitsmi.hip b/phoonnx_amd/csrc/vitsmi.hip
--- a/phoonnx_amd/csrc/vitsmi.hip
+++ b/phoonnx_amd/csrc/vitsmi.hip
@@ -761,6 +761,68 @@
     fused_launch_end(c, ev, members, 2, c1, T, fl, by);
 }
 
+bool pair_steps_on() {
+    const char *e = std::getenv("VITSMI_PAIR_STEPS");
+    return !(e && e[0] == '0');
+}
+
+bool sx_steps_ok(const vits_handle *h, const ResBlockDesc &rb) {
+    if (!pair_steps_on() || !rb.type1 || rb.n < 2 || rb.n > 3) return false;
+    int K1[3], d1[3], K2[3], d2[3];
+    for (int q = 0; q < rb.n; q++) {
+        const ConvDesc &c1 = rb.c1[q], &c2 = rb.c2[q];
+        if (!sx_pair_ok(h, c1, c2) || c1.K != 3 || c2.K != 3 || c1.padL * 2 != (c1.K - 1) * c1.dil || c1.cfg != rb.c1[0].cfg) return false;
+        K1[q] = c1.K, d1[q] = c1.dil, K2[q] = c2.K, d2[q] = c2.dil;
+    }
+    return sx_steps_geom(rb.c1[0].Cin, rb.c1[0].cfg, rb.n, K1, d1, K2, d2, nullptr);
+}
+
+static SxPairArgs sx_steps_args(const ConvDesc *const *c1, const ConvDesc *const *c2, int n, const float *A, const float *zeros,
+                                const float *x, int T, float *out, int flags, float div, float slope, SxRagged rag, unsigned *peak) {
+    SxPairArgs a{};
+    const auto P = [A](int64_t off) { return off >= 0 ? A + off : nullptr; };
+    a.xr = x;
+    a.islope = a.mslope = slope;
+    a.T = T;
+    a.out_raw = out;
+    a.zeros = zeros;
+    a.C = c1[0]->Cin;
+    a.flags = flags & (EPI_ACC | EPI_DIV);
+    a.div = div;
+    a.nchain = n;
+    for (int s = 0; s < n; s++) {
+        auto &ch = a.ch[s];
+        ch.wp1 = reinterpret_cast<const u32x4 *>(P(c1[s]->w_off));
+        ch.wp2 = reinterpret_cast<const u32x4 *>(P(c2[s]->w_off));
+        ch.bias1 = P(c1[s]->b_off);
+        ch.bias2 = P(c2[s]->b_off);
+        ch.wscale1 = c1[s]->wscale;
+        ch.wscale2 = c2[s]->wscale;
+        ch.K1 = c1[s]->K; ch.dil1 = c1[s]->dil;
+        ch.K2 = c2[s]->K; ch.dil2 = c2[s]->dil;
+    }
+    a.rag = rag;
+    a.peak = peak;
+    return a;
+}
+
+void conv_sx_steps(Ctx &c, const ResBlockDesc &rb, const float *x, int T, float *out, int flags, float div, float slope) {
+    const int n = rb.n;
+    const ConvDesc *c1[3], *c2[3], *members[6];
+    double macs = 0, bytes = 0;
+    for (int q = 0; q < n; q++) {
+        members[2 * q] = c1[q] = &rb.c1[q];
+        members[2 * q + 1] = c2[q] = &rb.c2[q];
+        macs += c1[q]->macs_per_t + c2[q]->macs_per_t;
+        bytes += 4.0 * ((double)(c1[q]->Cin + c1[q]->Cout) + (double)(c2[q]->Cin + c2[q]->Cout));
+    }
+    const SxPairArgs a = sx_steps_args(c1, c2, n, c.A, c.P(c.m.zeros_off), x, T, out, flags, div, slope, c.rag_at(T), range_slots(c.h, true));
+    const bool ev = conv_event_begin(c);
+    c.note(launch_conv_sx_steps(a, rb.c1[0].cfg, c.B, c.st));
+    const double wf = c.work_frac();
+    fused_launch_end(c, ev, members, 2 * n, rb.c1[0], T, 2.0 * macs * (double)T * c.B * wf, bytes * T * c.B * wf);
+}
+
 bool sx_pair16_ok(const vits_handle *h, const ConvDesc &c1, const ConvDesc &c2) {
     static const bool off = [] {
         const char *e = std::getenv("VITSMI_PAIR16");
@@ -1597,6 +1659,11 @@
                 }
                 return w;
             };
+            if (fr && sx_steps_ok(h, rbk)) {
+                const StepOut w = step_out(rbk.n - 1);
+                conv_sx_steps(c, rbk, y_raw, T, w.raw, w.flags, (float)nk, S);
+                continue;
+            }
             const float *cur = y_raw;
             const uint16_t *cura = y_pl;
             for (int q = 0; q < rbk.n; q++) {
@@ -4776,6 +4843,84 @@
     return VITS_OK;
 }
 
+int vits_test_conv_pair_steps(int device_id, vits_test_conv_pair_steps_args *p) {
+    if (int rc = test_dev(device_id)) return rc;
+    if (!p) return fail(nullptr, VITS_E_ARG, "no arguments");
+    const auto bad = [](const char *why) { return fail(nullptr, VITS_E_ARG, "fused steps hook: %s", why); };
+    const int B = p->B, C = p->C, T = p->T, K = p->K, ns = p->n;
+    if (B < 1 || C < 1 || T < 1 || K < 1 || !p->x || !p->out) return bad("bad shape or missing tensor");
+    if (ns < 2 || ns > 3) return bad("2 or 3 steps");
+    if (p->flags & ~(VITS_P16_EPI_ACC | VITS_P16_EPI_DIV)) return bad("unknown flag");
+    if ((p->flags & VITS_P16_EPI_DIV) && !(p->flags & VITS_P16_EPI_ACC)) return bad("div without acc");
+    if ((p->flags & VITS_P16_EPI_ACC) && !p->old_out) return bad("acc without old_out (the accumulate operand is the raw tensor's previous contents)");
+    if (p->lens && p->rag_mul < 1) return bad("rag_mul < 1");
+    if (p->lens)
+        for (int b = 0; b < B; b++)
+            if (p->lens[b] < 0 || p->lens[b] > T) return bad("lens outside [0, T]");
+    ConvDesc d1[3], d2[3];
+    std::vector<float> arena;
+    const TestPack o = sx_test_pack(SxPack::F16X2);
+    int K1[3], D1[3], K2[3], D2[3];
+    for (int s = 0; s < ns; s++) {
+        if (!p->w1[s] || !p->w2[s] || p->dil1[s] < 1 || p->dil2[s] < 1) return bad("a step without weights or dilation");
+        std::string e = pack_test_conv(p->w1[s], p->b1[s], C, C, K, p->dil1[s], p->dil1[s] * (K - 1) / 2, 3, &d1[s], &arena, o);
+        if (e.empty()) e = pack_test_conv(p->w2[s], p->b2[s], C, C, K, p->dil2[s], p->dil2[s] * (K - 1) / 2, 3, &d2[s], &arena, o);
+        if (!e.empty()) return fail(nullptr, VITS_E_ARG, "%s", e.c_str());
+        if (!d1[s].rawin || !d2[s].rawin || d1[s].cfg != d1[0].cfg || d2[s].cfg != d1[0].cfg) return bad("not raw-format convs of one tile");
+        K1[s] = d1[s].K, D1[s] = d1[s].dil, K2[s] = d2[s].K, D2[s] = d2[s].dil;
+    }
+    SxStepsGeom geom;
+    if (!sx_steps_geom(C, d1[0].cfg, ns, K1, D1, K2, D2, &geom))
+        return fail(nullptr, VITS_E_ARG, "these steps cannot run as one launch (C %d, kernel %d, first dilations %d, %d)", C, K, p->dil1[0], p->dil1[1]);
+    const size_t n = (size_t)B * C * T;
+    std::vector<int> l32(B);
+    for (int b = 0; b < B; b++) l32[b] = p->lens ? (int)p->lens[b] : T;
+    std::vector<float> ho(n, p->sentinel);
+    if (p->old_out) std::memcpy(ho.data(), p->old_out, n * 4);
+    DevBufs D;
+    float *dA = D.up(arena.data(), arena.size());
+    float *dx = D.up(p->x, n, 16);
+    float *dimg = D.up(ho.data(), n, 16);
+    float *dxr = D.alloc<float>(n, 16);
+    float *draw = D.alloc<float>(n, 16);
+    float *dout = D.alloc<float>(n, 16);
+    int *dlen = p->lens ? D.up(l32.data(), (size_t)B) : nullptr;
+    unsigned *dpk = D.fill<unsigned>((size_t)kSxPeakSlots * kSxPeakStride);
+    TCHECK(D.err);
+    const dim3 grid((T + 255) / 256, C / 8, B);
+    sx_block_kernel<<<grid, 256>>>(dx, (int64_t)C * T, T, nullptr, dxr, C, T);
+    sx_block_kernel<<<grid, 256>>>(dimg, (int64_t)C * T, T, nullptr, draw, C, T);
+    TCHECK(hipGetLastError());
+    const ConvDesc *c1[3], *c2[3];
+    for (int s = 0; s < ns; s++) c1[s] = &d1[s], c2[s] = &d2[s];
+    const int kflags = ((p->flags & VITS_P16_EPI_ACC) ? EPI_ACC : 0) | ((p->flags & VITS_P16_EPI_DIV) ? EPI_DIV : 0);
+    const SxRagged rag = dlen ? SxRagged{dlen, p->rag_add, p->rag_mul} : SxRagged{nullptr, 0, 0};
+    const SxPairArgs a = sx_steps_args(c1, c2, ns, dA, dA, dxr, T, draw, kflags, p->div == 0.f ? 1.f : p->div, p->slope, rag, dpk);
+    auto go = [&] { return launch_conv_sx_steps(a, d1[0].cfg, B, nullptr); };
+    const bool name_was_on = g_launch_name_on;
+    g_launch_name_on = true;
+    g_launch_name[0] = 0;
+    const hipError_t le = go();
+    g_launch_name_on = name_was_on;
+    if (le != hipSuccess) return fail(nullptr, VITS_E_DEVICE, "fused steps hook: launch_conv_sx_steps: %s", hipGetErrorString(le));
+    TCHECK(hipDeviceSynchronize());
+    std::snprintf(p->kernel, sizeof p->kernel, "%s", g_launch_name);
+    p->BNo = geom.BNo;
+    sx_unblock_kernel<<<grid, 256>>>(draw, nullptr, dout, C, T, 1);
+    TCHECK(hipGetLastError());
+    TCHECK(hipDeviceSynchronize());
+    TCHECK(download(p->out, dout, n));
+    {
+        std::vector<unsigned> slots((size_t)kSxPeakSlots * kSxPeakStride);
+        TCHECK(download(slots.data(), dpk, slots.size()));
+        unsigned top = 0;
+        for (int s = 0; s < kSxPeakSlots; s++) top = std::max(top, slots[(size_t)s * kSxPeakStride]);
+        std::memcpy(&p->peak, &top, 4);
+    }
+    if (p->ms_out) TCHECK(time_launches(10, go, p->ms_out));
+    return VITS_OK;
+}
+
 int vits_bench_conv1d_sx(int device_id, int B, int Cin, int Cout, int T, int K, int dil, int dbg, int iters,
                          float *ms_out) {
     if (int rc = test_dev(device_id)) return rc;
diff --git a/phoonnx_amd/session.py b/phoonnx_amd/session.py
--- a/phoonnx_amd/session.py
+++ b/phoonnx_amd/session.py
@@ -2408,6 +2408,46 @@
             "peak": float(a.peak), "guard_ok": bool(a.guard_ok)}
 
 
+def test_conv_pair_steps(x, steps, flags=(), slope=0.1, div=1.0, old_out=None, lens=None, rag_add=0, rag_mul=1,
+                         sentinel=CONV_EPI_SENTINEL, timed=False, device_id=0):
+    lib = _ffi.load()
+    f32 = lambda a: None if a is None else np.ascontiguousarray(a, np.float32)
+    x, old_out = f32(x), f32(old_out)
+    B, Cc, T = x.shape
+    if not 1 <= len(steps) <= 3:
+        raise ValueError("1 to 3 steps fit the argument block (the launch takes 2 or 3)")
+    K = np.shape(steps[0][0])[2]
+    ln = None if lens is None else np.ascontiguousarray(lens, np.int64)
+    keep = []
+    a = _ffi.VitsTestConvPairStepsArgs()
+    for s, (w1, b1, d1, w2, b2, d2) in enumerate(steps):
+        w1, b1, w2, b2 = (f32(v) for v in (w1, b1, w2, b2))
+        for name, arr, shape in (("w1", w1, (Cc, Cc, K)), ("w2", w2, (Cc, Cc, K)), ("b1", b1, (Cc,)), ("b2", b2, (Cc,))):
+            if arr is not None and arr.shape != shape:
+                raise ValueError(f"step {s}: {name} has shape {arr.shape}, the launch needs {shape}")
+        keep += [w1, b1, w2, b2]
+        a.w1[s], a.b1[s], a.w2[s], a.b2[s] = (_ffi.ptr(v) for v in (w1, b1, w2, b2))
+        a.dil1[s], a.dil2[s] = d1, d2
+    for name, arr, shape in (("old_out", old_out, (B, Cc, T)), ("lens", ln, (B,))):
+        if arr is not None and arr.shape != shape:
+            raise ValueError(f"{name} has shape {arr.shape}, the launch needs {shape}")
+    out = np.empty((B, Cc, T), np.float32)
+    ms = C.c_float(0.0)
+    a.B, a.C, a.T, a.K, a.n = B, Cc, T, K, len(steps)
+    a.flags = sum(P16_EPI_FLAGS[f] for f in flags)
+    a.slope, a.div, a.sentinel = slope, div, sentinel
+    a.x, a.old_out, a.lens, a.out = (_ffi.ptr(v) for v in (x, old_out, ln, out))
+    a.rag_add, a.rag_mul = rag_add, rag_mul
+    a.ms_out = C.cast(C.pointer(ms), C.c_void_p) if timed else None
+    rc = lib.vits_test_conv_pair_steps(device_id, C.byref(a))
+    if rc != 0:
+        raise SessionError(_ffi.last_error(None))
+    res = {"out": out, "kernel": a.kernel.decode(), "BNo": a.BNo, "peak": float(a.peak)}
+    if timed:
+        res["ms"] = float(ms.value)
+    return res
+
+
 def bench_conv1d_sx(B, Cin, Cout, T, K, dil=1, dbg=0, iters=20, device_id=0):
     lib = _ffi.load()
     res = np.zeros(8, np.float32)
```

Result: no change. 143.1 million, median of 6 (+0.7%).
